# arkworks-rs/sumcheck

Measured on AMD Instinct MI355X. Metric: MLSumcheck prover field-ops/s (BLS12-381 Fr, nv=24), higher is better.
Workload: dtype u256 (BLS12-381 Fr, Montgomery form; integer arithmetic on 9 x 29-bit limbs); 1 GPU; BASELINE config 3: MLSumcheck prove, ListOfProducts [[0, 1, 2, 3], [4, 5, 6], [7, 8], [9]] over 10 tables, nv=24 (24 per GPU shard), BLS12-381 Fr, tables HBM-resident; nv=24, nv_per_gpu=24, tables=10, degree=4, launcher=single process, ranks_seen=1, communicator=none, round_loop=library, round_loop_reason=single GPU: no exchange

## Files before the change

include/sumcheck_hip.h:

```cpp
#ifndef SUMCHECK_HIP_H
#define SUMCHECK_HIP_H

#include <stddef.h>
#include <stdint.h>

#ifdef __cplusplus
extern "C" {
#endif

#define SC_ABI_VERSION 5
#define SC_API __attribute__((visibility("default")))

enum sc_status {
    SC_OK = 0,
    SC_ERR_CONSTANT_POLY = 1,
    SC_ERR_FIRST_ROUND_HAS_MSG = 2,
    SC_ERR_MISSING_MSG = 3,
    SC_ERR_NOT_ACTIVE = 4,
    SC_ERR_BAD_ARG = 5,
    SC_ERR_HIP = 6,
    SC_ERR_OOM = 7,
    SC_ERR_REJECT = 8
};

enum sc_flags {
    SC_TABLES_ON_DEVICE = 1u << 0,
    SC_TABLES_BORROW = 1u << 1,
    SC_TABLES_STREAM = 1u << 2,
    SC_NO_DEVICE_POLLING = 1u << 3
};

typedef struct sc_poly_desc {
    uint32_t num_vars;
    uint32_t max_multiplicands;
    uint32_t n_products;
    const uint64_t *coeffs;
    const uint32_t *prod_offsets;
    const uint32_t *prod_indices;
    uint32_t n_tables;
    const uint64_t *const *tables;
    uint32_t flags;
} sc_poly_desc;

typedef struct sc_prover sc_prover;
typedef struct sc_rng sc_rng;

SC_API int sc_abi_version(void);
SC_API const char *sc_last_error(void);
SC_API int sc_device_count(void);
SC_API int sc_set_device(int ordinal);

SC_API int sc_prover_init(const sc_poly_desc *desc, sc_prover **out);
SC_API int sc_prover_init_streamed(const sc_poly_desc *desc, uint32_t chunk_log2, sc_prover **out);
SC_API int sc_prove_round(sc_prover *p, const uint64_t *r_or_null, uint64_t *out_evals);
SC_API int sc_prover_set_resident(sc_prover *p, uint32_t patience_polls);
SC_API int sc_prover_push_randomness(sc_prover *p, const uint64_t *r);
SC_API int sc_prover_state(sc_prover *p, uint64_t *randomness, uint32_t *n_randomness, uint64_t *tables_out, uint32_t *round);
SC_API void sc_prover_free(sc_prover *p);
SC_API int sc_prover_set_stream(sc_prover *p, void *hip_stream, int use_own);
SC_API int sc_prover_set_polling(sc_prover *p, int allow);

SC_API int sc_prove_round_partial(sc_prover *p, const uint64_t *r_or_null, uint64_t *d_wide_out);
SC_API int sc_wide_reduce(const uint64_t *wide, uint32_t n_elems, uint64_t *out);
SC_API int sc_prover_bind_final(sc_prover *p, const uint64_t *r, uint64_t *d_out);

typedef struct sc_comm sc_comm;
typedef int (*sc_allreduce_u64_fn)(void *ctx, uint64_t *inout, size_t count);
typedef int (*sc_allgather_fn)(void *ctx, const void *send, void *recv, size_t bytes);
SC_API int sc_comm_unique_id(uint8_t *out128);
SC_API int sc_comm_init(const uint8_t *id128, int rank, int nranks, sc_comm **out);
SC_API int sc_comm_init_host(int rank, int nranks, sc_allreduce_u64_fn allreduce, sc_allgather_fn allgather, void *ctx, sc_comm **out);
SC_API int sc_comm_init_p2p(uint64_t group_id, int rank, int nranks, sc_comm **out);
SC_API int sc_comm_selftest(sc_comm *comm);
SC_API void sc_comm_free(sc_comm *comm);
#define SC_COMM_RCCL 1
#define SC_COMM_HOST 2
#define SC_COMM_P2P 3
#define SC_COMM_DIRECT_PUBLISH 0x100
SC_API int sc_comm_info(sc_comm *comm, int *rank_out, int *nranks_out, int *kind_out);
SC_API int sc_comm_exchange_bench(sc_comm *comm, uint32_t n_words, uint32_t iters, double *us_mean_out, double *us_min_out_or_null);
SC_API int sc_set_publish_timeout_ms(uint32_t ms);
SC_API int sc_ml_prove_sharded(sc_prover *p, sc_comm *comm, sc_rng *rng_or_null, uint32_t nv_total, uint64_t *out_proof,
                               uint64_t *out_randomness);
SC_API int sc_ml_prove_sharded_rounds(sc_prover *p, sc_comm *comm, sc_rng *rng, uint32_t nv_total, uint32_t n_rounds, uint64_t *out_proof,
                                      uint64_t *out_randomness);

SC_API int sc_fix_variables(const uint64_t *in, uint32_t nv, const uint64_t *point, uint32_t k, uint64_t *out, uint32_t flags);

SC_API sc_rng *sc_rng_setup(void);
SC_API void sc_rng_free(sc_rng *rng);
SC_API void sc_rng_feed_bytes(sc_rng *rng, const uint8_t *buf, size_t len);
SC_API void sc_rng_fill_bytes(sc_rng *rng, uint8_t *dest, size_t len);
SC_API void sc_rng_feed_poly_info(sc_rng *rng, uint64_t max_multiplicands, uint64_t num_variables);
SC_API void sc_rng_feed_prover_msg(sc_rng *rng, const uint64_t *evals, uint32_t n);
SC_API void sc_rng_sample_fr(sc_rng *rng, uint64_t *out);

SC_API int sc_ml_prove(const sc_poly_desc *desc, sc_rng *rng_or_null, uint64_t *out_proof, sc_prover **out_state_or_null);
SC_API int sc_ml_prove_rounds(sc_prover *p, sc_rng *rng, uint32_t n_rounds, uint64_t *out_proof, uint64_t *out_randomness);
SC_API int sc_ml_prove_handle(sc_prover *p, sc_rng *rng_or_null, uint64_t *out_proof);
SC_API int sc_ml_prove_batch(const sc_poly_desc *descs, uint32_t n, sc_rng *const *rngs_or_null, uint64_t *out_proofs,
                             uint64_t *out_randomness_or_null);

SC_API int sc_interpolate_uni_poly(const uint64_t *p_i, uint32_t len, const uint64_t *eval_at, uint64_t *out);
SC_API int sc_ml_verify(uint32_t num_vars, uint32_t max_multiplicands, const uint64_t *claimed_sum, const uint64_t *proof,
                 uint64_t proof_elems, sc_rng *rng_or_null, uint64_t *out_point, uint64_t *out_expected);

SC_API int sc_gkr_phase_one(const uint64_t *f1_idx, const uint64_t *f1_vals, uint64_t nnz, uint32_t dim, const uint64_t *f3,
                     const uint64_t *g, uint32_t flags, uint64_t *h_g, uint64_t *f1g_idx, uint64_t *f1g_vals, uint64_t *f1g_nnz);
SC_API int sc_gkr_phase_two(const uint64_t *f1g_idx, const uint64_t *f1g_vals, uint64_t nnz, uint32_t dim, const uint64_t *u,
                     uint32_t flags, uint64_t *f1_gu);
SC_API int sc_gkr_prove(sc_rng *rng, const uint64_t *f1_idx, const uint64_t *f1_vals, uint64_t nnz, uint32_t dim,
                 const uint64_t *f2, const uint64_t *f3, const uint64_t *g, uint32_t flags, uint64_t *out_proof, uint64_t *out_uv_or_null);
SC_API int sc_gkr_prove_batch(uint32_t n, uint32_t dim, sc_rng *const *rngs,
                              const uint64_t *const *f1_idx, const uint64_t *const *f1_vals, const uint64_t *nnz,
                              const uint64_t *const *f2, const uint64_t *const *f3, const uint64_t *const *g,
                              uint32_t flags, uint64_t *out_proofs, uint64_t *out_uv_or_null);
SC_API int sc_gkr_phase_one_sharded(sc_comm *comm_or_null, const uint64_t *f1_idx, const uint64_t *f1_vals, uint64_t nnz_local, uint32_t dim,
                                    const uint64_t *f3, const uint64_t *g, uint32_t flags, uint64_t *h_g_or_null, uint64_t *lanes_or_null,
                                    uint64_t *f1g_idx, uint64_t *f1g_vals, uint64_t *f1g_nnz);
SC_API int sc_gkr_phase_two_sharded(sc_comm *comm_or_null, const uint64_t *f1g_idx, const uint64_t *f1g_vals, uint64_t nnz_local, uint32_t dim,
                                    const uint64_t *u, uint32_t flags, uint64_t *f1_gu_or_null, uint64_t *lanes_or_null);
SC_API int sc_gkr_prove_sharded(sc_comm *comm, sc_rng *rng, const uint64_t *f1_idx, const uint64_t *f1_vals, uint64_t nnz_local, uint32_t dim,
                                const uint64_t *f2, const uint64_t *f3, const uint64_t *g, uint32_t flags, uint64_t *out_proof,
                                uint64_t *out_uv_or_null);
SC_API int sc_wide_reduce_table(const uint64_t *lanes, uint64_t n, uint64_t *out, uint32_t flags);
SC_API int sc_dense_scale(const uint64_t *in, uint64_t n, const uint64_t *scalar, uint64_t *out, uint32_t flags);

SC_API int sc_poly_evaluate(const sc_poly_desc *desc, const uint64_t *point, uint64_t *out_value, uint64_t *out_table_values_or_null);

SC_API int sc_sparse_evaluate(const uint64_t *idx, const uint64_t *vals, uint64_t nnz, uint32_t num_vars, const uint64_t *point,
                              uint64_t *out);

SC_API int sc_poly_evaluate_batch(const sc_poly_desc *descs, uint32_t n, const uint64_t *points,
                                  uint64_t *out_values, uint64_t *out_table_values_or_null);
SC_API int sc_gkr_subclaim_batch(uint32_t n, uint32_t dim,
                                 const uint64_t *const *f1_idx, const uint64_t *const *f1_vals, const uint64_t *nnz,
                                 const uint64_t *const *f2, const uint64_t *const *f3, const uint64_t *const *g,
                                 const uint64_t *uv, uint32_t flags, uint64_t *out_evals);

SC_API int sc_release_caches(void);
SC_API int sc_set_cache_limit(uint64_t bytes);
SC_API int sc_library_stats(uint64_t *out, uint32_t n);
SC_API int sc_set_policy(const char *key, int64_t value);
SC_API int sc_get_policy(const char *key, int64_t *value);
SC_API uint32_t sc_plan_count(void);
SC_API const char *sc_plan_name(uint32_t i);
SC_API int sc_plan_stats(uint64_t *out, uint32_t n);

SC_API int sc_synth_table_device(uint64_t seed, uint64_t stream, uint64_t first, uint64_t n, uint64_t *d_out);
SC_API int sc_prover_last_round_ms(sc_prover *p, float *ms);
SC_API int sc_prover_set_timing(sc_prover *p, int on);
SC_API int sc_prover_get_timing(sc_prover *p, double *ms_per_product, uint64_t *launches_per_product, double *rounds_ms);
SC_API int sc_prover_get_round_timing(sc_prover *p, double *ms_per_round, uint64_t *launches_per_round);
SC_API int sc_prover_reset(sc_prover *p, const uint64_t *const *tables_or_null, uint32_t flags);
SC_API int sc_claim_weights(uint32_t M, const uint64_t *r, uint64_t *out);
SC_API int sc_fr_elementwise(int op, const uint64_t *a, const uint64_t *b, uint64_t *out, uint64_t n);
SC_API int sc_bench_modmul(uint64_t n_threads, uint32_t reps, uint32_t variant, float *ms_out, uint64_t *checksum_out);

#ifdef __cplusplus
}
#endif
#endif
```

sumcheck_amd/_lib.py:

```python
from __future__ import annotations

import ctypes as C
import os

HERE = os.path.dirname(os.path.abspath(__file__))
SO_PATH = os.path.join(HERE, "libsumcheck_hip_exp.so" if os.environ.get("SC_LIB_VARIANT") == "exp" else "libsumcheck_hip.so")
if os.environ.get("SC_LIB_PATH"):
    SO_PATH = os.environ["SC_LIB_PATH"]

u64p = C.POINTER(C.c_uint64)
u32p = C.POINTER(C.c_uint32)
u8p = C.POINTER(C.c_uint8)

SC_OK = 0
SC_ERR_CONSTANT_POLY = 1
SC_ERR_FIRST_ROUND_HAS_MSG = 2
SC_ERR_MISSING_MSG = 3
SC_ERR_NOT_ACTIVE = 4
SC_ERR_BAD_ARG = 5
SC_ERR_HIP = 6
SC_ERR_OOM = 7
SC_ERR_REJECT = 8

SC_TABLES_ON_DEVICE = 1
SC_TABLES_BORROW = 2
SC_TABLES_STREAM = 4
SC_NO_DEVICE_POLLING = 8


class PolyDesc(C.Structure):
    _fields_ = [
        ("num_vars", C.c_uint32),
        ("max_multiplicands", C.c_uint32),
        ("n_products", C.c_uint32),
        ("coeffs", u64p),
        ("prod_offsets", u32p),
        ("prod_indices", u32p),
        ("n_tables", C.c_uint32),
        ("tables", C.POINTER(C.c_void_p)),
        ("flags", C.c_uint32),
    ]


_V = C.c_void_p
SIGNATURES = {
    "sc_abi_version": (C.c_int, []),
    "sc_last_error": (C.c_char_p, []),
    "sc_device_count": (C.c_int, []),
    "sc_set_device": (C.c_int, [C.c_int]),
    "sc_prover_init": (C.c_int, [C.POINTER(PolyDesc), C.POINTER(_V)]),
    "sc_prover_init_streamed": (C.c_int, [C.POINTER(PolyDesc), C.c_uint32, C.POINTER(_V)]),
    "sc_prove_round": (C.c_int, [_V, _V, _V]),
    "sc_prover_push_randomness": (C.c_int, [_V, _V]),
    "sc_prover_state": (C.c_int, [_V, _V, u32p, _V, u32p]),
    "sc_prover_free": (None, [_V]),
    "sc_prover_set_stream": (C.c_int, [_V, _V, C.c_int]),
    "sc_prover_set_polling": (C.c_int, [_V, C.c_int]),
    "sc_prover_set_resident": (C.c_int, [_V, C.c_uint32]),
    "sc_set_cache_limit": (C.c_int, [C.c_uint64]),
    "sc_library_stats": (C.c_int, [u64p, C.c_uint32]),
    "sc_set_policy": (C.c_int, [C.c_char_p, C.c_int64]),
    "sc_get_policy": (C.c_int, [C.c_char_p, C.POINTER(C.c_int64)]),
    "sc_plan_count": (C.c_uint32, []),
    "sc_plan_name": (C.c_char_p, [C.c_uint32]),
    "sc_plan_stats": (C.c_int, [u64p, C.c_uint32]),
    "sc_prove_round_partial": (C.c_int, [_V, _V, _V]),
    "sc_wide_reduce": (C.c_int, [_V, C.c_uint32, _V]),
    "sc_prover_bind_final": (C.c_int, [_V, _V, _V]),
    "sc_comm_unique_id": (C.c_int, [_V]),
    "sc_comm_init": (C.c_int, [_V, C.c_int, C.c_int, C.POINTER(_V)]),
    "sc_comm_init_host": (C.c_int, [C.c_int, C.c_int, _V, _V, _V, C.POINTER(_V)]),
    "sc_comm_init_p2p": (C.c_int, [C.c_uint64, C.c_int, C.c_int, C.POINTER(_V)]),
    "sc_comm_selftest": (C.c_int, [_V]),
    "sc_comm_free": (None, [_V]),
    "sc_comm_info": (C.c_int, [_V, C.POINTER(C.c_int), C.POINTER(C.c_int), C.POINTER(C.c_int)]),
    "sc_comm_exchange_bench": (C.c_int, [_V, C.c_uint32, C.c_uint32, C.POINTER(C.c_double), C.POINTER(C.c_double)]),
    "sc_set_publish_timeout_ms": (C.c_int, [C.c_uint32]),
    "sc_ml_prove_sharded": (C.c_int, [_V, _V, _V, C.c_uint32, _V, _V]),
    "sc_ml_prove_sharded_rounds": (C.c_int, [_V, _V, _V, C.c_uint32, C.c_uint32, _V, _V]),
    "sc_fix_variables": (C.c_int, [_V, C.c_uint32, _V, C.c_uint32, _V, C.c_uint32]),
    "sc_poly_evaluate": (C.c_int, [_V, _V, _V, _V]),
    "sc_ml_prove_rounds": (C.c_int, [_V, _V, C.c_uint32, _V, _V]),
    "sc_release_caches": (C.c_int, []),
    "sc_sparse_evaluate": (C.c_int, [_V, _V, C.c_uint64, C.c_uint32, _V, _V]),
    "sc_rng_setup": (_V, []),
    "sc_rng_free": (None, [_V]),
    "sc_rng_feed_bytes": (None, [_V, C.c_char_p, C.c_size_t]),
    "sc_rng_fill_bytes": (None, [_V, _V, C.c_size_t]),
    "sc_rng_feed_poly_info": (None, [_V, C.c_uint64, C.c_uint64]),
    "sc_rng_feed_prover_msg": (None, [_V, _V, C.c_uint32]),
    "sc_rng_sample_fr": (None, [_V, _V]),
    "sc_ml_prove": (C.c_int, [C.POINTER(PolyDesc), _V, _V, C.POINTER(_V)]),
    "sc_ml_prove_handle": (C.c_int, [_V, _V, _V]),
    "sc_ml_prove_batch": (C.c_int, [C.POINTER(PolyDesc), C.c_uint32, C.POINTER(_V), _V, _V]),
    "sc_interpolate_uni_poly": (C.c_int, [_V, C.c_uint32, _V, _V]),
    "sc_ml_verify": (C.c_int, [C.c_uint32, C.c_uint32, _V, _V, C.c_uint64, _V, _V, _V]),
    "sc_gkr_phase_one": (C.c_int, [_V, _V, C.c_uint64, C.c_uint32, _V, _V, C.c_uint32, _V, _V, _V, u64p]),
    "sc_gkr_phase_two": (C.c_int, [_V, _V, C.c_uint64, C.c_uint32, _V, C.c_uint32, _V]),
    "sc_gkr_prove": (C.c_int, [_V, _V, _V, C.c_uint64, C.c_uint32, _V, _V, _V, C.c_uint32, _V, _V]),
    "sc_gkr_prove_batch": (C.c_int, [C.c_uint32, C.c_uint32, C.POINTER(_V), C.POINTER(_V), C.POINTER(_V), u64p, C.POINTER(_V), C.POINTER(_V), C.POINTER(_V),
                                     C.c_uint32, _V, _V]),
    "sc_poly_evaluate_batch": (C.c_int, [C.POINTER(PolyDesc), C.c_uint32, _V, _V, _V]),
    "sc_gkr_subclaim_batch": (C.c_int, [C.c_uint32, C.c_uint32, C.POINTER(_V), C.POINTER(_V), u64p, C.POINTER(_V), C.POINTER(_V), C.POINTER(_V), _V, C.c_uint32, _V]),
    "sc_dense_scale": (C.c_int, [_V, C.c_uint64, _V, _V, C.c_uint32]),
    "sc_gkr_phase_one_sharded": (C.c_int, [_V, _V, _V, C.c_uint64, C.c_uint32, _V, _V, C.c_uint32, _V, _V, _V, _V, u64p]),
    "sc_gkr_phase_two_sharded": (C.c_int, [_V, _V, _V, C.c_uint64, C.c_uint32, _V, C.c_uint32, _V, _V]),
    "sc_gkr_prove_sharded": (C.c_int, [_V, _V, _V, _V, C.c_uint64, C.c_uint32, _V, _V, _V, C.c_uint32, _V, _V]),
    "sc_wide_reduce_table": (C.c_int, [_V, C.c_uint64, _V, C.c_uint32]),
    "sc_synth_table_device": (C.c_int, [C.c_uint64, C.c_uint64, C.c_uint64, C.c_uint64, _V]),
    "sc_prover_last_round_ms": (C.c_int, [_V, C.POINTER(C.c_float)]),
    "sc_prover_set_timing": (C.c_int, [_V, C.c_int]),
    "sc_prover_get_timing": (C.c_int, [_V, C.POINTER(C.c_double), u64p, C.POINTER(C.c_double)]),
    "sc_prover_get_round_timing": (C.c_int, [_V, C.POINTER(C.c_double), u64p]),
    "sc_prover_reset": (C.c_int, [_V, _V, C.c_uint32]),
    "sc_claim_weights": (C.c_int, [C.c_uint32, _V, _V]),
    "sc_fr_elementwise": (C.c_int, [C.c_int, _V, _V, _V, C.c_uint64]),
    "sc_bench_modmul": (C.c_int, [C.c_uint64, C.c_uint32, C.c_uint32, C.POINTER(C.c_float), u64p]),
}

ABI_VERSION = 5
_lib = None


def _missing_symbol(name):
    def stub(*_a, **_k):
        raise SumcheckError(SC_ERR_BAD_ARG, f"{SO_PATH} does not export {name} (an older build loaded with SC_AB_ALLOW_MISSING=1)")
    return stub


class SumcheckError(RuntimeError):
    def __init__(self, code: int, msg: str):
        super().__init__(f"[sc_status {code}] {msg}")
        self.code = code
        self.msg = msg


def lib():
    global _lib
    if _lib is None:
        if not os.path.exists(SO_PATH):
            raise ImportError(
                f"{SO_PATH} is missing: build it with `python -c 'import __graft_entry__ as g; g.build()'` "
                "(sumcheck_amd has no CPU fallback)")
        try:
            import torch
        except Exception:
            pass
        L = C.CDLL(SO_PATH)
        allow_missing = os.environ.get("SC_AB_ALLOW_MISSING") == "1"
        for name, (res, args) in SIGNATURES.items():
            try:
                fn = getattr(L, name)
            except AttributeError:
                if not allow_missing:
                    raise
                setattr(L, name, _missing_symbol(name))
                continue
            fn.restype = res
            fn.argtypes = args
        got = L.sc_abi_version()
        if got != ABI_VERSION:
            msg = f"{SO_PATH} reports ABI version {got}, this loader declares {ABI_VERSION}: signatures may not match"
            if not allow_missing:
                raise ImportError(msg + " (rebuild: python -c 'import __graft_entry__ as g; g.build()')")
            import warnings
            warnings.warn(msg)
        _lib = L
    return _lib


def check(rc: int):
    if rc != SC_OK:
        raise SumcheckError(rc, lib().sc_last_error().decode("utf-8", "replace"))


def set_policy(key: str, value: int) -> None:
    check(lib().sc_set_policy(key.encode(), int(value)))


def get_policy(key: str) -> int:
    v = C.c_int64()
    check(lib().sc_get_policy(key.encode(), C.byref(v)))
    return int(v.value)


class policy:

    def __init__(self, **kv):
        self.kv, self.old = kv, {}

    def __enter__(self):
        for k, v in self.kv.items():
            self.old[k] = get_policy(k)
            set_policy(k, v)
        return self

    def __exit__(self, *exc):
        for k, v in self.old.items():
            set_policy(k, v)
        return False


def plan_stats() -> dict:
    L = lib()
    n = L.sc_plan_count()
    out = (C.c_uint64 * n)()
    check(L.sc_plan_stats(out, n))
    return {L.sc_plan_name(i).decode(): int(out[i]) for i in range(n)}
```

sumcheck_amd/csrc/abi.hip:

```cpp
#include "prover_internal.hpp"

static std::atomic<uint32_t> g_publish_timeout_ms{0};
std::chrono::milliseconds publish_timeout() {
    uint32_t ms = g_publish_timeout_ms.load(std::memory_order_relaxed);
    if (ms == 0) {
        const char *e = std::getenv("SC_PUBLISH_TIMEOUT_MS");
        const long v = e ? std::atol(e) : 0;
        ms = v > 0 ? (uint32_t)std::min<long>(v, 3600 * 1000L) : 20000u;
        g_publish_timeout_ms.store(ms, std::memory_order_relaxed);
    }
    return std::chrono::milliseconds(ms);
}
extern "C" int sc_set_publish_timeout_ms(uint32_t ms) {
    g_publish_timeout_ms.store(ms ? ms : 20000u, std::memory_order_relaxed);
    return SC_OK;
}
static thread_local std::string g_last_error;
static thread_local int g_device = 0;

static std::recursive_mutex g_gate_mutex[64];
thread_local uint16_t g_gate_depth[64];
void gate_lock(int device) {
    g_gate_mutex[(unsigned)device & 63u].lock();
    ++g_gate_depth[(unsigned)device & 63u];
}
void gate_unlock(int device) {
    --g_gate_depth[(unsigned)device & 63u];
    g_gate_mutex[(unsigned)device & 63u].unlock();
}
void sc_internal_gate_lock(int device) { gate_lock(device); }
void sc_internal_gate_unlock(int device) { gate_unlock(device); }

uint64_t sc_internal_cache_limit();
int sc_internal_device() { return g_device; }
int &sc_internal_device_ref() { return g_device; }

int sc_internal_fail(int code, const char *fmt, ...) {
    char buf[512];
    va_list ap;
    va_start(ap, fmt);
    vsnprintf(buf, sizeof(buf), fmt, ap);
    va_end(ap);
    g_last_error = buf;
    return code;
}

extern "C" int sc_abi_version(void) { return SC_ABI_VERSION; }
extern "C" const char *sc_last_error(void) { return g_last_error.c_str(); }
extern "C" int sc_device_count(void) {
    int n = 0;
    if (hipGetDeviceCount(&n) != hipSuccess) {
        (void)hipGetLastError();
        return 0;
    }
    return n;
}
extern "C" int sc_set_device(int ordinal) {
    HIP_TRY(hipSetDevice(ordinal));
    g_device = ordinal;
    return SC_OK;
}

extern "C" sc_rng *sc_rng_setup(void) { return new (std::nothrow) sc_rng(); }
extern "C" void sc_rng_free(sc_rng *rng) { delete rng; }
extern "C" void sc_rng_feed_bytes(sc_rng *rng, const uint8_t *buf, size_t len) { rng->rng.feed_bytes(buf, len); }
extern "C" void sc_rng_fill_bytes(sc_rng *rng, uint8_t *dest, size_t len) { rng->rng.fill_bytes(dest, len); }
extern "C" void sc_rng_feed_poly_info(sc_rng *rng, uint64_t max_multiplicands, uint64_t num_variables) {
    rng->rng.feed_poly_info(max_multiplicands, num_variables);
}
extern "C" void sc_rng_feed_prover_msg(sc_rng *rng, const uint64_t *evals, uint32_t n) {
    rng->rng.feed_prover_msg(reinterpret_cast<const sch::Fr *>(evals), n);
}
extern "C" void sc_rng_sample_fr(sc_rng *rng, uint64_t *out) {
    const sch::Fr a = rng->rng.sample_fr();
    std::memcpy(out, a.l, 32);
}


int resident_quiesce(sc_prover *p);
void prover_destroy(sc_prover *p) {
    if (!p) return;
    (void)resident_quiesce(p);
    DeviceGate gate_(p->device);
    (void)hipSetDevice(p->device);
    if (p->deferred_pending && p->sig) {
        __atomic_store_n(p->sig, p->sig_seq, __ATOMIC_RELEASE);
        p->deferred_pending = false;
    }
    if (p->own_stream) (void)hipStreamSynchronize(p->own_stream);
    if (p->arena) (void)hipFree(p->arena);
    if (p->d_partials) (void)hipFree(p->d_partials);
    if (p->d_partials2) (void)hipFree(p->d_partials2);
    if (p->d_fin_counters) (void)hipFree(p->d_fin_counters);
    if (p->d_finprods) (void)hipFree(p->d_finprods);
    if (p->d_W) (void)hipFree(p->d_W);
    if (p->d_scratch) (void)hipFree(p->d_scratch);
    if (p->d_sums[0]) (void)hipFree(p->d_sums[0]);
    if (p->d_out) (void)hipFree(p->d_out);
    if (p->h_out) (void)hipHostFree(p->h_out);
    if (p->h_flag) (void)hipHostFree(p->h_flag);
    for (int q = 0; q < 2; ++q) {
        if (p->ring[q]) (void)hipFree(p->ring[q]);
        if (p->ev_copied[q]) (void)hipEventDestroy(p->ev_copied[q]);
        if (p->ev_consumed[q]) (void)hipEventDestroy(p->ev_consumed[q]);
    }
    if (p->d_chunk_msg) (void)hipFree(p->d_chunk_msg);
    if (p->copy_stream) (void)hipStreamDestroy(p->copy_stream);
    if (p->copy_stream2) (void)hipStreamDestroy(p->copy_stream2);
    for (int q = 0; q < 2; ++q)
        if (p->ev_copied2[q]) (void)hipEventDestroy(p->ev_copied2[q]);
    if (p->tail) prover_destroy(p->tail);
    if (p->d_tail_send) (void)hipFree(p->d_tail_send);
    if (p->d_tail_recv) (void)hipFree(p->d_tail_recv);
    if (p->d_tail_tabs) (void)hipFree(p->d_tail_tabs);
    if (p->d_wide) (void)hipFree(p->d_wide);
    if (p->h_wide) (void)hipHostFree(p->h_wide);
    if (p->d_combos) (void)hipFree(p->d_combos);
    if (p->h_mail) (void)hipHostFree(p->h_mail);
    if (p->d_mail) (void)hipFree(p->d_mail);
    if (p->d_tail_sync) (void)hipFree(p->d_tail_sync);
    if (p->d_tail_xw) (void)hipFree(p->d_tail_xw);
    if (p->d_vram_mail) (void)hipFree(p->d_vram_mail);
    if (p->d_cur_tables) (void)hipFree(p->d_cur_tables);
    if (p->h_cur_tables) (void)hipHostFree(p->h_cur_tables);
    if (p->d_slot_table) (void)hipFree(p->d_slot_table);
    if (p->d_slot_exp) (void)hipFree(p->d_slot_exp);
    if (p->ev0) (void)hipEventDestroy(p->ev0);
    if (p->ev1) (void)hipEventDestroy(p->ev1);
    for (hipEvent_t e : p->prod_ev) (void)hipEventDestroy(e);
    if (p->own_stream) (void)hipStreamDestroy(p->own_stream);
    delete p;
}

bool handle_pool_offer(sc_prover *p);
extern "C" void sc_prover_free(sc_prover *p) {
    if (p) (void)resident_quiesce(p);
    if (p && handle_pool_offer(p)) return;
    prover_destroy(p);
}

int validate_desc(const sc_poly_desc *d) {
    if (!d) return sc_internal_fail(SC_ERR_BAD_ARG, "null descriptor");
    if (d->num_vars == 0) return sc_internal_fail(SC_ERR_CONSTANT_POLY, "Attempt to prove a constant.");
    if (d->num_vars > 40) return sc_internal_fail(SC_ERR_BAD_ARG, "num_vars %u too large", d->num_vars);
    if (d->n_tables == 0 || !d->tables) return sc_internal_fail(SC_ERR_BAD_ARG, "no tables");
    if (d->n_products && (!d->coeffs || !d->prod_offsets || !d->prod_indices)) return sc_internal_fail(SC_ERR_BAD_ARG, "null product arrays");
    uint32_t mx = 0;
    for (uint32_t k = 0; k < d->n_products; ++k) {
        if (d->prod_offsets[k + 1] <= d->prod_offsets[k]) return sc_internal_fail(SC_ERR_BAD_ARG, "product %u is empty", k);
        mx = std::max(mx, d->prod_offsets[k + 1] - d->prod_offsets[k]);
        for (uint32_t q = d->prod_offsets[k]; q < d->prod_offsets[k + 1]; ++q)
            if (d->prod_indices[q] >= d->n_tables) return sc_internal_fail(SC_ERR_BAD_ARG, "product %u refers to table %u >= %u", k, d->prod_indices[q], d->n_tables);
    }
    if (mx != d->max_multiplicands) return sc_internal_fail(SC_ERR_BAD_ARG, "max_multiplicands %u != max product length %u", d->max_multiplicands, mx);
    for (uint32_t u = 0; u < d->n_tables; ++u)
        if (!d->tables[u]) return sc_internal_fail(SC_ERR_BAD_ARG, "table %u is null", u);
    return SC_OK;
}

sch::Fr fr_small(int64_t v) { return v >= 0 ? sch::from_u64((uint64_t)v) : sch::neg(sch::from_u64((uint64_t)(-v))); }

void build_node_matrix(uint32_t M, uint32_t D, const sch::Fr &scale, std::vector<sch::Fr> &out) {
    std::vector<int64_t> xs;
    std::vector<uint32_t> fin;
    int inf_col = -1;
    for (uint32_t s = 0; s <= M; ++s) {
        const int32_t nv = scd::node_value((int)s);
        if (nv == scd::kNodeInf) inf_col = (int)s;
        else fin.push_back(s);
        xs.push_back(nv);
    }
    out.assign((size_t)D * (M + 1), sch::zero());
    for (uint32_t t = 0; t < D; ++t) {
        sch::Fr inf_w = sch::kOne;
        for (uint32_t e = 0; e < M; ++e) inf_w = sch::mul(inf_w, fr_small(t));
        for (uint32_t s : fin) {
            sch::Fr num = sch::kOne, den = sch::kOne;
            for (uint32_t j : fin) {
                if (j == s) continue;
                num = sch::mul(num, fr_small((int64_t)t - xs[j]));
                den = sch::mul(den, fr_small(xs[s] - xs[j]));
            }
            const sch::Fr l = sch::mul(num, sch::inverse(den));
            out[(size_t)t * (M + 1) + s] = sch::mul(scale, l);
            if (inf_col >= 0) {
                sch::Fr xm = sch::kOne;
                for (uint32_t e = 0; e < M; ++e) xm = sch::mul(xm, fr_small(xs[s]));
                inf_w = sch::sub(inf_w, sch::mul(xm, l));
            }
        }
        if (inf_col >= 0) out[(size_t)t * (M + 1) + inf_col] = sch::mul(scale, inf_w);
    }
}

void claim_weights(uint32_t M, const sch::Fr &r, sch::Fr *lam) {
    struct Den {
        sch::Fr inv[5][5];
        Den() {
            for (uint32_t m = 1; m <= 4; ++m)
                for (uint32_t s = 0; s <= m; ++s) {
                    inv[m][s] = sch::zero();
                    if (scd::node_value((int)s) == scd::kNodeInf) continue;
                    sch::Fr den = sch::kOne;
                    for (uint32_t j = 0; j <= m; ++j)
                        if (j != s && scd::node_value((int)j) != scd::kNodeInf) den = sch::mul(den, fr_small((int64_t)scd::node_value((int)s) - scd::node_value((int)j)));
                    inv[m][s] = sch::inverse(den);
                }
        }
    };
    static const Den den;
    sch::Fr diff[5];
    for (uint32_t j = 0; j <= M; ++j)
        if (scd::node_value((int)j) != scd::kNodeInf) diff[j] = sch::sub(r, fr_small(scd::node_value((int)j)));
    sch::Fr inf_w = sch::kOne;
    for (uint32_t e = 0; e < M; ++e) inf_w = sch::mul(inf_w, r);
    int inf_col = -1;
    for (uint32_t s = 0; s <= M; ++s) {
        const int32_t xs = scd::node_value((int)s);
        if (xs == scd::kNodeInf) {
            inf_col = (int)s;
            continue;
        }
        sch::Fr l = den.inv[M][s];
        for (uint32_t j = 0; j <= M; ++j)
            if (j != s && scd::node_value((int)j) != scd::kNodeInf) l = sch::mul(l, diff[j]);
        lam[s] = l;
        sch::Fr xm = sch::kOne;
        for (uint32_t e = 0; e < M; ++e) xm = sch::mul(xm, fr_small(xs));
        inf_w = sch::sub(inf_w, sch::mul(xm, l));
    }
    if (inf_col >= 0) lam[inf_col] = inf_w;
}

int prover_build(const sc_poly_desc *d, sc_prover *p) {
    DeviceGate gate_(g_device);
    if (sc_device_count() <= 0) return sc_internal_fail(SC_ERR_HIP, "no HIP device visible: libsumcheck_hip has no CPU fallback");
    p->device = g_device;
    HIP_TRY(hipSetDevice(p->device));
    HIP_TRY(hipStreamCreateWithFlags(&p->own_stream, hipStreamNonBlocking));
    p->stream = p->own_stream;
    HIP_TRY(hipEventCreate(&p->ev0));
    HIP_TRY(hipEventCreate(&p->ev1));
    p->nv = d->num_vars;
    p->max_mult = d->max_multiplicands;
    p->D = d->max_multiplicands + 1;
    p->K = d->n_products;
    p->U = d->n_tables;
    p->randomness.reserve(p->nv);
    if (d->flags & SC_NO_DEVICE_POLLING) {
        p->pipeline_ok = false;
        p->polling_off_by_caller = true;
    }
#ifdef SC_EXPERIMENTS
    if (const char *e = std::getenv("SC_FE")) p->use_fe = std::atoi(e) != 0;
    if (const char *e = std::getenv("SC_KERNEL")) p->kernel_variant = std::atoi(e);
    if (!p->use_fe && p->kernel_variant == 3) p->kernel_variant = 0;
#endif
    p->use_f29 = p->kernel_variant == 3;
    p->wide_tree = wide_tree_enabled();
#ifdef SC_EXPERIMENTS
    if (const char *e = std::getenv("SC_F29")) p->use_f29 = p->use_f29 && std::atoi(e) != 0;
#endif
    for (uint32_t k = 0; k < d->n_products; ++k)
        if (d->prod_offsets[k + 1] - d->prod_offsets[k] > (p->wide_tree ? 8u : 4u)) p->use_f29 = false;
    if (d->n_tables > (uint32_t)scd::kMaxSmallTables) p->use_f29 = false;
    p->merge_rounds = p->kernel_variant == 3 && d->n_products > 0 && d->n_products <= (uint32_t)scd::kMaxRoundProds;
    for (uint32_t k = 0; k < d->n_products; ++k)
        if (d->prod_offsets[k + 1] - d->prod_offsets[k] > 4) p->merge_rounds = false;
#ifdef SC_EXPERIMENTS
    if (const char *e = std::getenv("SC_MERGE")) p->merge_rounds = p->merge_rounds && std::atoi(e) != 0;
    if (const char *e = std::getenv("SC_FUSED_FIN")) p->fused_finalize = std::atoi(e) != 0;
#endif
    p->use_tail = scd::policy(scd::kPolTail) != 0;

    uint64_t partial_elems = 0;
    std::vector<uint32_t> slot_table, slot_exp;
    std::vector<FinProd> fin(p->K);
    std::vector<Combo> combos;
    std::vector<sch::Fr> Wall;
    for (uint32_t k = 0; k < p->K; ++k) {
        Product pr;
        std::memcpy(&pr.coeff, d->coeffs + 4 * k, 32);
        if (sch::geq_p(pr.coeff)) return sc_internal_fail(SC_ERR_BAD_ARG, "coefficient %u is not a canonical field element", k);
        for (uint32_t q = d->prod_offsets[k]; q < d->prod_offsets[k + 1]; ++q) {
            const uint32_t t = d->prod_indices[q];
            auto it = std::find(pr.tables.begin(), pr.tables.end(), t);
            if (it == pr.tables.end()) {
                pr.tables.push_back(t);
                pr.exps.push_back(1);
            } else {
                pr.exps[it - pr.tables.begin()]++;
            }
        }
        p->prod_indices.emplace_back(d->prod_indices + d->prod_offsets[k], d->prod_indices + d->prod_offsets[k + 1]);
        pr.M = d->prod_offsets[k + 1] - d->prod_offsets[k];
        pr.fused = pr.M <= (uint32_t)scd::kMaxFusedM;
        if (!pr.fused) p->any_generic = true;
        pr.partial_off = partial_elems;
        partial_elems += (uint64_t)scd::kMaxGrid * (pr.M + 1);
        pr.slot_off = (uint32_t)slot_table.size();
        slot_table.insert(slot_table.end(), pr.tables.begin(), pr.tables.end());
        slot_exp.insert(slot_exp.end(), pr.exps.begin(), pr.exps.end());
        fin[k].M = pr.M;
        fin[k].pad = 0;
        fin[k].partial_off = pr.partial_off;
        {
            sch::Fr sc = pr.coeff;
            for (uint32_t dbl = 0; dbl < 5 * (pr.M - 1); ++dbl) sc = sch::add(sc, sc);
            std::vector<sch::Fr> w;
            fin[k].w_off = Wall.size();
            build_node_matrix(pr.M, p->D, pr.coeff, w);
            Wall.insert(Wall.end(), w.begin(), w.end());
            build_node_matrix(pr.M, p->D, sc, w);
            Wall.insert(Wall.end(), w.begin(), w.end());
        }
        for (uint32_t t = 0; t <= pr.M; ++t) {
            Combo c;
            c.t = t;
            c.M = pr.M;
            c.slot_off = pr.slot_off;
            c.n_slots = (uint32_t)pr.tables.size();
            c.partial_off = pr.partial_off;
            combos.push_back(c);
        }
        p->prods.push_back(std::move(pr));
    }

    const bool on_device = d->flags & SC_TABLES_ON_DEVICE;
    const bool borrow = on_device && (d->flags & SC_TABLES_BORROW);
    const uint64_t n = 1ULL << p->nv;
    const bool streamed = !on_device && (d->flags & SC_TABLES_STREAM) && p->nv >= 11;
    const bool small_foot = borrow || streamed;
    bool staged = false;
    const uint64_t s0 = small_foot ? std::max<uint64_t>(n >> 1, 1) : n;
    const uint64_t s1 = small_foot ? std::max<uint64_t>(n >> 2, 1) : std::max<uint64_t>(n >> 1, 1);
    const uint64_t per_table = (s0 + s1) * 36;
    HIP_TRY(hipMalloc(&p->arena, per_table * p->U));
    p->arena_bytes = per_table * p->U;
    p->tabs.resize(p->U);
    p->borrow = borrow;
    if (on_device && !borrow) HIP_TRY(hipDeviceSynchronize());
    for (uint32_t u = 0; u < p->U; ++u) {
        Table &t = p->tabs[u];
        char *base = static_cast<char *>(p->arena) + per_table * u;
        t.buf[0] = reinterpret_cast<uint4 *>(base);
        t.buf[1] = reinterpret_cast<uint4 *>(base + s0 * 32);
        t.buf_top[0] = reinterpret_cast<int32_t *>(base + (s0 + s1) * 32);
        t.buf_top[1] = t.buf_top[0] + s0;
        if (streamed) {
            t.cur = nullptr;
            t.next = 0;
            p->host_tabs.push_back(d->tables[u]);
        } else if (borrow) {
            t.cur = reinterpret_cast<const uint4 *>(d->tables[u]);
            t.next = 0;
            p->origin.push_back(t.cur);
        } else {
            if (!on_device && (d->flags & SC_TABLES_STREAM)) p->host_tabs.push_back(d->tables[u]);
            if (!(staged = !on_device && staged_init_applies(p)))
                HIP_TRY(hipMemcpyAsync(t.buf[0], d->tables[u], n * 32, on_device ? hipMemcpyDeviceToDevice : hipMemcpyHostToDevice, p->stream));
            t.cur = t.buf[0];
            t.next = 1;
        }
    }

    if (streamed) {
        p->streamed = true;
        uint32_t cl = p->stream_chunk_request ? p->stream_chunk_request : 22u;
        cl = std::max(10u, std::min(cl, p->nv));
        p->chunk_log2 = cl;
        for (int q = 0; q < 2; ++q) {
            HIP_TRY(hipMalloc(&p->ring[q], ((size_t)p->U << cl) * 32));
            HIP_TRY(hipEventCreateWithFlags(&p->ev_copied[q], hipEventDisableTiming));
            HIP_TRY(hipEventCreateWithFlags(&p->ev_consumed[q], hipEventDisableTiming));
        }
        HIP_TRY(hipStreamCreateWithFlags(&p->copy_stream, hipStreamNonBlocking));
        HIP_TRY(hipMalloc(&p->d_chunk_msg, (size_t)2 * p->D * 32));
    }
    HIP_TRY(hipMalloc(&p->d_partials, std::max<uint64_t>(partial_elems, 1) * 32));
    HIP_TRY(hipMalloc(&p->d_partials2, std::max<uint64_t>(partial_elems, 1) * 32));
    HIP_TRY(hipMalloc(&p->d_fin_counters, 4 * (2 + scd::kMaxGrid / 32 + 16)));
    HIP_TRY(hipMemsetAsync(p->d_fin_counters, 0, 4 * (2 + scd::kMaxGrid / 32 + 16), p->stream));
    p->d_fin_mb_counter = p->d_fin_counters + (2 + scd::kMaxGrid / 32 + 8);
    HIP_TRY(hipMalloc(&p->d_finprods, std::max<size_t>(p->K, 1) * sizeof(FinProd)));
    if (p->K) HIP_TRY(hipMemcpyAsync(p->d_finprods, fin.data(), p->K * sizeof(FinProd), hipMemcpyHostToDevice, p->stream));
    p->h_finprods = fin;
    HIP_TRY(hipMalloc(&p->d_W, std::max<size_t>(2 * Wall.size(), 1) * 32));
    p->w_elems = (uint32_t)Wall.size();
    if (!Wall.empty()) {
        HIP_TRY(hipMemcpyAsync(p->d_W, Wall.data(), Wall.size() * 32, hipMemcpyHostToDevice, p->stream));
        HIP_TRY(hipMemcpyAsync(p->d_W + Wall.size(), Wall.data(), Wall.size() * 32, hipMemcpyHostToDevice, p->stream));
    }
    HIP_TRY(hipMalloc(&p->d_scratch, (size_t)(2 + p->D) * std::max<uint32_t>(p->K, 1) * p->D * 32));
    {
        const size_t one = (size_t)std::max<uint32_t>(p->K, 1) * p->D * 32;
        HIP_TRY(hipMalloc(&p->d_sums[0], 2 * one));
        p->d_sums[1] = reinterpret_cast<FrHost *>(reinterpret_cast<char *>(p->d_sums[0]) + one);
    }
    HIP_TRY(hipMalloc(&p->d_out, (size_t)p->D * 32));
    HIP_TRY(hipHostMalloc(reinterpret_cast<void **>(&p->h_out), (size_t)p->D * 32, hipHostMallocMapped | hipHostMallocCoherent));
    HIP_TRY(hipHostMalloc(reinterpret_cast<void **>(&p->h_flag), 64, hipHostMallocMapped | hipHostMallocCoherent));
    *p->h_flag = 0;
    HIP_TRY(hipHostGetDevicePointer(reinterpret_cast<void **>(&p->h_out_dev), p->h_out, 0));
    HIP_TRY(hipHostGetDevicePointer(reinterpret_cast<void **>(&p->h_flag_dev), p->h_flag, 0));
    p->has_meta = combos.size() <= (size_t)scd::kMetaCombos && slot_table.size() <= (size_t)scd::kMetaSlots;
    if (p->has_meta) {
        std::memset(&p->meta, 0, sizeof(p->meta));
        std::copy(combos.begin(), combos.end(), p->meta.combo);
        std::copy(slot_table.begin(), slot_table.end(), p->meta.slot_table);
        std::copy(slot_exp.begin(), slot_exp.end(), p->meta.slot_exp);
    }
    p->n_combos = (int)combos.size();
    HIP_TRY(hipMalloc(&p->d_combos, std::max<size_t>(combos.size(), 1) * sizeof(Combo)));
    if (!combos.empty()) HIP_TRY(hipMemcpyAsync(p->d_combos, combos.data(), combos.size() * sizeof(Combo), hipMemcpyHostToDevice, p->stream));
    HIP_TRY(hipMalloc(&p->d_slot_table, std::max<size_t>(slot_table.size(), 1) * 4));
    HIP_TRY(hipMalloc(&p->d_slot_exp, std::max<size_t>(slot_exp.size(), 1) * 4));
    if (!slot_table.empty()) {
        HIP_TRY(hipMemcpyAsync(p->d_slot_table, slot_table.data(), slot_table.size() * 4, hipMemcpyHostToDevice, p->stream));
        HIP_TRY(hipMemcpyAsync(p->d_slot_exp, slot_exp.data(), slot_exp.size() * 4, hipMemcpyHostToDevice, p->stream));
    }
    if (p->any_generic || p->U > (uint32_t)scd::kMaxSmallTables) {
        HIP_TRY(hipMalloc(&p->d_cur_tables, 2 * p->U * sizeof(void *)));
        HIP_TRY(hipHostMalloc(reinterpret_cast<void **>(&p->h_cur_tables), 2 * p->U * sizeof(void *), hipHostMallocDefault));
    }
    if (staged) {
        int rc_s = staged_copy_and_round1(p, d->tables);
        if (rc_s) return rc_s;
    }
    HIP_TRY(hipStreamSynchronize(p->stream));
    return SC_OK;
}

std::vector<uint8_t> pool_key_of(const sc_poly_desc *d, int device);
sc_prover *handle_pool_take(const std::vector<uint8_t> &key);
void reset_owner_policy(sc_prover *p, uint32_t desc_flags) {
    p->polling_off_by_caller = (desc_flags & SC_NO_DEVICE_POLLING) != 0;
    p->pipeline_ok = !p->polling_off_by_caller;
    p->resident_spins = kResidentSpinsDefault;
    if (p->timing) (void)sc_prover_set_timing(p, 0);
    p->n_retries = 0;
}
extern "C" int sc_prover_init(const sc_poly_desc *desc, sc_prover **out) {
    if (!out) return sc_internal_fail(SC_ERR_BAD_ARG, "null out");
    *out = nullptr;
    int rc = validate_desc(desc);
    if (rc) return rc;
    std::vector<uint8_t> key = pool_key_of(desc, g_device);
    if (sc_prover *kept = handle_pool_take(key)) {
        if (sc_prover_reset(kept, desc->tables, desc->flags & SC_TABLES_ON_DEVICE) == SC_OK) {
            reset_owner_policy(kept, desc->flags);
            *out = kept;
            return SC_OK;
        }
        kept->pool_key.clear();
        prover_destroy(kept);
    }
    sc_prover *p = new (std::nothrow) sc_prover();
    if (!p) return sc_internal_fail(SC_ERR_OOM, "host allocation failed");
    rc = prover_build(desc, p);
    if (rc) {
        prover_destroy(p);
        return rc;
    }
    p->pool_key = std::move(key);
    *out = p;
    return SC_OK;
}

extern "C" int sc_prover_init_streamed(const sc_poly_desc *desc, uint32_t chunk_log2, sc_prover **out) {
    if (!out) return sc_internal_fail(SC_ERR_BAD_ARG, "null out");
    *out = nullptr;
    int rc = validate_desc(desc);
    if (rc) return rc;
    if (desc->flags & SC_TABLES_ON_DEVICE) return sc_internal_fail(SC_ERR_BAD_ARG, "streamed tables are host tables");
    sc_prover *p = new (std::nothrow) sc_prover();
    if (!p) return sc_internal_fail(SC_ERR_OOM, "host allocation failed");
    p->stream_chunk_request = chunk_log2;
    sc_poly_desc d2 = *desc;
    d2.flags |= SC_TABLES_STREAM;
    rc = prover_build(&d2, p);
    if (rc) {
        prover_destroy(p);
        return rc;
    }
    *out = p;
    return SC_OK;
}

extern "C" int sc_prover_set_stream(sc_prover *p, void *hip_stream, int use_own) {
    if (!p) return sc_internal_fail(SC_ERR_BAD_ARG, "null prover");
    int rc_q = resident_quiesce(p);
    if (rc_q) return rc_q;
    DeviceGate gate_(p->device);
    HIP_TRY(hipSetDevice(p->device));
    HIP_TRY(hipStreamSynchronize(p->stream));
    p->stream = use_own ? p->own_stream : static_cast<hipStream_t>(hip_stream);
    return SC_OK;
}

int collect_timing(sc_prover *p) {
    if (!p->timing || !p->timing_pending) return SC_OK;
    HIP_TRY(hipEventSynchronize(p->ev1));
    float ms = 0.f;
    HIP_TRY(hipEventElapsedTime(&ms, p->ev0, p->ev1));
    p->rounds_ms += ms;
    for (uint32_t k = 0; k < (p->prod_merged ? 1u : p->K) && p->prod_timed; ++k) {
        HIP_TRY(hipEventElapsedTime(&ms, p->prod_ev[2 * k], p->prod_ev[2 * k + 1]));
        p->prod_ms[k] += ms;
        p->prod_launches[k] += 1;
        if (p->timed_round >= 1 && p->timed_round <= p->round_kernel_ms.size()) {
            p->round_kernel_ms[p->timed_round - 1] += ms;
            if (k == 0) p->round_kernel_launches[p->timed_round - 1] += 1;
        }
    }
    p->timing_pending = false;
    return SC_OK;
}

int prover_bind_out(sc_prover *p, const uint64_t *r, uint64_t *d_out) {
    int rc_q = resident_quiesce(p);
    if (rc_q) return rc_q;
    DeviceGate gate_(p->device);
    if (p->exhausted || p->round == 0 || p->round > p->nv) return sc_internal_fail(SC_ERR_NOT_ACTIVE, "bind needs a prover that has run at least one round");
    if (p->streamed && p->round < 2) return sc_internal_fail(SC_ERR_NOT_ACTIVE, "a streamed handle's tables are resident from round 2 on: nothing to bind yet");
    sch::Fr rr;
    std::memcpy(&rr, r, 32);
    if (sch::geq_p(rr)) return sc_internal_fail(SC_ERR_BAD_ARG, "challenge is not a canonical field element");
    HIP_TRY(hipSetDevice(p->device));
    p->randomness.push_back(rr);
    const uint64_t n_out = 1ULL << (p->nv - p->round);
    for (uint32_t u0 = 0; u0 < p->U; u0 += (uint32_t)scd::kMaxSmallTables) {
        const uint32_t cnt = std::min<uint32_t>(p->U - u0, (uint32_t)scd::kMaxSmallTables);
        TablePtrs tp;
        std::memset(&tp, 0, sizeof(tp));
        for (uint32_t j = 0; j < cnt; ++j) {
            tp.src[j] = p->tabs[u0 + j].cur;
// ... 355 lines not shown
    DeviceGate gate_(g_device);
    HIP_TRY(hipSetDevice(g_device));
    const bool on_device = d->flags & SC_TABLES_ON_DEVICE;
    const uint64_t n = 1ULL << nv;
    std::vector<int> levels;
    for (uint32_t left = nv; left > 0;) {
        const int l = left >= 3 ? 3 : (int)left;
        levels.push_back(l);
        left -= l;
    }
    const uint64_t na = levels.empty() ? 1 : n >> levels[0];
    const uint64_t nb = levels.size() < 2 ? 1 : na >> levels[1];
    const size_t bytes_stage = on_device ? 0 : (size_t)U * n * 32, bytes_a = (size_t)U * na * 32, bytes_b = (size_t)U * nb * 32, bytes_v = (size_t)U * 32;
    struct Area {
        void *p = nullptr;
    } stage, wa, wb, vals;
    EvalLease lease;
    DevMem own;
    StreamGuard sg;
    hipStream_t s_eval = nullptr;
    char *base = static_cast<char *>(lease.get(g_device, bytes_stage + bytes_a + bytes_b + bytes_v, &s_eval));
    if (!base) {
        HIP_TRY(hipMalloc(&own.p, bytes_stage + bytes_a + bytes_b + bytes_v));
        HIP_TRY(hipStreamCreateWithFlags(&sg.s, hipStreamNonBlocking));
        base = static_cast<char *>(own.p);
        s_eval = sg.s;
    }
    stage.p = base;
    wa.p = base + bytes_stage;
    wb.p = base + bytes_stage + bytes_a;
    vals.p = base + bytes_stage + bytes_a + bytes_b;
    std::vector<const uint4 *> cur(U);
    for (uint32_t u = 0; u < U; ++u) {
        if (on_device) {
            cur[u] = reinterpret_cast<const uint4 *>(d->tables[u]);
        } else {
            uint4 *dst = static_cast<uint4 *>(stage.p) + 2 * n * u;
            HIP_TRY(hipMemcpyAsync(dst, d->tables[u], n * 32, hipMemcpyHostToDevice, s_eval));
            cur[u] = dst;
        }
    }
    uint64_t m = n;
    uint32_t var = 0;
    for (size_t ps = 0; ps < levels.size(); ++ps) {
        const int L = levels[ps];
        m >>= L;
        const bool last = ps + 1 == levels.size();
        uint4 *area = static_cast<uint4 *>((ps & 1) ? wb.p : wa.p);
        for (uint32_t u0 = 0; u0 < U; u0 += (uint32_t)scd::kMaxSmallTables) {
            const uint32_t cnt = std::min<uint32_t>(U - u0, (uint32_t)scd::kMaxSmallTables);
            scd::FoldArgs fa;
            std::memset(&fa, 0, sizeof(fa));
            for (uint32_t j = 0; j < cnt; ++j) {
                fa.src[j] = cur[u0 + j];
                fa.dst[j] = last ? static_cast<uint4 *>(vals.p) + 2 * (u0 + j) : area + 2 * m * (u0 + j);
            }
            for (int l = 0; l < L; ++l) {
                sch::Fr r32v = pt[var + l];
                for (int dbl = 0; dbl < 5; ++dbl) r32v = sch::add(r32v, r32v);
                fa.r32[l] = to_dev(r32v);
            }
            HIP_TRY(scd::launch_fold_multi(fa, L, (int)cnt, m, s_eval));
            for (uint32_t j = 0; j < cnt; ++j) cur[u0 + j] = fa.dst[j];
        }
        var += L;
    }
    std::vector<sch::Fr> tv(U);
    if (levels.empty()) {
        for (uint32_t u = 0; u < U; ++u) HIP_TRY(hipMemcpyAsync(&tv[u], cur[u], 32, hipMemcpyDeviceToHost, s_eval));
    } else {
        HIP_TRY(hipMemcpyAsync(tv.data(), vals.p, (size_t)U * 32, hipMemcpyDeviceToHost, s_eval));
    }
    HIP_TRY(hipStreamSynchronize(s_eval));
    sch::Fr acc = sch::zero();
    for (uint32_t k = 0; k < d->n_products; ++k) {
        sch::Fr pr;
        std::memcpy(&pr, d->coeffs + 4 * k, 32);
        if (sch::geq_p(pr)) return sc_internal_fail(SC_ERR_BAD_ARG, "coefficient %u is not a canonical field element", k);
        for (uint32_t q = d->prod_offsets[k]; q < d->prod_offsets[k + 1]; ++q) pr = sch::mul(pr, tv[d->prod_indices[q]]);
        acc = sch::add(acc, pr);
    }
    std::memcpy(out_value, &acc, 32);
    if (out_table_values_or_null) std::memcpy(out_table_values_or_null, tv.data(), (size_t)U * 32);
    return SC_OK;
}

static std::atomic<uint64_t> g_cache_limit{16ULL << 30};
uint64_t sc_internal_cache_limit() { return g_cache_limit.load(std::memory_order_relaxed); }
struct HandlePool {
    std::mutex mu;
    sc_prover *h = nullptr;
};
static HandlePool g_pool;
std::vector<uint8_t> pool_key_of(const sc_poly_desc *d, int device) {
    std::vector<uint8_t> k;
    auto put = [&](const void *p, size_t n) {
        const uint8_t *b = static_cast<const uint8_t *>(p);
        k.insert(k.end(), b, b + n);
    };
    const uint32_t head[8] = {d->num_vars, d->max_multiplicands, d->n_products, d->n_tables, d->flags, (uint32_t)device,
                              (uint32_t)scd::policy(scd::kPolWideTree), (uint32_t)scd::policy(scd::kPolTail)};
    put(head, sizeof(head));
    if (d->n_products) {
        put(d->prod_offsets, (size_t)(d->n_products + 1) * 4);
        put(d->prod_indices, (size_t)d->prod_offsets[d->n_products] * 4);
        put(d->coeffs, (size_t)d->n_products * 32);
    }
    return k;
}
sc_prover *handle_pool_take(const std::vector<uint8_t> &key) {
    std::lock_guard<std::mutex> lk(g_pool.mu);
    if (!g_pool.h || g_pool.h->pool_key != key) return nullptr;
    sc_prover *p = g_pool.h;
    g_pool.h = nullptr;
    return p;
}
bool handle_pool_offer(sc_prover *p) {
    if (p->pool_key.empty() || p->arena_bytes > sc_internal_cache_limit() || p->streamed) return false;
    if (p->stream != p->own_stream) return false;
    abandon_deferred(p);
    {
        DeviceGate gate_(p->device);
        (void)hipSetDevice(p->device);
        (void)hipStreamSynchronize(p->own_stream);
    }
    if (p->timing) (void)sc_prover_set_timing(p, 0);
    sc_prover *old = nullptr;
    {
        std::lock_guard<std::mutex> lk(g_pool.mu);
        old = g_pool.h;
        g_pool.h = p;
    }
    if (old) prover_destroy(old);
    return true;
}
void sc_internal_release_handle_pool() {
    sc_prover *old = nullptr;
    {
        std::lock_guard<std::mutex> lk(g_pool.mu);
        old = g_pool.h;
        g_pool.h = nullptr;
    }
    if (old) prover_destroy(old);
}

namespace {
struct PolicyDef {
    const char *name;
    int64_t def, lo, hi;
};
constexpr PolicyDef kPolicyDefs[scd::kPolCount] = {
    {"pipeline", 1, 0, 1},     {"resident", 1, 0, 1},          {"tail_slices", 1, 0, 1}, {"vram_mailbox", 1, 0, 1},           {"wide_tree", 1, 0, 1},
    {"rccl_direct", 1, 0, 1},  {"shard_gather_log2", 15, 1, 15}, {"gkr_direct", 1, 0, 1},  {"wait_spins", 1 << 22, 1, 0xffffffffLL}, {"tail", 1, 0, 1},
    {"staged_init", 1, 0, 1},  {"batch", 1, 0, 2},
};
struct PolicyTable {
    std::atomic<int64_t> v[scd::kPolCount];
    PolicyTable() {
        for (int i = 0; i < scd::kPolCount; ++i) {
            int64_t x = kPolicyDefs[i].def;
#ifdef SC_EXPERIMENTS
            std::string env = "SC_";
            for (const char *c = kPolicyDefs[i].name; *c; ++c) env += (char)std::toupper((unsigned char)*c);
            if (const char *e = std::getenv(env.c_str())) x = std::min(std::max<int64_t>(std::atoll(e), kPolicyDefs[i].lo), kPolicyDefs[i].hi);
#endif
            v[i].store(x, std::memory_order_relaxed);
        }
    }
};
PolicyTable &policy_table() {
    static PolicyTable t;
    return t;
}
std::atomic<uint64_t> g_plan[scd::kPlanCount];
constexpr const char *kPlanNames[scd::kPlanCount] = {
    "big.merged.round1", "big.merged.bind_chain", "big.merged.bind", "big.claim_identity", "big.store_f29", "big.store_canonical", "big.per_product_tree",
    "big.wide", "big.wide16", "big.generic", "big.node_by_node", "big.bind_pass", "big.streamed", "big.staged_round1", "finalize.multi_block", "finalize.one_block", "finalize.no_lds",
    "small.launched", "small.combos_table", "small.ptrs", "small.pipelined", "tail.slices8", "tail.slices12", "tail.rounds", "resident.slices",
    "resident.rounds", "sharded.rccl_direct", "sharded.rccl_publish", "sharded.host", "sharded.p2p", "sharded.gather_tail", "gkr.bucketed_grouped",
    "gkr.bucketed_counted", "gkr.list_form", "gkr.coeff_from_bound_table", "gkr.sharded", "fold_multi",
    "batch.eval_one_block", "batch.eval_serial", "batch.gkr_eval_one_block", "batch.gkr_eval_serial",
    "batch.one_block", "batch.serial", "batch.gkr_one_block", "batch.gkr_serial",
};
}
int64_t scd::policy(int key) { return key >= 0 && key < scd::kPolCount ? policy_table().v[key].load(std::memory_order_relaxed) : 0; }
void scd::plan_hit(int plan) {
    if (plan >= 0 && plan < scd::kPlanCount) g_plan[plan].fetch_add(1, std::memory_order_relaxed);
}
extern "C" int sc_set_policy(const char *key, int64_t value) {
    if (!key) return sc_internal_fail(SC_ERR_BAD_ARG, "null policy key");
    for (int i = 0; i < scd::kPolCount; ++i) {
        if (std::strcmp(key, kPolicyDefs[i].name) != 0) continue;
        if (value < kPolicyDefs[i].lo || value > kPolicyDefs[i].hi)
            return sc_internal_fail(SC_ERR_BAD_ARG, "policy %s takes %lld..%lld", key, (long long)kPolicyDefs[i].lo, (long long)kPolicyDefs[i].hi);
        policy_table().v[i].store(value, std::memory_order_relaxed);
        return SC_OK;
    }
    return sc_internal_fail(SC_ERR_BAD_ARG, "unknown policy key '%s'", key);
}
extern "C" int sc_get_policy(const char *key, int64_t *value) {
    if (!key || !value) return sc_internal_fail(SC_ERR_BAD_ARG, "null argument");
    for (int i = 0; i < scd::kPolCount; ++i) {
        if (std::strcmp(key, kPolicyDefs[i].name) != 0) continue;
        *value = scd::policy(i);
        return SC_OK;
    }
    return sc_internal_fail(SC_ERR_BAD_ARG, "unknown policy key '%s'", key);
}
extern "C" uint32_t sc_plan_count(void) { return (uint32_t)scd::kPlanCount; }
extern "C" const char *sc_plan_name(uint32_t i) { return i < (uint32_t)scd::kPlanCount ? kPlanNames[i] : nullptr; }
extern "C" int sc_plan_stats(uint64_t *out, uint32_t n) {
    if (!out) return sc_internal_fail(SC_ERR_BAD_ARG, "null argument");
    for (uint32_t i = 0; i < n; ++i) out[i] = i < (uint32_t)scd::kPlanCount ? g_plan[i].load(std::memory_order_relaxed) : 0;
    return SC_OK;
}

extern "C" int sc_library_stats(uint64_t *out, uint32_t n) {
    if (!out) return sc_internal_fail(SC_ERR_BAD_ARG, "null argument");
    for (uint32_t i = 0; i < n; ++i) out[i] = i < 8 ? g_stat[i].load(std::memory_order_relaxed) : 0;
    return SC_OK;
}

extern "C" int sc_set_cache_limit(uint64_t bytes) {
    const uint64_t before = g_cache_limit.exchange(bytes);
    return bytes < before ? sc_release_caches() : SC_OK;
}

extern "C" int sc_prover_set_resident(sc_prover *p, uint32_t patience_polls) {
    if (!p) return sc_internal_fail(SC_ERR_BAD_ARG, "null prover");
    int rc_q = resident_quiesce(p);
    if (rc_q) return rc_q;
    p->resident_spins = patience_polls;
    return SC_OK;
}

extern "C" int sc_prover_set_polling(sc_prover *p, int allow) {
    if (!p) return sc_internal_fail(SC_ERR_BAD_ARG, "null prover");
    if (p->deferred_pending) return sc_internal_fail(SC_ERR_BAD_ARG, "a pipelined round is waiting for its challenge");
    int rc_q = resident_quiesce(p);
    if (rc_q) return rc_q;
    p->pipeline_ok = allow != 0;
    p->polling_off_by_caller = allow == 0;
    return SC_OK;
}


sch::Fr fr_from_u128(sch::u128 x) {
    const sch::Fr lo = sch::from_u64((uint64_t)x), hi = sch::from_u64((uint64_t)(x >> 64));
    static const sch::Fr two64 = sch::mul(sch::Fr{{0, 1, 0, 0}}, sch::kR2);
    return sch::add(lo, sch::mul(hi, two64));
}

sch::Fr interpolate(const sch::Fr *y, uint32_t len, const sch::Fr &x) {
    std::vector<sch::Fr> evals;
    evals.reserve(len);
    sch::Fr prod = x;
    evals.push_back(x);
    sch::Fr check = sch::zero();
    for (uint32_t i = 1; i < len; ++i) {
        if (sch::eq(x, check)) return y[i - 1];
        check = sch::add(check, sch::kOne);
        const sch::Fr tmp = sch::sub(x, check);
        evals.push_back(tmp);
        prod = sch::mul(prod, tmp);
    }
    if (sch::eq(x, check)) return y[len - 1];
    sch::Fr res = sch::zero();
    auto term = [&](uint32_t i, const sch::Fr &num, const sch::Fr &den) {
        res = sch::add(res, sch::mul(sch::mul(sch::mul(y[i], prod), num), sch::inverse(sch::mul(den, evals[i]))));
    };
    if (len <= 20) {
        uint64_t fact = 1;
        for (uint32_t k = 2; k < len; ++k) fact *= k;
        const sch::Fr last_denom = sch::from_u64(fact);
        int64_t ratio_numerator = 1;
        uint64_t ratio_enumerator = 1;
        for (uint32_t i = len; i-- > 0;) {
            const sch::Fr rn = ratio_numerator < 0 ? sch::neg(sch::from_u64((uint64_t)(-ratio_numerator))) : sch::from_u64((uint64_t)ratio_numerator);
            term(i, sch::from_u64(ratio_enumerator), sch::mul(last_denom, rn));
            if (i != 0) {
                ratio_numerator *= -((int64_t)len - (int64_t)i);
                ratio_enumerator *= (uint64_t)i;
            }
        }
    } else if (len <= 33) {
        sch::u128 fact = 1;
        for (uint32_t k = 2; k < len; ++k) fact *= k;
        const sch::Fr last_denom = fr_from_u128(fact);
        __int128 ratio_numerator = 1;
        sch::u128 ratio_enumerator = 1;
        for (uint32_t i = len; i-- > 0;) {
            const sch::Fr rn = ratio_numerator < 0 ? sch::neg(fr_from_u128((sch::u128)(-ratio_numerator))) : fr_from_u128((sch::u128)ratio_numerator);
            term(i, fr_from_u128(ratio_enumerator), sch::mul(last_denom, rn));
            if (i != 0) {
                ratio_numerator *= -((__int128)len - (__int128)i);
                ratio_enumerator *= (sch::u128)i;
            }
        }
    } else {
        sch::Fr denom_up = sch::kOne;
        for (uint32_t k = 1; k < len; ++k) denom_up = sch::mul(denom_up, sch::from_u64(k));
        sch::Fr denom_down = sch::kOne;
        for (uint32_t i = len; i-- > 0;) {
            term(i, denom_down, denom_up);
            if (i != 0) {
                denom_up = sch::mul(denom_up, sch::neg(sch::from_u64(len - i)));
                denom_down = sch::mul(denom_down, sch::from_u64(i));
            }
        }
    }
    return res;
}

int require_canonical(const uint64_t *limbs, size_t n_elems, const char *what) {
    for (size_t i = 0; i < n_elems; ++i) {
        sch::Fr v;
        std::memcpy(&v, limbs + 4 * i, 32);
        if (sch::geq_p(v)) return sc_internal_fail(SC_ERR_BAD_ARG, "%s element %zu is not a canonical field element", what, i);
    }
    return SC_OK;
}

extern "C" int sc_interpolate_uni_poly(const uint64_t *p_i, uint32_t len, const uint64_t *eval_at, uint64_t *out) {
    if (!p_i || !eval_at || !out || len == 0) return sc_internal_fail(SC_ERR_BAD_ARG, "null argument");
    int rc = require_canonical(p_i, len, "p_i");
    if (!rc) rc = require_canonical(eval_at, 1, "eval_at");
    if (rc) return rc;
    sch::Fr x;
    std::memcpy(&x, eval_at, 32);
    const sch::Fr v = interpolate(reinterpret_cast<const sch::Fr *>(p_i), len, x);
    std::memcpy(out, v.l, 32);
    return SC_OK;
}

extern "C" int sc_ml_verify(uint32_t num_vars, uint32_t max_multiplicands, const uint64_t *claimed_sum, const uint64_t *proof,
                            uint64_t proof_elems, sc_rng *rng_or_null, uint64_t *out_point, uint64_t *out_expected) {
    if (!claimed_sum || !proof || !out_point || !out_expected) return sc_internal_fail(SC_ERR_BAD_ARG, "null argument");
    if (max_multiplicands == 0 || max_multiplicands == UINT32_MAX)
        return sc_internal_fail(SC_ERR_BAD_ARG, "max_multiplicands %u: a round message needs at least two evaluations", max_multiplicands);
    const uint32_t D = max_multiplicands + 1;
    if (proof_elems != (uint64_t)num_vars * D) return sc_internal_fail(SC_ERR_BAD_ARG, "incorrect number of evaluations");
    int rc = require_canonical(claimed_sum, 1, "claimed_sum");
    if (!rc) rc = require_canonical(proof, (size_t)proof_elems, "proof");
    if (rc) return rc;
    sc_rng local;
    sch::Blake2b512Rng &rng = rng_or_null ? rng_or_null->rng : local.rng;
    rng.feed_poly_info(max_multiplicands, num_vars);
    const sch::Fr *msgs = reinterpret_cast<const sch::Fr *>(proof);
    std::vector<sch::Fr> rs(num_vars);
    for (uint32_t i = 0; i < num_vars; ++i) {
        rng.feed_prover_msg(msgs + (size_t)i * D, D);
        rs[i] = rng.sample_fr();
    }
    sch::Fr expected;
    std::memcpy(&expected, claimed_sum, 32);
    for (uint32_t i = 0; i < num_vars; ++i) {
        const sch::Fr *ev = msgs + (size_t)i * D;
        if (!sch::eq(sch::add(ev[0], ev[1]), expected)) return sc_internal_fail(SC_ERR_REJECT, "Prover message is not consistent with the claim.");
        expected = interpolate(ev, D, rs[i]);
    }
    if (num_vars) std::memcpy(out_point, rs.data(), (size_t)num_vars * 32);
    std::memcpy(out_expected, expected.l, 32);
    return SC_OK;
}

extern "C" int sc_wide_reduce(const uint64_t *wide, uint32_t n_elems, uint64_t *out) {
    if (!wide || !out) return sc_internal_fail(SC_ERR_BAD_ARG, "null argument");
    for (uint32_t e = 0; e < n_elems; ++e) {
        uint64_t v[6] = {0, 0, 0, 0, 0, 0};
        for (int j = 0; j < 8; ++j) {
            const uint64_t lane = wide[8 * (size_t)e + j];
            const int w = j >> 1, sh = (j & 1) * 32;
            sch::u128 add = (sch::u128)lane << sh;
            sch::u128 c = (sch::u128)v[w] + (uint64_t)add;
            v[w] = (uint64_t)c;
            c = (c >> 64) + (uint64_t)(add >> 64);
            for (int q = w + 1; q < 6 && c != 0; ++q) {
                c += v[q];
                v[q] = (uint64_t)c;
                c >>= 64;
            }
        }
        if (v[5] != 0) return sc_internal_fail(SC_ERR_BAD_ARG, "wide lanes overflow");
        sch::Fr lo = {{v[0], v[1], v[2], v[3]}};
        while (sch::geq_p(lo)) lo = sch::sub_p(lo);
        const sch::Fr hi = sch::mul(sch::Fr{{v[4], 0, 0, 0}}, sch::kR2);
        const sch::Fr res = sch::add(lo, hi);
        std::memcpy(out + 4 * (size_t)e, res.l, 32);
    }
    return SC_OK;
}

extern "C" int sc_synth_table_device(uint64_t seed, uint64_t stream, uint64_t first, uint64_t n, uint64_t *d_out) {
    if (!d_out) return sc_internal_fail(SC_ERR_BAD_ARG, "null argument");
    if (sc_device_count() <= 0) return sc_internal_fail(SC_ERR_HIP, "no HIP device visible");
    HIP_TRY(hipSetDevice(g_device));
    HIP_TRY(scd::launch_synth(seed, stream, first, n, reinterpret_cast<uint4 *>(d_out), nullptr));
    HIP_TRY(hipStreamSynchronize(nullptr));
    return SC_OK;
}

extern "C" int sc_claim_weights(uint32_t M, const uint64_t *r, uint64_t *out) {
    if (!r || !out) return sc_internal_fail(SC_ERR_BAD_ARG, "null argument");
    if (M < 1 || M > 4) return sc_internal_fail(SC_ERR_BAD_ARG, "claim weights exist for 1..4 multiplicands, not %u", M);
    sch::Fr rr, lam[5];
    std::memcpy(&rr, r, 32);
    if (sch::geq_p(rr)) return sc_internal_fail(SC_ERR_BAD_ARG, "the point is not a canonical field element");
    claim_weights(M, rr, lam);
    std::memcpy(out, lam, (size_t)(M + 1) * 32);
    return SC_OK;
}

extern "C" int sc_fr_elementwise(int op, const uint64_t *a, const uint64_t *b, uint64_t *out, uint64_t n) {
    if (!a || !b || !out) return sc_internal_fail(SC_ERR_BAD_ARG, "null argument");
    if (op < 0 || op > 5) return sc_internal_fail(SC_ERR_BAD_ARG, "unknown op %d", op);
    if (n == 0) return SC_OK;
    if (sc_device_count() <= 0) return sc_internal_fail(SC_ERR_HIP, "no HIP device visible: libsumcheck_hip has no CPU fallback");
    HIP_TRY(hipSetDevice(g_device));
    void *da = nullptr, *db = nullptr, *dout = nullptr;
    HIP_TRY(hipMalloc(&da, n * 32));
    HIP_TRY(hipMalloc(&db, n * 32));
    HIP_TRY(hipMalloc(&dout, n * 32));
    HIP_TRY(hipMemcpy(da, a, n * 32, hipMemcpyHostToDevice));
    HIP_TRY(hipMemcpy(db, b, n * 32, hipMemcpyHostToDevice));
    FrHost u;
    std::memcpy(&u, b, 32);
    HIP_TRY(scd::launch_fr_elementwise(op, static_cast<const uint4 *>(da), static_cast<const uint4 *>(db), u, static_cast<uint4 *>(dout), n, nullptr));
    HIP_TRY(hipMemcpy(out, dout, n * 32, hipMemcpyDeviceToHost));
    (void)hipFree(da);
    (void)hipFree(db);
    (void)hipFree(dout);
    return SC_OK;
}

extern "C" int sc_bench_modmul(uint64_t n_threads, uint32_t reps, uint32_t variant, float *ms_out, uint64_t *checksum_out) {
    if (!ms_out) return sc_internal_fail(SC_ERR_BAD_ARG, "null argument");
    if (sc_device_count() <= 0) return sc_internal_fail(SC_ERR_HIP, "no HIP device visible");
    HIP_TRY(hipSetDevice(g_device));
    uint64_t *d_sink = nullptr;
    hipEvent_t e0, e1;
    HIP_TRY(hipMalloc(&d_sink, 8));
    HIP_TRY(hipEventCreate(&e0));
    HIP_TRY(hipEventCreate(&e1));
    HIP_TRY(scd::launch_bench_modmul(n_threads, 8, variant, d_sink, nullptr));
    HIP_TRY(hipEventRecord(e0, nullptr));
    HIP_TRY(scd::launch_bench_modmul(n_threads, reps, variant, d_sink, nullptr));
    HIP_TRY(hipEventRecord(e1, nullptr));
    HIP_TRY(hipEventSynchronize(e1));
    HIP_TRY(hipEventElapsedTime(ms_out, e0, e1));
    if (checksum_out) HIP_TRY(hipMemcpy(checksum_out, d_sink, 8, hipMemcpyDeviceToHost));
    (void)hipFree(d_sink);
    (void)hipEventDestroy(e0);
    (void)hipEventDestroy(e1);
    return SC_OK;
}
```

sumcheck_amd/csrc/kernels.h:

```cpp
#pragma once
#include <hip/hip_runtime.h>
#include <stdint.h>

namespace scd {

constexpr int kBlock = 256;
constexpr int kMaxFusedM = 8;
constexpr int kMaxGrid = 1024;
constexpr int kMaxSmallTables = 32;
constexpr uint64_t kSmallRoundPairs = 1u << 14;

struct FrHost {
    uint64_t l[4];
};

constexpr int32_t kNodeInf = 0x7fffffff;
__host__ __device__ constexpr int32_t node_value(int s) {
    return s == 0 ? 0 : s == 1 ? 1 : s == 2 ? kNodeInf : ((s - 3) % 2 == 0 ? -((s - 3) / 2 + 1) : ((s - 3) / 2 + 2));
}

struct BindConst {
    int32_t R[9][9];
};

struct Slot {
    const uint4 *src;
    uint4 *dst;
    uint32_t mode;
    uint32_t exp;
    const int32_t *src_top;
    int32_t *dst_top;
};

struct ProdArgs {
    Slot slot[kMaxFusedM];
    int n_slots;
};
constexpr int kMaxWideM = 12;
struct WideArgs16 {
    Slot slot[kMaxWideM];
    int n_slots;
};

constexpr int kMaxRoundProds = 12;
constexpr int kRoundTreeGrid = 768;
struct TreeProd {
    Slot slot[4];
    uint32_t M;
    uint32_t pad;
    uint64_t partial_off;
};
struct RoundFin {
    int enabled;
    int D;
    uint64_t w_off[kMaxRoundProds];
    const uint4 *Wm;
    uint4 *partials2;
    uint32_t *counters;
    uint4 *out;
    uint64_t *out_wide;
    uint4 *h_out;
    uint32_t *h_flag;
    uint32_t seq;
};
struct RoundArgs {
    TreeProd prod[kMaxRoundProds];
    int n_prod;
    RoundFin fin;
    uint32_t part_stride, part_block0;
};

struct FinProd {
    uint32_t M;
    uint32_t pad;
    uint64_t partial_off;
    uint64_t w_off;
};

struct TablePtrs {
    const uint4 *src[kMaxSmallTables];
    uint4 *dst[kMaxSmallTables];
    const int32_t *src_top[kMaxSmallTables];
};
struct Combo {
    uint32_t t;
    uint32_t M;
    uint32_t slot_off;
    uint32_t n_slots;
    uint64_t partial_off;
};

constexpr int kFoldMaxLevels = 3;
struct FoldArgs {
    const uint4 *src[kMaxSmallTables];
    uint4 *dst[kMaxSmallTables];
    FrHost r32[kFoldMaxLevels];
};
hipError_t launch_fold_multi(const FoldArgs &args, int levels, int n_tables, uint64_t n_out, hipStream_t stream);

constexpr int kMetaProds = 16;
struct FinMeta {
    FinProd prod[kMetaProds];
};
constexpr int kMetaCombos = 24, kMetaSlots = 48;
struct ComboMeta {
    Combo combo[kMetaCombos];
    uint32_t slot_table[kMetaSlots];
    uint32_t slot_exp[kMetaSlots];
};

#ifndef SC_TAIL_MAX_PAIRS
#define SC_TAIL_MAX_PAIRS 2048
#endif
constexpr uint64_t kTailMaxPairs = SC_TAIL_MAX_PAIRS;
static_assert(kTailMaxPairs >= kBlock && (kTailMaxPairs & (kTailMaxPairs - 1)) == 0 && kTailMaxPairs <= kSmallRoundPairs, "a power of two within the small rounds");
constexpr int kTailMaxGrid = 1024;
constexpr int kTailFlatPairs = 16;
__host__ __device__ constexpr uint64_t tail_flat_pairs(int n_combos) {
    uint64_t p = kTailFlatPairs;
    while (p < 64 && 2 * p * (uint64_t)n_combos <= (uint64_t)kBlock) p *= 2;
    return p;
}
struct TailTables {
    const uint4 *cur0[kMaxSmallTables];
    const int32_t *cur0_top[kMaxSmallTables];
    uint4 *b0[kMaxSmallTables];
    uint4 *b1[kMaxSmallTables];
};
struct TailArgs {
    TailTables t;
    int n_tables;
    int n_rounds;
    int first_has_bind;
    uint64_t first_pairs;
    FrHost r0;
    int n_combos, K, D;
    const uint4 *Wm;
    uint4 *partials;
    uint32_t *sync;
    uint4 *sums;
    uint64_t *chal;
    uint4 *h_out;
    uint32_t *h_flag;
    uint32_t seq0;
    uint32_t *sig;
    const uint64_t *mail_host;
    uint32_t sig0;
    uint32_t max_spins;
};
constexpr int kTsBlock = 256, kTsMaxBlocks = 256;
constexpr uint64_t kTsMaxPairs = 1u << 16;
constexpr size_t kTsAccWords = 4 * 8 * (size_t)kMetaCombos * 8;
constexpr size_t kTsXwWords = kTsAccWords + (size_t)kTsMaxBlocks * kMaxSmallTables * 10 + 8;
struct TailSlicesArgs {
    TailArgs base;
    int B;
    uint64_t *xw;
    const uint64_t *mail_vram;
    uint32_t tag0;
    uint32_t fin_bytes;
    uint32_t lds_entries;
    uint32_t stage_off;
};
int tail_slices_blocks(uint64_t first_pairs, int n_tables, int K, int D, int n_combos, int max_multiplicands, int max_blocks);
int tail_slices_max_blocks(int device, int max_multiplicands);
hipError_t ensure_dynamic_lds(const void *kernel, int bytes, bool (&done)[64]);
hipError_t launch_tail_slices(TailSlicesArgs args, const ComboMeta &meta, const FinMeta &fin, int max_multiplicands, hipStream_t stream);
struct BatchArgs {
    const uint4 *const *tables;
    const uint4 *Wm;
    uint32_t w_stride;
    uint32_t n, n_tables, nv;
    int n_combos, K, D;
    uint32_t *ticket;
    uint64_t *h_msg;
    const uint64_t *mail;
    uint32_t mail_local;
    uint32_t *h_giveup;
    uint32_t tag0;
    uint32_t max_spins;
    uint32_t fin_bytes;
};
bool batch_shape_fits(uint32_t nv, uint32_t n_tables, int K, int D, uint32_t max_multiplicands);
int batch_blocks_per_cu(int device, uint32_t nv, uint32_t n_tables, int K, int D);
hipError_t launch_batch_proofs(BatchArgs args, const ComboMeta &meta, const FinMeta &fin, int grid, hipStream_t stream);
constexpr int kGkrBatchMaxDim = 9;
constexpr uint64_t kGkrBatchMaxNnzPerCell = 64;
struct GkrBatchInst {
    const uint64_t *idx;
    const uint4 *vals;
    const uint4 *f2, *f3;
    const uint4 *g;
    uint64_t nnz;
};
struct BatchGkrArgs {
    const GkrBatchInst *inst;
    const uint4 *Wm;
    uint32_t n, dim;
    uint32_t *ticket;
    uint64_t *h_msg;
    const uint64_t *mail;
    uint32_t mail_local;
    uint32_t *h_giveup;
    uint32_t tag0;
    uint32_t max_spins;
    uint32_t fin_bytes;
};
bool gkr_batch_shape_fits(uint32_t dim, uint64_t nnz_max);
int gkr_batch_blocks_per_cu(int device, uint32_t dim);
hipError_t launch_batch_gkr_idx_range(const GkrBatchInst *inst, uint32_t n, uint32_t dim, uint32_t *flags, hipStream_t stream);
hipError_t launch_batch_gkr(BatchGkrArgs args, const ComboMeta &meta, const FinMeta &fin, int grid, hipStream_t stream);
constexpr uint32_t kEvalBatchMaxNv = 14;
struct EvalBatchArgs {
    const uint4 *const *tables;
    const uint4 *points;
    uint4 *out;
    uint32_t nv, group_size, pt_stride, pt_base, pt_step, out_stride, out_base;
};
bool eval_batch_shape_fits(uint32_t nv);
hipError_t launch_batch_eval(const EvalBatchArgs &args, uint32_t blocks, hipStream_t stream);
bool gkr_eval_batch_shape_fits(uint32_t dim, uint64_t nnz_max);
hipError_t launch_batch_gkr_eval(const GkrBatchInst *inst, uint32_t n, uint32_t dim, uint4 *out, uint32_t out_stride, hipStream_t stream);
int tail_max_resident_blocks(int device);
uint32_t wait_spins_default();

enum PolicyKey {
    kPolPipeline = 0,
    kPolResident,
    kPolTailSlices,
    kPolVramMailbox,
    kPolWideTree,
    kPolRcclDirect,
    kPolShardGatherLog2,
    kPolGkrDirect,
    kPolWaitSpins,
    kPolTail,
    kPolStagedInit,
    kPolBatch,
    kPolCount
};
int64_t policy(int key);

enum Plan {
    kPlanBigMergedRound1 = 0,
    kPlanBigMergedBindChain,
    kPlanBigMergedBind,
    kPlanBigClaimIdentity,
    kPlanBigF29Store,
    kPlanBigCanonicalStore,
    kPlanBigPerProductTree,
    kPlanBigWide,
    kPlanBigWide16,
    kPlanBigGeneric,
    kPlanBigNodeByNode,
    kPlanBigBindPass,
    kPlanBigStreamed,
    kPlanBigStagedRound1,
    kPlanFinalizeMultiBlock,
    kPlanFinalizeOneBlock,
    kPlanFinalizeNoLds,
    kPlanSmallLaunched,
    kPlanSmallCombosTable,
    kPlanSmallPtrs,
    kPlanSmallPipelined,
    kPlanTailSlices8,
    kPlanTailSlices12,
    kPlanTailRounds,
    kPlanResidentSlices,
    kPlanResidentRounds,
    kPlanShardedRcclDirect,
    kPlanShardedRcclPublish,
    kPlanShardedHost,
    kPlanShardedP2P,
    kPlanShardedGatherTail,
    kPlanGkrBucketedGrouped,
    kPlanGkrBucketedCounted,
    kPlanGkrListForm,
    kPlanGkrCoeffFromBound,
    kPlanGkrSharded,
    kPlanFoldMulti,
    kPlanBatchEvalOneBlock,
    kPlanBatchEvalSerial,
    kPlanBatchGkrEvalOneBlock,
    kPlanBatchGkrEvalSerial,
    kPlanBatchOneBlock,
    kPlanBatchSerial,
    kPlanBatchGkrOneBlock,
    kPlanBatchGkrSerial,
    kPlanCount
};
void plan_hit(int plan);
hipError_t launch_scale_w_by_table_eval(FrHost *W, const FrHost *W0, uint32_t n, const void *table, const FrHost &r, hipStream_t stream);
hipError_t launch_zero_words(uint32_t *p, uint32_t n, hipStream_t stream, uint32_t *p2 = nullptr, uint32_t n2 = 0);
hipError_t launch_tail_rounds(const TailArgs &args, const ComboMeta &meta, const FinMeta &fin, int grid, hipStream_t stream);

int grid_for_pairs(uint64_t n_pairs);

#ifdef SC_EXPERIMENTS
hipError_t launch_prod_round(int M, const ProdArgs &args, const FrHost &r, uint64_t n_pairs, FrHost *d_partials, int grid,
                             hipStream_t stream);
#endif
hipError_t launch_prod_round_fe(int M, const ProdArgs &args, const FrHost &r32, uint64_t n_pairs, FrHost *d_partials, int grid,
                                hipStream_t stream);
hipError_t launch_prod_tree(int M, const ProdArgs &args, const BindConst &rc, uint64_t n_pairs, FrHost *d_partials, int grid,
                            hipStream_t stream);
hipError_t launch_prod_tree_wide(int M, const ProdArgs &args, const BindConst &rc, uint64_t n_pairs, FrHost *d_partials, int grid, hipStream_t stream);
hipError_t launch_prod_tree_wide16(int M, const WideArgs16 &args, const FrHost &comp, uint64_t n_pairs, FrHost *d_partials, int grid, hipStream_t stream);
hipError_t launch_round_tree(const RoundArgs &args, const BindConst &rc, uint64_t n_pairs, FrHost *d_partials, int grid, hipStream_t stream, bool split = true,
                             bool skip1 = false);
#ifdef SC_EXPERIMENTS
int grid_for_tiles(uint64_t n_pairs);
hipError_t launch_round_tile(int M, const ProdArgs &args, const FrHost &r32, uint64_t n_pairs, FrHost *d_partials, int grid,
                             hipStream_t stream);
#endif
hipError_t launch_sum_generic(const uint4 *const *d_cur_tables, const uint32_t *d_slot_table, const uint32_t *d_slot_exp,
                              int n_slots, int M, uint64_t n_pairs, FrHost *d_partials, int grid, hipStream_t stream);
hipError_t launch_fix(const uint4 *src, uint4 *dst, const FrHost &r, uint64_t n_out, hipStream_t stream);
hipError_t launch_wait_challenge(uint32_t *flag_dev, uint32_t want, const FrHost *mail_host_dev, FrHost *mail_dev, hipStream_t stream,
                                 uint32_t spins_override = 0);
hipError_t launch_fix_multi(const TablePtrs &tp, int n_tables, const FrHost &r, const FrHost *r_mail, uint64_t n_out, hipStream_t stream);
hipError_t launch_sum_combos(const TablePtrs &tp, const Combo *d_combos, int n_combos, const uint32_t *d_slot_table,
                             const uint32_t *d_slot_exp, uint64_t n_pairs, FrHost *d_partials, int grid, hipStream_t stream);
hipError_t launch_sum_combos_ptrs(const uint4 *const *d_cur_tables, const Combo *d_combos, int n_combos, const uint32_t *d_slot_table,
                                  const uint32_t *d_slot_exp, uint64_t n_pairs, FrHost *d_partials, int grid, hipStream_t stream);
hipError_t launch_sum_combos_meta(const TablePtrs &tp, const ComboMeta &meta, int n_combos, uint64_t n_pairs, FrHost *d_partials, int grid,
                                  hipStream_t stream);
struct ClaimArgs {
    uint32_t skip1;
    uint32_t pad;
    const uint4 *prev;
    FrHost lam[14];
};
__host__ __device__ constexpr int claim_off(int M) { return (M - 1) * (M + 2) / 2; }
constexpr int kWideTagShift = 44;
__host__ __device__ constexpr uint32_t wide_tag_of(uint32_t seq) { return (seq & 0x7fffu) + 1u; }
bool finalize_keeps_sums(int K, int D, int nblocks, bool have_host_prods, bool have_counter);
hipError_t launch_finalize(const FinProd *d_prods, const FinProd *h_prods_or_null, const FrHost *d_W, int K, int D, int nblocks, const FrHost *d_partials, FrHost *d_scratch,
                           FrHost *d_out, uint64_t *d_out_wide, FrHost *h_out_mapped, uint32_t *h_flag_mapped, uint32_t seq,
                           int scaled , uint32_t *d_counter_or_null, hipStream_t stream, const ClaimArgs *claim_or_null = nullptr);
hipError_t launch_synth(uint64_t seed, uint64_t stream_id, uint64_t first, uint64_t n, uint4 *d_out, hipStream_t stream);
hipError_t launch_scale(const uint4 *src, uint4 *dst, const FrHost &s, uint64_t n, hipStream_t stream);
hipError_t launch_tag_words(uint64_t *d_words, int n, uint32_t gen, hipStream_t stream);
hipError_t launch_publish_words(const uint64_t *d_src, uint64_t *h_dst_mapped, int n, uint32_t *h_flag_mapped, uint32_t seq, hipStream_t stream);
constexpr int kP2PMaxRanks = 16, kP2PWords = 64;
constexpr size_t kP2PInboxWords = 2 * (size_t)kP2PMaxRanks * kP2PWords;
constexpr uint32_t kP2PRetryBit = 0x80000000u;
struct P2PArgs {
    uint64_t *inbox[kP2PMaxRanks];
    int nranks, rank, n_words;
    uint32_t gen;
    uint32_t max_spins;
};
struct PeerLanes {
    const uint64_t *p[kP2PMaxRanks];
    int n;
};
hipError_t launch_sum_peer_lanes(const PeerLanes &peers, uint64_t n_words, uint64_t *out, hipStream_t stream);
hipError_t launch_p2p_allreduce(const P2PArgs &args, uint64_t *d_lanes, uint64_t *h_dst_mapped, uint32_t *h_flag_mapped, uint32_t seq, hipStream_t stream);
hipError_t launch_gather_to_tables(const uint4 *recv, uint4 *tabs, uint32_t G, uint32_t U, uint32_t per, hipStream_t stream);
hipError_t launch_msg_accumulate(const FrHost *in, FrHost *acc, int D, bool first, bool last, FrHost *d_out, uint64_t *d_out_wide, FrHost *h_out_mapped,
                                 uint32_t *h_flag_mapped, uint32_t seq, hipStream_t stream);
hipError_t launch_f29_to_sat(const uint4 *src, const int32_t *src_top, uint4 *dst, uint64_t n, hipStream_t stream);
hipError_t launch_fr_elementwise(int op, const uint4 *a, const uint4 *b, const FrHost &u, uint4 *out, uint64_t n, hipStream_t stream);
hipError_t launch_bench_modmul(uint64_t n_threads, uint32_t reps, uint32_t variant, uint64_t *d_sink, hipStream_t stream);

}
```

sumcheck_amd/csrc/kernels_big.hip:

```cpp
#include "kernel_common.hpp"
#include "finalize_device.hpp"
#include "load_factor.hpp"

#include <algorithm>
#include <cstdlib>
#include <cstring>

namespace scd {

#ifdef SC_EXPERIMENTS
template <int M>
__global__ __launch_bounds__(kBlock) void k_prod_round(const ProdArgs A, const FrHost r_h, const uint64_t n_pairs,
                                                       uint4 *__restrict__ partials) {
    __shared__ uint32_t sm[kBlock / 64][8];
    const FrU r = fru_from_host(r_h);
    Fr acc[M + 1];
#pragma unroll
    for (int t = 0; t <= M; ++t) acc[t] = fr_zero();

    const uint64_t stride = (uint64_t)gridDim.x * kBlock;
    for (uint64_t b = (uint64_t)blockIdx.x * kBlock + threadIdx.x; b < n_pairs; b += stride) {
        Fr prod[M + 1];
        bool first = true;
        for (int s = 0; s < A.n_slots; ++s) {
            Fr lo, hi;
            if (A.slot[s].mode == 0) {
                const uint4 *p = A.slot[s].src + 4 * b;
                lo = fr_load(p);
                hi = fr_load(p + 2);
            } else {
                const uint4 *p = A.slot[s].src + 8 * b;
                const Fr e0 = fr_load(p), e1 = fr_load(p + 2), e2 = fr_load(p + 4), e3 = fr_load(p + 6);
                Fr ml, mh;
                fr_mul2_comba_u(fr_sub(e1, e0), r, fr_sub(e3, e2), r, ml, mh);
                lo = fr_add(e0, ml);
                hi = fr_add(e2, mh);
                uint4 *q = A.slot[s].dst + 4 * b;
                fr_store(q, lo);
                fr_store(q + 2, hi);
            }
            const Fr step = fr_sub(hi, lo);
            const uint32_t e = A.slot[s].exp;
            Fr curP = hi, curN = lo;
            Fr cur[M + 1];
#pragma unroll
            for (int t = 0; t <= M; ++t) {
                const int32_t nv = node_value(t);
                if (nv == 0) cur[t] = lo;
                else if (nv == 1) cur[t] = hi;
                else if (nv == kNodeInf) cur[t] = step;
                else if (nv < 0) { curN = fr_sub(curN, step); cur[t] = curN; }
                else { curP = fr_add(curP, step); cur[t] = curP; }
            }
            uint32_t k = 0;
            if (first) {
#pragma unroll
                for (int t = 0; t <= M; ++t) prod[t] = cur[t];
                k = 1;
            }
            for (; k < e; ++k) {
#pragma unroll
                for (int t = 0; t + 1 <= M; t += 2) fr_mul2_comba(prod[t], cur[t], prod[t + 1], cur[t + 1], prod[t], prod[t + 1]);
                if ((M + 1) % 2 == 1) prod[M] = fr_mul(prod[M], cur[M]);
            }
            first = false;
        }
#pragma unroll
        for (int t = 0; t <= M; ++t) acc[t] = fr_add(acc[t], prod[t]);
    }
#pragma unroll
    for (int t = 0; t <= M; ++t) {
        const Fr s = block_sum(acc[t], sm);
        if (threadIdx.x == 0) fr_store(partials + 2 * ((uint64_t)t * gridDim.x + blockIdx.x), s);
    }
}

#endif

template <int M>
__global__ __launch_bounds__(kBlock) void k_prod_round_fe(const ProdArgs A, const FrHost r32_h, const uint64_t n_pairs,
                                                          uint4 *__restrict__ partials) {
    __shared__ uint32_t sm[kBlock / 64][8];
    const FeU r = feu_from_host(r32_h);
    Fe acc[M + 1];
#pragma unroll
    for (int t = 0; t <= M; ++t) acc[t] = fe_zero();

    const uint64_t stride = (uint64_t)gridDim.x * kBlock;
    uint32_t iter = 0;
    for (uint64_t b = (uint64_t)blockIdx.x * kBlock + threadIdx.x; b < n_pairs; b += stride, ++iter) {
        Fe prod[M + 1];
        bool first = true;
        for (int s = 0; s < A.n_slots; ++s) {
            Fe lo, hi;
            if (A.slot[s].mode == 0) {
                const uint4 *p = A.slot[s].src + 4 * b;
                lo = fe_from_fr(fr_load(p));
                hi = fe_from_fr(fr_load(p + 2));
            } else {
                const uint4 *p = A.slot[s].src + 8 * b;
                const Fe e0 = fe_from_fr(fr_load(p)), e1 = fe_from_fr(fr_load(p + 2));
                const Fe e2 = fe_from_fr(fr_load(p + 4)), e3 = fe_from_fr(fr_load(p + 6));
                const Fe l0 = fe_add(e0, fe_mul_u(fe_sub(e1, e0), r));
                const Fe h0 = fe_add(e2, fe_mul_u(fe_sub(e3, e2), r));
                const Fr lc = fe_to_fr(l0), hc = fe_to_fr(h0);
                uint4 *q = A.slot[s].dst + 4 * b;
                fr_store(q, lc);
                fr_store(q + 2, hc);
                lo = fe_from_fr(lc);
                hi = fe_from_fr(hc);
            }
            const Fe step = fe_sub(hi, lo);
            const uint32_t e = A.slot[s].exp;
            Fe curP = hi, curN = lo;
#pragma unroll
            for (int t = 0; t <= M; ++t) {
                const int32_t nv = node_value(t);
                Fe cur;
                if (nv == 0) cur = lo;
                else if (nv == 1) cur = hi;
                else if (nv == kNodeInf) cur = step;
                else if (nv < 0) {
                    curN = (nv == -1) ? fe_sub(curN, step) : fe_sub(fe_carry_pass(curN), step);
                    cur = curN;
                } else {
                    curP = (nv == 2) ? fe_add(curP, step) : fe_add(fe_carry_pass(curP), step);
                    cur = curP;
                }
                uint32_t k = 0;
                if (first) { prod[t] = (nv == 0 || nv == 1) ? cur : fe_carry_pass(cur); k = 1; }
                for (; k < e; ++k) prod[t] = fe_mul(cur, prod[t]);
            }
            first = false;
        }
#pragma unroll
        for (int t = 0; t <= M; ++t) acc[t] = fe_carry_pass(fe_add(acc[t], prod[t]));
        if ((iter & 31u) == 31u) {
#pragma unroll
            for (int t = 0; t <= M; ++t) acc[t] = fe_from_fr(fe_to_fr(acc[t]));
        }
    }
#pragma unroll
    for (int t = 0; t <= M; ++t) {
        const Fr s = block_sum(fe_to_fr(acc[t]), sm);
        if (threadIdx.x == 0) fr_store(partials + 2 * ((uint64_t)t * gridDim.x + blockIdx.x), s);
    }
}

template <int M, bool kR1 = false, bool kChain = kChainDefault, bool kSkip1 = false>
__device__ __forceinline__ void tree_pass(const Slot *S, const int32_t (&r)[kBindLds], const uint64_t n_pairs, uint4 *__restrict__ row, uint32_t (*sm)[8],
                                          int32_t *lacc, const uint32_t part_stride = 0) {
    const uint64_t pstride = part_stride ? part_stride : gridDim.x;
    static_assert(!(kSkip1 && kR1), "round 1 has no previous round to take node 1 from");
    int32_t *my = lacc + threadIdx.x;
#pragma unroll
    for (int i = 0; i < 9 * (M + 1); ++i) my[i * kBlock] = 0;
    const uint64_t stride = (uint64_t)gridDim.x * kBlock;
    uint32_t iter = 0;
    uint64_t b = (uint64_t)blockIdx.x * kBlock + threadIdx.x;
#ifdef SC_M4_PAIRS
    constexpr bool kM4Pairs = true;
#else
    constexpr bool kM4Pairs = kR1;
#endif
    if constexpr (M == 2 || M == 3 || (M == 4 && kM4Pairs)) {
        for (; b + stride < n_pairs; b += 2 * stride, ++iter) {
            Fe P[M + 1];
            const uint64_t b2 = b + stride;
            [[maybe_unused]] auto accumulate = [&](const int t, const Fe &v) {
                Fe acc;
#pragma unroll
                for (int l = 0; l < 9; ++l) acc.l[l] = my[(9 * t + l) * kBlock];
                acc = fe_add(acc, v);
                if (iter & 1u) acc = fe_carry_pass(acc);
                if ((iter & 31u) == 31u) acc = fe_from_fr(fe_to_fr(acc));
#pragma unroll
                for (int l = 0; l < 9; ++l) my[(9 * t + l) * kBlock] = acc.l[l];
            };
            if constexpr (M == 4) {
                Fe a0, a1, ai, b0, b1, bi, c0, c1, ci, d0, d1, di;
                {
                    Fe l0, h0, l1, h1;
                    LoadFactor<0, kR1, kChain>::run(S, b, r, l0, h0);
                    LoadFactor<1, kR1, kChain>::run(S, b, r, l1, h1);
                    a0 = fe_mul<kChain>(l0, l1);
                    a1 = fe_mul<kChain>(h0, h1);
                    ai = fe_mul<kChain>(fe_sub(h0, l0), fe_sub(h1, l1));
                }
                fe_pin3(a0, a1, ai);
                {
                    Fe l2, h2, l3, h3;
                    LoadFactor<2, kR1, kChain>::run(S, b, r, l2, h2);
                    LoadFactor<3, kR1, kChain>::run(S, b, r, l3, h3);
                    b0 = fe_mul<kChain>(l2, l3);
                    b1 = fe_mul<kChain>(h2, h3);
                    bi = fe_mul<kChain>(fe_sub(h2, l2), fe_sub(h3, l3));
                }
                fe_pin3(b0, b1, bi);
                {
                    Fe l0, h0, l1, h1;
                    LoadFactor<0, kR1, kChain>::run(S, b2, r, l0, h0);
                    LoadFactor<1, kR1, kChain>::run(S, b2, r, l1, h1);
                    c0 = fe_mul<kChain>(l0, l1);
                    c1 = fe_mul<kChain>(h0, h1);
                    ci = fe_mul<kChain>(fe_sub(h0, l0), fe_sub(h1, l1));
                }
                fe_pin3(c0, c1, ci);
                {
                    Fe l2, h2, l3, h3;
                    LoadFactor<2, kR1, kChain>::run(S, b2, r, l2, h2);
                    LoadFactor<3, kR1, kChain>::run(S, b2, r, l3, h3);
                    d0 = fe_mul<kChain>(l2, l3);
                    d1 = fe_mul<kChain>(h2, h3);
                    di = fe_mul<kChain>(fe_sub(h2, l2), fe_sub(h3, l3));
                }
                accumulate(0, fe_mul2_sum<kChain>(a0, b0, c0, d0));
                if constexpr (!kSkip1) accumulate(1, fe_mul2_sum<kChain>(a1, b1, c1, d1));
                accumulate(2, fe_mul2_sum<kChain>(ai, bi, ci, di));
                auto extend = [](Fe &q0, Fe &q1, const Fe &qi) {
                    const Fe t = fe_add(qi, qi);
                    const Fe m1 = fe_carry_pass(fe_sub(fe_add(t, fe_add(q0, q0)), q1));
                    const Fe p2 = fe_carry_pass(fe_sub(fe_add(t, fe_add(q1, q1)), q0));
                    q0 = m1;
                    q1 = p2;
                };
                extend(a0, a1, ai);
                extend(b0, b1, bi);
                extend(c0, c1, ci);
                extend(d0, d1, di);
                fe_pin3(a0, b0, c0);
                fe_pin3(a1, b1, c1);
                accumulate(3, fe_mul2_sum<kChain>(a0, b0, c0, d0));
                accumulate(4, fe_mul2_sum<kChain>(a1, b1, c1, d1));
                continue;
            } else if constexpr (M == 2) {
                Fe l0, h0, l1, h1, m0, k0, m1, k1;
                LoadFactor<0, kR1, kChain>::run(S, b, r, l0, h0);
                LoadFactor<1, kR1, kChain>::run(S, b, r, l1, h1);
                LoadFactor<0, kR1, kChain>::run(S, b2, r, m0, k0);
                LoadFactor<1, kR1, kChain>::run(S, b2, r, m1, k1);
                P[0] = fe_mul2_sum<kChain>(l0, l1, m0, m1);
                if constexpr (!kSkip1) P[1] = fe_mul2_sum<kChain>(h0, h1, k0, k1);
                P[2] = fe_mul2_sum<kChain>(fe_sub(h0, l0), fe_sub(h1, l1), fe_sub(k0, m0), fe_sub(k1, m1));
            } else {
                Fe q0, q1, qi, l2, h2;
                {
                    Fe l0, h0, l1, h1;
                    LoadFactor<0, kR1, kChain>::run(S, b, r, l0, h0);
                    LoadFactor<1, kR1, kChain>::run(S, b, r, l1, h1);
                    q0 = fe_mul<kChain>(l0, l1);
                    q1 = fe_mul<kChain>(h0, h1);
                    qi = fe_mul<kChain>(fe_sub(h0, l0), fe_sub(h1, l1));
                }
                fe_pin3(q0, q1, qi);
                LoadFactor<2, kR1, kChain>::run(S, b, r, l2, h2);
                Fe s0, s1, si, m2, k2;
                {
                    Fe l0, h0, l1, h1;
                    LoadFactor<0, kR1, kChain>::run(S, b2, r, l0, h0);
                    LoadFactor<1, kR1, kChain>::run(S, b2, r, l1, h1);
                    s0 = fe_mul<kChain>(l0, l1);
                    s1 = fe_mul<kChain>(h0, h1);
                    si = fe_mul<kChain>(fe_sub(h0, l0), fe_sub(h1, l1));
                }
                fe_pin3(s0, s1, si);
                LoadFactor<2, kR1, kChain>::run(S, b2, r, m2, k2);
                P[0] = fe_mul2_sum<kChain>(l2, q0, m2, s0);
                if constexpr (!kSkip1) P[1] = fe_mul2_sum<kChain>(h2, q1, k2, s1);
                P[2] = fe_mul2_sum<kChain>(fe_sub(h2, l2), qi, fe_sub(k2, m2), si);
                const Fe qm1 = fe_carry_pass(fe_sub(fe_add(fe_add(qi, qi), fe_add(q0, q0)), q1));
                const Fe sm1 = fe_carry_pass(fe_sub(fe_add(fe_add(si, si), fe_add(s0, s0)), s1));
                P[3] = fe_mul2_sum<kChain>(fe_carry_pass(fe_sub(fe_add(l2, l2), h2)), qm1, fe_carry_pass(fe_sub(fe_add(m2, m2), k2)), sm1);
            }
#pragma unroll
            for (int t = 0; t <= M; ++t) {
                if (kSkip1 && t == 1) continue;
                Fe a;
#pragma unroll
                for (int l = 0; l < 9; ++l) a.l[l] = my[(9 * t + l) * kBlock];
                a = fe_add(a, P[t]);
                if (iter & 1u) a = fe_carry_pass(a);
                if ((iter & 31u) == 31u) a = fe_from_fr(fe_to_fr(a));
#pragma unroll
                for (int l = 0; l < 9; ++l) my[(9 * t + l) * kBlock] = a.l[l];
            }
        }
    }
    for (; b < n_pairs; b += stride, ++iter) {
        Fe P[M + 1];
        if constexpr (M == 1) {
            LoadFactor<0, kR1, kChain>::run(S, b, r, P[0], P[1]);
        } else if constexpr (M == 2) {
            Fe l0, h0, l1, h1;
            LoadFactor<0, kR1, kChain>::run(S, b, r, l0, h0);
            LoadFactor<1, kR1, kChain>::run(S, b, r, l1, h1);
            P[0] = fe_mul<kChain>(l0, l1);
            if constexpr (!kSkip1) P[1] = fe_mul<kChain>(h0, h1);
            P[2] = fe_mul<kChain>(fe_sub(h0, l0), fe_sub(h1, l1));
        } else if constexpr (M == 3) {
            Fe q0, q1, qi;
            {
                Fe l0, h0, l1, h1;
                LoadFactor<0, kR1, kChain>::run(S, b, r, l0, h0);
                LoadFactor<1, kR1, kChain>::run(S, b, r, l1, h1);
                q0 = fe_mul<kChain>(l0, l1);
                q1 = fe_mul<kChain>(h0, h1);
                qi = fe_mul<kChain>(fe_sub(h0, l0), fe_sub(h1, l1));
            }
            fe_pin3(q0, q1, qi);
            const Fe qm1 = fe_carry_pass(fe_sub(fe_add(fe_add(qi, qi), fe_add(q0, q0)), q1));
            Fe l2, h2;
            LoadFactor<2, kR1, kChain>::run(S, b, r, l2, h2);
            P[0] = fe_mul<kChain>(l2, q0);
            if constexpr (!kSkip1) P[1] = fe_mul<kChain>(h2, q1);
            P[2] = fe_mul<kChain>(fe_sub(h2, l2), qi);
            P[3] = fe_mul<kChain>(fe_sub(fe_add(l2, l2), h2), qm1);
        } else {
            static_assert(M == 4, "the tree kernels take products of at most four multiplicands");
            Fe a0, a1, ai, b0, b1, bi;
            {
                Fe l0, h0, l1, h1;
                LoadFactor<0, kR1, kChain>::run(S, b, r, l0, h0);
                LoadFactor<1, kR1, kChain>::run(S, b, r, l1, h1);
                a0 = fe_mul<kChain>(l0, l1);
                a1 = fe_mul<kChain>(h0, h1);
                ai = fe_mul<kChain>(fe_sub(h0, l0), fe_sub(h1, l1));
            }
            fe_pin3(a0, a1, ai);
            {
                Fe l2, h2, l3, h3;
                LoadFactor<2, kR1, kChain>::run(S, b, r, l2, h2);
                LoadFactor<3, kR1, kChain>::run(S, b, r, l3, h3);
                b0 = fe_mul<kChain>(l2, l3);
                b1 = fe_mul<kChain>(h2, h3);
                bi = fe_mul<kChain>(fe_sub(h2, l2), fe_sub(h3, l3));
            }
            const Fe a2i = fe_add(ai, ai), b2i = fe_add(bi, bi);
            P[0] = fe_mul<kChain>(a0, b0);
            if constexpr (!kSkip1) P[1] = fe_mul<kChain>(a1, b1);
            P[2] = fe_mul<kChain>(ai, bi);
            P[3] = fe_mul<kChain>(fe_carry_pass(fe_sub(fe_add(a2i, fe_add(a0, a0)), a1)), fe_carry_pass(fe_sub(fe_add(b2i, fe_add(b0, b0)), b1)));
            P[4] = fe_mul<kChain>(fe_carry_pass(fe_sub(fe_add(a2i, fe_add(a1, a1)), a0)), fe_carry_pass(fe_sub(fe_add(b2i, fe_add(b1, b1)), b0)));
        }
#pragma unroll
        for (int t = 0; t <= M; ++t) {
            if (kSkip1 && t == 1) continue;
            Fe a;
#pragma unroll
            for (int l = 0; l < 9; ++l) a.l[l] = my[(9 * t + l) * kBlock];
            a = fe_add(a, P[t]);
            if (iter & 1u) a = fe_carry_pass(a);
            if ((iter & 31u) == 31u) a = fe_from_fr(fe_to_fr(a));
#pragma unroll
            for (int l = 0; l < 9; ++l) my[(9 * t + l) * kBlock] = a.l[l];
        }
    }
#ifndef SC_SERIAL_EPILOGUE
    (void)sm;
    Fr s[M + 1];
#pragma unroll
    for (int t = 0; t <= M; ++t) {
        if (kSkip1 && t == 1) { s[t] = fr_zero(); continue; }
        Fe a;
#pragma unroll
        for (int l = 0; l < 9; ++l) a.l[l] = my[(9 * t + l) * kBlock];
        s[t] = fe_to_fr(a);
    }
#pragma unroll
    for (int off = 32; off >= 1; off >>= 1) {
#pragma unroll
        for (int t = 0; t <= M; ++t)
            if (!(kSkip1 && t == 1)) s[t] = fr_add(s[t], fr_shfl_down(s[t], off));
    }
    const int lane = threadIdx.x & 63, wave = threadIdx.x >> 6;
    uint32_t *x = reinterpret_cast<uint32_t *>(lacc);
    __syncthreads();
    if (lane == 0) {
#pragma unroll
        for (int t = 0; t <= M; ++t)
#pragma unroll
            for (int i = 0; i < 8; ++i) x[(wave * (M + 1) + t) * 8 + i] = s[t].v[i];
    }
    __syncthreads();
    if (threadIdx.x <= (uint32_t)M && !(kSkip1 && threadIdx.x == 1)) {
        const int t = threadIdx.x;
        Fr acc;
#pragma unroll
        for (int i = 0; i < 8; ++i) acc.v[i] = x[t * 8 + i];
        for (int w = 1; w < kBlock / 64; ++w) {
            Fr o;
#pragma unroll
            for (int i = 0; i < 8; ++i) o.v[i] = x[(w * (M + 1) + t) * 8 + i];
            acc = fr_add(acc, o);
        }
        fr_store(row + 2 * ((uint64_t)t * pstride), acc);
    }
    __syncthreads();
#else
#pragma unroll
    for (int t = 0; t <= M; ++t) {
        if (kSkip1 && t == 1) continue;
        Fe a;
#pragma unroll
        for (int l = 0; l < 9; ++l) a.l[l] = my[(9 * t + l) * kBlock];
        const Fr s = block_sum(fe_to_fr(a), sm);
        if (threadIdx.x == 0) fr_store(row + 2 * ((uint64_t)t * pstride), s);
    }
#endif
}

template <int M>
__global__ __launch_bounds__(kBlock) void k_prod_tree(const ProdArgs A, const BindConst r, const uint64_t n_pairs,
                                                      uint4 *__restrict__ partials) {
    __shared__ uint32_t sm[kBlock / 64][8];
    __shared__ int32_t rt[kBindLds];
    __shared__ int32_t lacc[9 * (M + 1) * kBlock];
    bind_consts_to_lds(r, rt);
    tree_pass<M>(A.slot, rt, n_pairs, partials + 2 * (uint64_t)blockIdx.x, sm, lacc);
}

#ifdef SC_EXPERIMENTS
constexpr int kTilePairs = 64;

template <int M>
__global__ __launch_bounds__(64 * (M + 1)) void k_round_tile(const ProdArgs A, const FrHost r32_h, const uint64_t n_pairs,
                                                             uint4 *__restrict__ partials) {
    constexpr int kThreads = 64 * (M + 1);
    constexpr int kEnt = 2 * kTilePairs;
    __shared__ int32_t lds[M * 9 * kEnt];
    const FeU r = feu_from_host(r32_h);
    const int tid = threadIdx.x;
    const int node_idx = tid >> 6;
    const int lane = tid & 63;
    const int32_t nv = node_value(node_idx);
    const int n_slots = A.n_slots;
    Fe acc = fe_zero();
    const uint64_t n_tiles = (n_pairs + kTilePairs - 1) / kTilePairs;
    uint32_t iter = 0;
    for (uint64_t tile = blockIdx.x; tile < n_tiles; tile += gridDim.x, ++iter) {
        const uint64_t b0 = tile * kTilePairs;
        const uint64_t ent_left = 2 * (n_pairs - b0);
        for (int item = tid; item < n_slots * kEnt; item += kThreads) {
            const int s = item / kEnt, i = item % kEnt;
            Fe v = fe_zero();
            if ((uint64_t)i < ent_left) {
                if (A.slot[s].mode == 0) {
                    v = fe_from_fr(fr_load(A.slot[s].src + 2 * (2 * b0 + i)));
                } else {
                    const uint4 *p = A.slot[s].src + 4 * (2 * b0 + i);
                    const Fe e0 = fe_from_fr(fr_load(p)), e1 = fe_from_fr(fr_load(p + 2));
                    const Fr c = fe_to_fr(fe_add(e0, fe_mul_u(fe_sub(e1, e0), r)));
                    fr_store(A.slot[s].dst + 2 * (2 * b0 + i), c);
                    v = fe_from_fr(c);
                }
            }
            int32_t *row = lds + (s * 9) * kEnt + i;
#pragma unroll
            for (int l = 0; l < 9; ++l) row[l * kEnt] = v.l[l];
        }
        __syncthreads();
        {
            Fe prod;
            bool first = true;
            for (int s = 0; s < n_slots; ++s) {
                Fe lo, hi;
                const int32_t *row = lds + (s * 9) * kEnt + 2 * lane;
#pragma unroll
                for (int l = 0; l < 9; ++l) {
                    const int2 w = *reinterpret_cast<const int2 *>(row + l * kEnt);
                    lo.l[l] = w.x;
                    hi.l[l] = w.y;
                }
                Fe val;
                if (nv == 0) val = lo;
                else if (nv == 1) val = hi;
                else if (nv == kNodeInf) val = fe_sub(hi, lo);
                else if (nv == -1) val = fe_sub(fe_add(lo, lo), hi);
                else if (nv == 2) val = fe_sub(fe_add(hi, hi), lo);
                else {
                    const Fe step = fe_sub(hi, lo);
                    if (nv > 0) {
                        val = fe_sub(fe_add(hi, hi), lo);
                        for (int32_t c = 2; c < nv; ++c) val = fe_add(fe_carry_pass(val), step);
                    } else {
                        val = fe_sub(fe_add(lo, lo), hi);
                        for (int32_t c = -1; c > nv; --c) val = fe_sub(fe_carry_pass(val), step);
                    }
                }
                uint32_t k = 0;
                if (first) { prod = (nv == 0 || nv == 1) ? val : fe_carry_pass(val); k = 1; first = false; }
                for (; k < A.slot[s].exp; ++k) prod = fe_mul(val, prod);
            }
            if (b0 + lane < n_pairs) acc = fe_carry_pass(fe_add(acc, prod));
            if ((iter & 31u) == 31u) acc = fe_from_fr(fe_to_fr(acc));
        }
        __syncthreads();
    }
    Fr sum = fe_to_fr(acc);
#pragma unroll
    for (int off = 32; off >= 1; off >>= 1) sum = fr_add(sum, fr_shfl_down(sum, off));
    if (lane == 0) fr_store(partials + 2 * ((uint64_t)node_idx * gridDim.x + blockIdx.x), sum);
}

#endif

#ifdef SC_EXPERIMENTS
constexpr int kFinGroup = 32;
__global__ __launch_bounds__(kBlock, 3) void k_round_tree(const RoundArgs R, const BindConst r, const uint64_t n_pairs,
                                                       uint4 *__restrict__ partials) {
    __shared__ uint32_t sm[kBlock / 64][8];
    __shared__ int32_t rt[kBindLds];
    __shared__ int32_t lacc[9 * 5 * kBlock];
#ifdef SC_EXPERIMENTS
    __shared__ uint32_t role_sh;
#endif
    bind_consts_to_lds(r, rt);
    const int n = R.n_prod;
    int k = (int)((blockIdx.x & 7u) % (uint32_t)n);
    for (int i = 0; i < n; ++i) {
        const TreeProd &T = R.prod[k];
        uint4 *row = partials + 2 * (T.partial_off + (uint64_t)blockIdx.x);
        switch (T.M) {
        case 1: tree_pass<1>(T.slot, rt, n_pairs, row, sm, lacc); break;
        case 2: tree_pass<2>(T.slot, rt, n_pairs, row, sm, lacc); break;
        case 3: tree_pass<3>(T.slot, rt, n_pairs, row, sm, lacc); break;
        default: tree_pass<4>(T.slot, rt, n_pairs, row, sm, lacc); break;
        }
        if (++k == n) k = 0;
    }
#ifdef SC_EXPERIMENTS
    if (!R.fin.enabled) return;
    const uint32_t G = gridDim.x, n_groups = (G + kFinGroup - 1) / kFinGroup;
    const uint32_t g = blockIdx.x / kFinGroup, g_first = g * kFinGroup, g_size = min((uint32_t)kFinGroup, G - g_first);
    __syncthreads();
    if (threadIdx.x == 0) {
        __builtin_amdgcn_fence(__ATOMIC_RELEASE, "agent");
        const uint32_t d = __hip_atomic_fetch_add(R.fin.counters + 1 + g, 1u, __ATOMIC_RELAXED, __HIP_MEMORY_SCOPE_AGENT);
        role_sh = d == g_size - 1 ? 1u : 0u;
        if (role_sh) __builtin_amdgcn_fence(__ATOMIC_ACQUIRE, "agent");
    }
    __syncthreads();
    if (!role_sh) return;
    {
        int n_items = 0;
        for (int q = 0; q < n; ++q) n_items += (int)R.prod[q].M + 1;
        for (int it0 = 0; it0 < 4 * n_items; it0 += kBlock) {
            const int it = it0 + (int)threadIdx.x;
            const bool live = it < 4 * n_items;
            int c = live ? it >> 2 : 0, q4 = it & 3, pk = 0;
            while (c > (int)R.prod[pk].M) { c -= (int)R.prod[pk].M + 1; ++pk; }
            const uint4 *base = partials + 2 * (R.prod[pk].partial_off + (uint64_t)c * G + g_first);
            Fr acc = fr_zero();
            if (live)
                for (uint32_t b = (uint32_t)q4 * 8; b < min((uint32_t)q4 * 8 + 8, g_size); ++b) acc = fr_add(acc, fr_load(base + 2 * b));
            acc = fr_add(acc, fr_shfl_down(acc, 2));
            acc = fr_add(acc, fr_shfl_down(acc, 1));
            if (live && q4 == 0) fr_store(R.fin.partials2 + 2 * (R.prod[pk].partial_off + (uint64_t)c * n_groups + g), acc);
        }
    }
    __syncthreads();
    if (threadIdx.x == 0) {
        __builtin_amdgcn_fence(__ATOMIC_RELEASE, "agent");
        const uint32_t d = __hip_atomic_fetch_add(R.fin.counters, 1u, __ATOMIC_RELAXED, __HIP_MEMORY_SCOPE_AGENT);
        role_sh = d == n_groups - 1 ? 2u : 0u;
        if (role_sh) __builtin_amdgcn_fence(__ATOMIC_ACQUIRE, "agent");
    }
    __syncthreads();
    if (role_sh != 2u) return;
    for (uint32_t i = threadIdx.x; i <= n_groups; i += kBlock)
        __hip_atomic_store(R.fin.counters + i, 0u, __ATOMIC_RELAXED, __HIP_MEMORY_SCOPE_AGENT);
    auto prod_of = [&](int q) -> FinProd {
        FinProd f;
        f.M = R.prod[q].M;
        f.pad = 0;
        f.partial_off = R.prod[q].partial_off;
        f.w_off = R.fin.w_off[q];
        return f;
    };
    finalize_body<kBlock>(prod_of, R.fin.Wm, n, R.fin.D, (int)n_groups, R.fin.partials2, reinterpret_cast<uint4 *>(lacc), R.fin.out, R.fin.out_wide,
                          R.fin.h_out, R.fin.h_flag, R.fin.seq, 1);
#endif
}
#endif

__global__ __launch_bounds__(kBlock, 3) void k_round1_tree_split(const RoundArgs R, const uint64_t n_pairs, uint4 *__restrict__ partials) {
    __shared__ uint32_t sm[kBlock / 64][8];
    __shared__ int32_t rt[kBindLds];
    __shared__ int32_t lacc[9 * 5 * kBlock];
    const TreeProd &T = R.prod[blockIdx.y];
    uint4 *row = partials + 2 * (T.partial_off + (uint64_t)R.part_block0 + (uint64_t)blockIdx.x);
#ifdef SC_NO_CHAIN_R1
    constexpr bool kC1 = false;
#else
    constexpr bool kC1 = true;
#endif
    switch (T.M) {
    case 1: tree_pass<1, true, kC1>(T.slot, rt, n_pairs, row, sm, lacc, R.part_stride); break;
    case 2: tree_pass<2, true, kC1>(T.slot, rt, n_pairs, row, sm, lacc, R.part_stride); break;
    case 3: tree_pass<3, true, kC1>(T.slot, rt, n_pairs, row, sm, lacc, R.part_stride); break;
    default: tree_pass<4, true, kC1>(T.slot, rt, n_pairs, row, sm, lacc, R.part_stride); break;
    }
}
template <bool kChain, bool kSkip1>
__global__ __launch_bounds__(kBlock, 3) void k_round_tree_split(const RoundArgs R, const BindConst r, const uint64_t n_pairs, uint4 *__restrict__ partials) {
    __shared__ uint32_t sm[kBlock / 64][8];
    __shared__ int32_t rt[kBindLds];
    __shared__ int32_t lacc[9 * 5 * kBlock];
    bind_consts_to_lds(r, rt);
    const TreeProd &T = R.prod[blockIdx.y];
    uint4 *row = partials + 2 * (T.partial_off + (uint64_t)blockIdx.x);
    switch (T.M) {
    case 1: tree_pass<1, false, kChain, kSkip1>(T.slot, rt, n_pairs, row, sm, lacc); break;
    case 2: tree_pass<2, false, kChain, kSkip1>(T.slot, rt, n_pairs, row, sm, lacc); break;
    case 3: tree_pass<3, false, kChain, kSkip1>(T.slot, rt, n_pairs, row, sm, lacc); break;
    default: tree_pass<4, false, kChain, kSkip1>(T.slot, rt, n_pairs, row, sm, lacc); break;
    }
}

#ifdef SC_EXPERIMENTS
__global__ __launch_bounds__(kBlock, 3) void k_round1_tree(const RoundArgs R, const uint64_t n_pairs, uint4 *__restrict__ partials) {
    __shared__ uint32_t sm[kBlock / 64][8];
    __shared__ int32_t rt[kBindLds];
    __shared__ int32_t lacc[9 * 5 * kBlock];
    const int n = R.n_prod;
    int k = (int)((blockIdx.x & 7u) % (uint32_t)n);
    for (int i = 0; i < n; ++i) {
        const TreeProd &T = R.prod[k];
        uint4 *row = partials + 2 * (T.partial_off + (uint64_t)blockIdx.x);
        switch (T.M) {
        case 1: tree_pass<1, true>(T.slot, rt, n_pairs, row, sm, lacc); break;
        case 2: tree_pass<2, true>(T.slot, rt, n_pairs, row, sm, lacc); break;
        case 3: tree_pass<3, true>(T.slot, rt, n_pairs, row, sm, lacc); break;
        default: tree_pass<4, true>(T.slot, rt, n_pairs, row, sm, lacc); break;
        }
        if (++k == n) k = 0;
    }
}
#endif

#ifdef SC_EXPERIMENTS
template <int M>
static hipError_t launch_prod_round_t(const ProdArgs &args, const FrHost &r, uint64_t n_pairs, FrHost *d_partials, int grid,
                                      hipStream_t stream) {
    hipLaunchKernelGGL(k_prod_round<M>, dim3(grid), dim3(kBlock), 0, stream, args, r, n_pairs, (uint4 *)d_partials);
    return hipGetLastError();
}

#endif

template <int M>
static hipError_t launch_prod_round_fe_t(const ProdArgs &args, const FrHost &r32, uint64_t n_pairs, FrHost *d_partials, int grid,
                                         hipStream_t stream) {
    hipLaunchKernelGGL(k_prod_round_fe<M>, dim3(grid), dim3(kBlock), 0, stream, args, r32, n_pairs, (uint4 *)d_partials);
    return hipGetLastError();
}

hipError_t launch_prod_round_fe(int M, const ProdArgs &args, const FrHost &r32, uint64_t n_pairs, FrHost *d_partials, int grid,
                                hipStream_t stream) {
    switch (M) {
    case 1: return launch_prod_round_fe_t<1>(args, r32, n_pairs, d_partials, grid, stream);
    case 2: return launch_prod_round_fe_t<2>(args, r32, n_pairs, d_partials, grid, stream);
    case 3: return launch_prod_round_fe_t<3>(args, r32, n_pairs, d_partials, grid, stream);
    case 4: return launch_prod_round_fe_t<4>(args, r32, n_pairs, d_partials, grid, stream);
    case 5: return launch_prod_round_fe_t<5>(args, r32, n_pairs, d_partials, grid, stream);
    case 6: return launch_prod_round_fe_t<6>(args, r32, n_pairs, d_partials, grid, stream);
    case 7: return launch_prod_round_fe_t<7>(args, r32, n_pairs, d_partials, grid, stream);
    case 8: return launch_prod_round_fe_t<8>(args, r32, n_pairs, d_partials, grid, stream);
    default: return hipErrorInvalidValue;
    }
}

template <int M>
static hipError_t launch_prod_tree_t(const ProdArgs &args, const BindConst &r32, uint64_t n_pairs, FrHost *d_partials, int grid,
                                     hipStream_t stream) {
    hipLaunchKernelGGL(k_prod_tree<M>, dim3(grid), dim3(kBlock), 0, stream, args, r32, n_pairs, (uint4 *)d_partials);
    return hipGetLastError();
}

hipError_t launch_prod_tree(int M, const ProdArgs &args, const BindConst &r32, uint64_t n_pairs, FrHost *d_partials, int grid,
                            hipStream_t stream) {
    switch (M) {
    case 1: return launch_prod_tree_t<1>(args, r32, n_pairs, d_partials, grid, stream);
    case 2: return launch_prod_tree_t<2>(args, r32, n_pairs, d_partials, grid, stream);
    case 3: return launch_prod_tree_t<3>(args, r32, n_pairs, d_partials, grid, stream);
    case 4: return launch_prod_tree_t<4>(args, r32, n_pairs, d_partials, grid, stream);
    default: return launch_prod_tree_wide(M, args, r32, n_pairs, d_partials, grid, stream);
    }
}

hipError_t launch_round_tree(const RoundArgs &args, const BindConst &r32, uint64_t n_pairs, FrHost *d_partials, int grid, hipStream_t stream, bool split,
                             bool skip1) {
    size_t extra_lds = 0;
#ifdef SC_EXPERIMENTS
    static const size_t env_lds = [] {
        const char *e = std::getenv("SC_EXTRA_LDS");
        return e ? (size_t)std::strtoul(e, nullptr, 10) : (size_t)0;
    }();
    extra_lds = env_lds;
#endif
    bool round1 = args.fin.enabled == 0;
    for (int q = 0; q < args.n_prod && round1; ++q)
        for (uint32_t f = 0; f < args.prod[q].M; ++f) round1 = round1 && args.prod[q].slot[f].mode == 0 && args.prod[q].slot[f].src_top == nullptr;
#ifdef SC_EXPERIMENTS
    if (!split) {
        if (skip1) return hipErrorInvalidValue;
        if (round1 && extra_lds == 0) hipLaunchKernelGGL(k_round1_tree, dim3(grid), dim3(kBlock), 0, stream, args, n_pairs, (uint4 *)d_partials);
        else hipLaunchKernelGGL(k_round_tree, dim3(grid), dim3(kBlock), extra_lds, stream, args, r32, n_pairs, (uint4 *)d_partials);
        return hipGetLastError();
    }
#else
    (void)split;
    (void)extra_lds;
#endif
#ifdef SC_NO_CHAIN_R2
    bool canonical_sources = false;
#else
    bool canonical_sources = !round1;
#endif
    for (int q = 0; q < args.n_prod && canonical_sources; ++q)
        for (uint32_t f = 0; f < args.prod[q].M; ++f) canonical_sources = canonical_sources && args.prod[q].slot[f].src_top == nullptr;
    const dim3 g(grid, args.n_prod), b(kBlock);
    uint4 *const part = (uint4 *)d_partials;
    plan_hit(round1 ? kPlanBigMergedRound1 : canonical_sources ? kPlanBigMergedBindChain : kPlanBigMergedBind);
    if (skip1) plan_hit(kPlanBigClaimIdentity);
    if (round1) {
        if (skip1) return hipErrorInvalidValue;
        hipLaunchKernelGGL(k_round1_tree_split, g, b, 0, stream, args, n_pairs, part);
    } else if (canonical_sources) {
        if (skip1) hipLaunchKernelGGL((k_round_tree_split<true, true>), g, b, 0, stream, args, r32, n_pairs, part);
        else hipLaunchKernelGGL((k_round_tree_split<true, false>), g, b, 0, stream, args, r32, n_pairs, part);
    } else {
        if (skip1) hipLaunchKernelGGL((k_round_tree_split<kChainDefault, true>), g, b, 0, stream, args, r32, n_pairs, part);
        else hipLaunchKernelGGL((k_round_tree_split<kChainDefault, false>), g, b, 0, stream, args, r32, n_pairs, part);
    }
    return hipGetLastError();
}

#ifdef SC_EXPERIMENTS
template <int M>
static hipError_t launch_round_tile_t(const ProdArgs &args, const FrHost &r32, uint64_t n_pairs, FrHost *d_partials, int grid,
                                      hipStream_t stream) {
    hipLaunchKernelGGL(k_round_tile<M>, dim3(grid), dim3(64 * (M + 1)), 0, stream, args, r32, n_pairs, (uint4 *)d_partials);
    return hipGetLastError();
}

int grid_for_tiles(uint64_t n_pairs) {
    uint64_t g = (n_pairs + kTilePairs - 1) / kTilePairs;
    if (g < 1) g = 1;
    if (g > (uint64_t)kMaxGrid) g = kMaxGrid;
    return (int)g;
}

hipError_t launch_round_tile(int M, const ProdArgs &args, const FrHost &r32, uint64_t n_pairs, FrHost *d_partials, int grid,
                             hipStream_t stream) {
    switch (M) {
    case 1: return launch_round_tile_t<1>(args, r32, n_pairs, d_partials, grid, stream);
    case 2: return launch_round_tile_t<2>(args, r32, n_pairs, d_partials, grid, stream);
    case 3: return launch_round_tile_t<3>(args, r32, n_pairs, d_partials, grid, stream);
    case 4: return launch_round_tile_t<4>(args, r32, n_pairs, d_partials, grid, stream);
    case 5: return launch_round_tile_t<5>(args, r32, n_pairs, d_partials, grid, stream);
    case 6: return launch_round_tile_t<6>(args, r32, n_pairs, d_partials, grid, stream);
    case 7: return launch_round_tile_t<7>(args, r32, n_pairs, d_partials, grid, stream);
    case 8: return launch_round_tile_t<8>(args, r32, n_pairs, d_partials, grid, stream);
    default: return hipErrorInvalidValue;
    }
}

hipError_t launch_prod_round(int M, const ProdArgs &args, const FrHost &r, uint64_t n_pairs, FrHost *d_partials, int grid,
                             hipStream_t stream) {
    switch (M) {
    case 1: return launch_prod_round_t<1>(args, r, n_pairs, d_partials, grid, stream);
    case 2: return launch_prod_round_t<2>(args, r, n_pairs, d_partials, grid, stream);
    case 3: return launch_prod_round_t<3>(args, r, n_pairs, d_partials, grid, stream);
    case 4: return launch_prod_round_t<4>(args, r, n_pairs, d_partials, grid, stream);
    case 5: return launch_prod_round_t<5>(args, r, n_pairs, d_partials, grid, stream);
    case 6: return launch_prod_round_t<6>(args, r, n_pairs, d_partials, grid, stream);
    case 7: return launch_prod_round_t<7>(args, r, n_pairs, d_partials, grid, stream);
    case 8: return launch_prod_round_t<8>(args, r, n_pairs, d_partials, grid, stream);
    default: return hipErrorInvalidValue;
    }
}

#endif

}
```

sumcheck_amd/csrc/protocol.hip:

```cpp
#include "prover_internal.hpp"

uint64_t small_pairs_limit() {
#ifdef SC_EXPERIMENTS
    static const uint64_t v = [] {
        const char *e = std::getenv("SC_SMALL_LOG2");
        return e ? (1ULL << std::atoi(e)) : scd::kSmallRoundPairs;
    }();
    return v;
#else
    return scd::kSmallRoundPairs;
#endif
}

bool launches_are_async(sc_prover *p) {
    static const bool ok = [p] {
        uint32_t *h = nullptr, *d = nullptr;
        FrHost *dm = nullptr;
        if (hipHostMalloc(reinterpret_cast<void **>(&h), 256, hipHostMallocMapped | hipHostMallocCoherent) != hipSuccess) return false;
        bool good = hipHostGetDevicePointer(reinterpret_cast<void **>(&d), h, 0) == hipSuccess &&
                    hipMalloc(reinterpret_cast<void **>(&dm), sizeof(FrHost)) == hipSuccess;
        if (good) {
            std::memset(h, 0, 256);
            good = scd::launch_wait_challenge(d, 0xffffffffu, reinterpret_cast<const FrHost *>(d + 16), dm, p->stream, 1) == hipSuccess &&
                   hipStreamSynchronize(p->stream) == hipSuccess;
// ... 120 lines not shown
    if (r_or_null) {
        std::memcpy(&r, r_or_null, 32);
        if (sch::geq_p(r)) return sc_internal_fail(SC_ERR_BAD_ARG, "challenge is not a canonical field element");
    }
    HIP_TRY(hipSetDevice(p->device));
    int rc_t = collect_timing(p);
    if (rc_t) return rc_t;
    const bool bind = r_or_null != nullptr;
    if (bind) p->randomness.push_back(r);
    p->round += 1;
    scd::BindConst rc;
    std::memset(&rc, 0, sizeof(rc));
    if (bind) make_bind_const(r, rc);
    const uint64_t C = 1ULL << p->chunk_log2, n = 1ULL << p->nv, n_chunks = n / C;
    const uint64_t pairs_per_chunk = bind ? C / 4 : C / 2;
    const bool merged = p->merge_rounds && !p->any_generic;
    const int grid = merged ? std::min(scd::grid_for_pairs(pairs_per_chunk), scd::kRoundTreeGrid) : scd::grid_for_pairs(pairs_per_chunk);
    sch::Fr r32v = sch::zero();
    const FrHost r32 = to_dev(r32v);
    p->seq += 1;
    for (uint64_t c = 0; c < n_chunks; ++c) {
        const int q = (int)(c & 1);
        if (c >= 2) HIP_TRY(hipStreamWaitEvent(p->copy_stream, p->ev_consumed[q], 0));
        for (uint32_t u = 0; u < p->U; ++u)
            HIP_TRY(hipMemcpyAsync(static_cast<char *>(p->ring[q]) + (((size_t)u << p->chunk_log2) * 32), p->host_tabs[u] + 4 * c * C, C * 32, hipMemcpyHostToDevice,
                                   p->copy_stream));
        HIP_TRY(hipEventRecord(p->ev_copied[q], p->copy_stream));
        HIP_TRY(hipStreamWaitEvent(p->stream, p->ev_copied[q], 0));
        auto ring_tab = [&](uint32_t u) { return reinterpret_cast<const uint4 *>(static_cast<char *>(p->ring[q]) + (((size_t)u << p->chunk_log2) * 32)); };
        if (merged) {
            scd::RoundArgs ra;
            std::memset(&ra, 0, sizeof(ra));
            ra.n_prod = (int)p->K;
            std::vector<uint8_t> bound(p->U, 0);
            for (uint32_t k = 0; k < p->K; ++k) {
                const Product &pr = p->prods[k];
                scd::TreeProd &tp = ra.prod[k];
                tp.M = pr.M;
                tp.partial_off = pr.partial_off;
                int f = 0;
                for (size_t s = 0; s < pr.tables.size(); ++s) {
                    const uint32_t u = pr.tables[s];
                    Table &t = p->tabs[u];
                    for (uint32_t rep = 0; rep < pr.exps[s]; ++rep, ++f) {
                        scd::Slot &sl = tp.slot[f];
                        sl.exp = 1;
                        sl.src = ring_tab(u);
                        sl.src_top = nullptr;
                        if (!bind) {
                            sl.mode = 0;
                        } else if (!bound[u]) {
                            sl.mode = 1;
                            sl.dst = t.buf[0] + 2 * (c * (C / 2));
                            sl.dst_top = p->use_f29 ? t.buf_top[0] + c * (C / 2) : nullptr;
                            bound[u] = 1;
                        } else {
                            sl.mode = 3;
                            sl.dst_top = p->use_f29 ? t.buf_top[0] : nullptr;
                        }
                    }
                }
            }
            HIP_TRY(scd::launch_round_tree(ra, rc, pairs_per_chunk, p->d_partials, grid, p->stream, true));
            if (bind) {
                for (uint32_t u = 0; u < p->U; ++u)
                    if (!bound[u]) HIP_TRY(scd::launch_fix(ring_tab(u), p->tabs[u].buf[0] + 2 * (c * (C / 2)), to_dev(r), C / 2, p->stream));
            }
        } else {
            std::vector<const uint4 *> src(p->U);
            for (uint32_t u = 0; u < p->U; ++u) {
                if (bind) {
                    uint4 *dst = p->tabs[u].buf[0] + 2 * (c * (C / 2));
                    HIP_TRY(scd::launch_fix(ring_tab(u), dst, to_dev(r), C / 2, p->stream));
                    src[u] = dst;
                } else {
                    src[u] = ring_tab(u);
                }
            }
            bool ptrs_uploaded = false;
            for (uint32_t k = 0; k < p->K; ++k) {
                const Product &pr = p->prods[k];
                FrHost *partials = p->d_partials + pr.partial_off;
                ProdArgs a;
                std::memset(&a, 0, sizeof(a));
                if (pr.fused && p->kernel_variant == 3 && pr.M <= 4) {
                    a.n_slots = (int)pr.M;
                    int f = 0;
                    for (size_t s2 = 0; s2 < pr.tables.size(); ++s2)
                        for (uint32_t rep = 0; rep < pr.exps[s2]; ++rep, ++f) {
                            a.slot[f].exp = 1;
                            a.slot[f].mode = 0;
                            a.slot[f].src = src[pr.tables[s2]];
                        }
                    HIP_TRY(scd::launch_prod_tree((int)pr.M, a, rc, pairs_per_chunk, partials, grid, p->stream));
                } else if (pr.fused) {
                    a.n_slots = (int)pr.tables.size();
                    for (size_t s2 = 0; s2 < pr.tables.size(); ++s2) {
                        a.slot[s2].exp = pr.exps[s2];
                        a.slot[s2].mode = 0;
                        a.slot[s2].src = src[pr.tables[s2]];
                    }
                    HIP_TRY(scd::launch_prod_round_fe((int)pr.M, a, r32, pairs_per_chunk, partials, grid, p->stream));
                } else {
                    if (!ptrs_uploaded) {
                        const uint4 **h = p->h_cur_tables + (size_t)q * p->U;
                        if (c >= 2) HIP_TRY(hipEventSynchronize(p->ev_consumed[q]));
                        for (uint32_t u = 0; u < p->U; ++u) h[u] = src[u];
                        HIP_TRY(hipMemcpyAsync(p->d_cur_tables + (size_t)q * p->U, h, p->U * sizeof(void *), hipMemcpyHostToDevice, p->stream));
                        ptrs_uploaded = true;
                    }
                    HIP_TRY(scd::launch_sum_generic(p->d_cur_tables + (size_t)q * p->U, p->d_slot_table + pr.slot_off, p->d_slot_exp + pr.slot_off, (int)pr.tables.size(),
                                                    (int)pr.M, pairs_per_chunk, partials, grid, p->stream));
                }
            }
        }
        HIP_TRY(scd::launch_finalize(p->d_finprods, p->h_finprods.empty() ? nullptr : p->h_finprods.data(), p->d_W, (int)p->K, (int)p->D, grid, p->d_partials,
                                     p->d_scratch, p->d_chunk_msg, nullptr, nullptr, nullptr, 0, 1, p->d_fin_mb_counter, p->stream));
        const bool last = c + 1 == n_chunks;
        HIP_TRY(scd::launch_msg_accumulate(p->d_chunk_msg, p->d_chunk_msg + p->D, (int)p->D, c == 0, last, p->d_out, last ? d_wide : nullptr,
                                           (last && publish_to_host) ? p->h_out_dev : nullptr, (last && publish_to_host) ? p->h_flag_dev : nullptr, p->seq, p->stream));
        HIP_TRY(hipEventRecord(p->ev_consumed[q], p->stream));
    }
    if (bind) {
        for (uint32_t u = 0; u < p->U; ++u) {
            Table &t = p->tabs[u];
            bool referenced = false;
            for (const Product &pr : p->prods)
                for (uint32_t tt : pr.tables) referenced |= tt == u;
            t.cur = t.buf[0];
            t.cur_top = (merged && p->use_f29 && referenced) ? t.buf_top[0] : nullptr;
            t.next = 1;
        }
    }
    p->timed = false;
    p->timing_pending = false;
    return SC_OK;
}

struct SlowCallProbe {
    const char *what;
    std::chrono::steady_clock::time_point t0;
    bool on;
    explicit SlowCallProbe(const char *w) : what(w), on(std::getenv("SC_HOST_TRACE") != nullptr) {
        if (on) t0 = std::chrono::steady_clock::now();
    }
    ~SlowCallProbe() {
        if (!on) return;
        const double ms = std::chrono::duration<double, std::milli>(std::chrono::steady_clock::now() - t0).count();
        if (ms > 1.0) std::fprintf(stderr, "[sc] slow host call: %s took %.1f ms\n", what, ms);
    }
};
bool fin_mb_enabled();
bool staged_init_applies(const sc_prover *p) {
    return scd::policy(scd::kPolStagedInit) != 0 && p->merge_rounds && !p->any_generic && !p->streamed && !p->borrow && !p->fused_finalize && p->kernel_variant == 3 &&
           p->nv >= 18 && p->K > 0 && p->K <= (uint32_t)scd::kMetaProds;
}
int staged_copy_and_round1(sc_prover *p, const uint64_t *const *host_tables) {
    HIP_TRY(hipSetDevice(p->device));
    if (!p->copy_stream) HIP_TRY(hipStreamCreateWithFlags(&p->copy_stream, hipStreamNonBlocking));
    if (!p->copy_stream2) HIP_TRY(hipStreamCreateWithFlags(&p->copy_stream2, hipStreamNonBlocking));
    for (int q = 0; q < 2; ++q) {
        if (!p->ev_copied[q]) HIP_TRY(hipEventCreateWithFlags(&p->ev_copied[q], hipEventDisableTiming));
        if (!p->ev_copied2[q]) HIP_TRY(hipEventCreateWithFlags(&p->ev_copied2[q], hipEventDisableTiming));
    }
    const uint64_t n = 1ULL << p->nv, n_pairs = n >> 1;
    int G = n_pairs >= (1ULL << 21) ? 1024 : n_pairs >= (1ULL << 20) ? 768 : n_pairs >= (1ULL << 18) ? 384 : n_pairs >= (1ULL << 17) ? 256 : 192;
    if (p->K == 1) G = std::min(G, scd::kRoundTreeGrid);
    G = std::min(G, scd::grid_for_pairs(n_pairs));
    int levels = p->nv >= 21 ? 5 : 2;
    int sec[6], n_chunks = levels + 1;
    if (levels == 5 && G % 8 == 0) {
        sec[0] = G / 4, sec[1] = G / 8, sec[2] = G / 8;
        sec[3] = G / 8, sec[4] = G / 8, sec[5] = G / 4;
    } else {
        levels = 2;
        while (levels > 0 && (G % (1 << levels)) != 0) --levels;
        n_chunks = levels + 1;
        for (int c = 0; c < n_chunks; ++c) sec[c] = G >> (c < levels ? c + 1 : levels);
    }
    for (uint32_t u = 0; u < p->U; ++u)
        if (!host_tables[u]) return sc_internal_fail(SC_ERR_BAD_ARG, "table %u is null", u);
    scd::BindConst rc;
    std::memset(&rc, 0, sizeof(rc));
    HIP_TRY(hipEventRecord(p->ev_copied[1], p->stream));
    HIP_TRY(hipStreamWaitEvent(p->copy_stream, p->ev_copied[1], 0));
    HIP_TRY(hipStreamWaitEvent(p->copy_stream2, p->ev_copied[1], 0));
    int block0 = 0;
    for (int c = 0; c < n_chunks; ++c) {
        const int sh = c < levels ? c + 1 : levels;
        const uint64_t chunk = n >> sh, first = n - (n >> c);
        const int gc = sec[c];
        for (uint32_t u = 0; u < p->U; ++u) {
            HIP_TRY(hipMemcpyAsync(reinterpret_cast<char *>(p->tabs[u].buf[0]) + (size_t)first * 32, reinterpret_cast<const char *>(host_tables[u]) + (size_t)first * 32,
                                   (size_t)chunk * 32, hipMemcpyHostToDevice, (u & 1) ? p->copy_stream2 : p->copy_stream));
        }
        HIP_TRY(hipEventRecord(p->ev_copied[c & 1], p->copy_stream));
        HIP_TRY(hipStreamWaitEvent(p->stream, p->ev_copied[c & 1], 0));
        if (p->U > 1) {
            HIP_TRY(hipEventRecord(p->ev_copied2[c & 1], p->copy_stream2));
            HIP_TRY(hipStreamWaitEvent(p->stream, p->ev_copied2[c & 1], 0));
        }
        scd::RoundArgs ra;
        std::memset(&ra, 0, sizeof(ra));
        ra.n_prod = (int)p->K;
        for (uint32_t k = 0; k < p->K; ++k) {
            const Product &pr = p->prods[k];
            scd::TreeProd &tp = ra.prod[k];
            tp.M = pr.M;
            tp.partial_off = pr.partial_off;
            int f = 0;
            for (size_t s2 = 0; s2 < pr.tables.size(); ++s2)
                for (uint32_t rep = 0; rep < pr.exps[s2]; ++rep, ++f) {
                    tp.slot[f].exp = 1;
                    tp.slot[f].mode = 0;
                    tp.slot[f].src = p->tabs[pr.tables[s2]].buf[0] + 2 * (size_t)first;
                }
        }
        ra.part_stride = (uint32_t)G;
        ra.part_block0 = (uint32_t)block0;
        HIP_TRY(scd::launch_round_tree(ra, rc, chunk >> 1, p->d_partials, gc, p->stream, true, false));
        block0 += gc;
    }
    if (block0 != G) return sc_internal_fail(SC_ERR_HIP, "staged initialisation: the sections do not cover the grid");
    scd::plan_hit(scd::kPlanBigStagedRound1);
    const bool keeps = scd::finalize_keeps_sums((int)p->K, (int)p->D, G, !p->h_finprods.empty(), fin_mb_enabled());
    HIP_TRY(scd::launch_finalize(p->d_finprods, p->h_finprods.data(), p->d_W, (int)p->K, (int)p->D, G, p->d_partials, keeps ? p->d_sums[1] : p->d_scratch, p->d_out, nullptr,
                                 p->h_out_dev, p->h_flag_dev, p->seq + 1, 1, fin_mb_enabled() ? p->d_fin_mb_counter : nullptr, p->stream, nullptr));
    p->r1_cached = true;
    p->r1_keeps = keeps;
    return SC_OK;
}

int launch_round(sc_prover *p, const uint64_t *r_or_null, uint64_t *d_wide, bool publish_to_host, bool deferred) {
    if (p->res.active) {
        int rc_q = resident_quiesce(p);
        if (rc_q) return rc_q;
    }
    DeviceGate gate(p->device);
    if (p->streamed && p->round < 2 && !p->exhausted) {
        if (deferred) return sc_internal_fail(SC_ERR_BAD_ARG, "streamed tables: rounds 1 and 2 are not pipelined");
        return launch_round_streamed(p, r_or_null, d_wide, publish_to_host);
    }
    if (p->exhausted) return sc_internal_fail(SC_ERR_NOT_ACTIVE, "Prover is not active");
    if (p->deferred_pending) return sc_internal_fail(SC_ERR_BAD_ARG, "a pipelined round is waiting for its challenge");
    if (r_or_null && p->round == 0) return sc_internal_fail(SC_ERR_FIRST_ROUND_HAS_MSG, "first round should be prover first.");
    if (!r_or_null && p->round > 0 && !deferred) return sc_internal_fail(SC_ERR_MISSING_MSG, "verifier message is empty");
    if (p->round + 1 > p->nv) return sc_internal_fail(SC_ERR_NOT_ACTIVE, "Prover is not active");
    sch::Fr r = sch::zero();
    if (r_or_null) {
        std::memcpy(&r, r_or_null, 32);
        if (sch::geq_p(r)) return sc_internal_fail(SC_ERR_BAD_ARG, "challenge is not a canonical field element");
    }
    if (deferred) {
        const uint64_t np = 1ULL << (p->nv - (p->round + 1));
        if (!(np <= small_pairs_limit() && p->U <= (uint32_t)scd::kMaxSmallTables && p->K > 0)) return sc_internal_fail(SC_ERR_BAD_ARG, "only late rounds are pipelined");
    }
    HIP_TRY(hipSetDevice(p->device));
    if (!deferred) {
        int rc_t = collect_timing(p);
        if (rc_t) return rc_t;
    }
    if (p->r1_cached) {
        p->r1_cached = false;
        if (p->round == 0 && !r_or_null && !deferred && !d_wide && publish_to_host) {
            p->round = 1;
            p->seq += 1;
            p->sums_round = p->r1_keeps ? 1 : -1;
            p->timed = false;
            p->timing_pending = false;
            p->prod_timed = false;
            return SC_OK;
        }
    }
    bool bind = r_or_null != nullptr || deferred;
    if (r_or_null) p->randomness.push_back(r);
    p->round += 1;
    const uint64_t n_pairs = 1ULL << (p->nv - p->round);
    const FrHost rdev = to_dev(r);
    sch::Fr r32v = r;
    for (int d = 0; d < 5; ++d) r32v = sch::add(r32v, r32v);
    const FrHost r32 = to_dev(r32v);
    int scaled = 0;
    const uint64_t small_pairs = small_pairs_limit();
    const bool small_round = n_pairs <= small_pairs && p->K > 0 && (p->U <= (uint32_t)scd::kMaxSmallTables || p->d_cur_tables != nullptr);
#ifdef SC_EXPERIMENTS
    const bool tiled = !small_round && !p->any_generic && p->kernel_variant == 2;
#else
    const bool tiled = false;
    (void)tiled;
#endif
    scd::BindConst rc;
    std::memset(&rc, 0, sizeof(rc));
    if (bind && !small_round && p->kernel_variant == 3) make_bind_const(r, rc);
    int grid = scd::grid_for_pairs(n_pairs);
#ifdef SC_EXPERIMENTS
    if (tiled) grid = scd::grid_for_tiles(n_pairs);
#endif
    const bool timed = p->timing && !deferred;
    if (timed) HIP_TRY(hipEventRecord(p->ev0, p->stream));
    const FrHost *r_mail = nullptr;
    if (deferred) {
        p->sig_seq += 1;
        {
            SlowCallProbe pr("launch k_wait_challenge");
            HIP_TRY(scd::launch_wait_challenge(p->sig_dev, p->sig_seq, p->h_mail_dev + (p->sig_seq & 1u), p->d_mail + (p->sig_seq & 1u), p->stream));
        }
        r_mail = p->d_mail + (p->sig_seq & 1u);
        p->deferred_pending = true;
    }

    auto bind_table = [&](uint32_t u) -> hipError_t {
        Table &t = p->tabs[u];
        uint4 *dst = t.buf[t.next];
        hipError_t e = scd::launch_fix(t.cur, dst, rdev, 2 * n_pairs, p->stream);
        t.cur = dst;
        t.next ^= 1;
        return e;
    };

    const bool small = small_round;
    if (small) {
        TablePtrs tp;
        if (bind) {
            for (uint32_t u0 = 0; u0 < p->U; u0 += (uint32_t)scd::kMaxSmallTables) {
                const uint32_t cnt = std::min<uint32_t>(p->U - u0, (uint32_t)scd::kMaxSmallTables);
                std::memset(&tp, 0, sizeof(tp));
                for (uint32_t j = 0; j < cnt; ++j) {
                    Table &t = p->tabs[u0 + j];
                    tp.src[j] = t.cur;
                    tp.src_top[j] = t.cur_top;
                    tp.dst[j] = t.buf[t.next];
                }
                {
                    SlowCallProbe pr("launch k_fix_multi");
                    HIP_TRY(scd::launch_fix_multi(tp, (int)cnt, rdev, r_mail, 2 * n_pairs, p->stream));
                }
                for (uint32_t j = 0; j < cnt; ++j) {
                    Table &t = p->tabs[u0 + j];
                    t.cur = t.buf[t.next];
                    t.cur_top = nullptr;
                    t.next ^= 1;
                }
            }
        }
        SlowCallProbe pr_sum("launch k_sum_combos");
        scd::plan_hit(deferred ? scd::kPlanSmallPipelined : p->U > (uint32_t)scd::kMaxSmallTables ? scd::kPlanSmallPtrs : p->has_meta ? scd::kPlanSmallLaunched : scd::kPlanSmallCombosTable);
        if (p->U <= (uint32_t)scd::kMaxSmallTables) {
            std::memset(&tp, 0, sizeof(tp));
            for (uint32_t u = 0; u < p->U; ++u) tp.src[u] = p->tabs[u].cur;
            if (p->has_meta) HIP_TRY(scd::launch_sum_combos_meta(tp, p->meta, p->n_combos, n_pairs, p->d_partials, grid, p->stream));
            else HIP_TRY(scd::launch_sum_combos(tp, p->d_combos, p->n_combos, p->d_slot_table, p->d_slot_exp, n_pairs, p->d_partials, grid, p->stream));
        } else {
            for (uint32_t u = 0; u < p->U; ++u) p->h_cur_tables[u] = p->tabs[u].cur;
            HIP_TRY(hipMemcpyAsync(p->d_cur_tables, p->h_cur_tables, p->U * sizeof(void *), hipMemcpyHostToDevice, p->stream));
            HIP_TRY(scd::launch_sum_combos_ptrs(p->d_cur_tables, p->d_combos, p->n_combos, p->d_slot_table, p->d_slot_exp, n_pairs, p->d_partials, grid, p->stream));
        }
        scaled = 1;
        bind = false;
    }
    if (bind && p->any_generic) {
        scd::plan_hit(scd::kPlanBigBindPass);
        for (uint32_t u0 = 0; u0 < p->U; u0 += (uint32_t)scd::kMaxSmallTables) {
            const uint32_t cnt = std::min<uint32_t>(p->U - u0, (uint32_t)scd::kMaxSmallTables);
            TablePtrs tp;
            std::memset(&tp, 0, sizeof(tp));
            for (uint32_t j = 0; j < cnt; ++j) {
                Table &t = p->tabs[u0 + j];
                tp.src[j] = t.cur;
                tp.src_top[j] = t.cur_top;
                tp.dst[j] = t.buf[t.next];
            }
            HIP_TRY(scd::launch_fix_multi(tp, (int)cnt, rdev, nullptr, 2 * n_pairs, p->stream));
            for (uint32_t j = 0; j < cnt; ++j) {
                Table &t = p->tabs[u0 + j];
                t.cur = t.buf[t.next];
                t.cur_top = nullptr;
                t.next ^= 1;
            }
        }
        bind = false;
    }
    std::vector<uint8_t> bound(p->U, 0);
    bool ptrs_uploaded = false;
    bool finalized = false;
    bool skip1 = false;
    const bool merged = !small && p->merge_rounds && !p->any_generic;
    if (merged) {
        grid = std::min(grid, scd::kRoundTreeGrid);
        bool split = !p->fused_finalize;
        int split_grid = n_pairs >= (1ULL << 21) ? 1024 : n_pairs >= (1ULL << 20) ? 768 : n_pairs >= (1ULL << 18) ? 384 : n_pairs >= (1ULL << 17) ? 256 : 192;
#ifdef SC_EXPERIMENTS
        static const bool split_off = std::getenv("SC_SPLIT") && std::atoi(std::getenv("SC_SPLIT")) == 0;
        static const int split_cap = std::getenv("SC_SPLIT_GRID") ? std::atoi(std::getenv("SC_SPLIT_GRID")) : 0;
        if (split_off) split = false;
        if (split_cap > 0) split_grid = split_cap;
#endif
#ifndef SC_NO_KGRID
        if (p->K < 4 && n_pairs < (1ULL << 21)) split_grid = std::min(scd::kMaxGrid, split_grid * 4 / (int)p->K);
        else if (p->K == 1) split_grid = std::min(split_grid, scd::kRoundTreeGrid);
#else
        if (p->K == 1) split_grid = std::min(split_grid, scd::kRoundTreeGrid);
#endif
        if (split) grid = std::min(scd::grid_for_pairs(n_pairs), split_grid);
        skip1 = bind && split && p->sums_round == (int64_t)p->round - 1 && skip1_enabled() &&
                scd::finalize_keeps_sums((int)p->K, (int)p->D, grid, !p->h_finprods.empty(), fin_mb_enabled());
        scd::RoundArgs ra;
        std::memset(&ra, 0, sizeof(ra));
        ra.n_prod = (int)p->K;
        std::vector<const uint4 *> old_src(p->U);
        std::vector<const int32_t *> old_top(p->U);
        for (uint32_t u = 0; u < p->U; ++u) {
            old_src[u] = p->tabs[u].cur;
            old_top[u] = p->tabs[u].cur_top;
        }
        for (uint32_t k = 0; k < p->K; ++k) {
            const Product &pr = p->prods[k];
            scd::TreeProd &tp = ra.prod[k];
            tp.M = pr.M;
            tp.partial_off = pr.partial_off;
            int f = 0;
            for (size_t s = 0; s < pr.tables.size(); ++s) {
                const uint32_t u = pr.tables[s];
                Table &t = p->tabs[u];
                for (uint32_t rep = 0; rep < pr.exps[s]; ++rep, ++f) {
                    scd::Slot &sl = tp.slot[f];
                    sl.exp = 1;
                    sl.src = old_src[u];
                    sl.src_top = old_top[u];
                    if (!bind) {
                        sl.mode = 0;
                    } else if (!bound[u]) {
                        sl.mode = 1;
                        sl.dst = t.buf[t.next];
                        sl.dst_top = p->use_f29 ? t.buf_top[t.next] : nullptr;
                        t.cur = t.buf[t.next];
                        t.cur_top = sl.dst_top;
                        t.next ^= 1;
                        bound[u] = 1;
                    } else {
                        sl.mode = 3;
                        sl.dst_top = p->use_f29 ? t.buf_top[0] : nullptr;
                    }
                }
            }
        }
        p->seq += 1;
        ra.fin.enabled = p->fused_finalize ? 1 : 0;
        ra.fin.D = (int)p->D;
        for (uint32_t k = 0; k < p->K; ++k) ra.fin.w_off[k] = p->h_finprods[k].w_off;
        ra.fin.Wm = reinterpret_cast<const uint4 *>(p->d_W);
        ra.fin.partials2 = reinterpret_cast<uint4 *>(p->d_partials2);
        ra.fin.counters = p->d_fin_counters;
        ra.fin.out = reinterpret_cast<uint4 *>(p->d_out);
        ra.fin.out_wide = d_wide;
        ra.fin.h_out = publish_to_host ? reinterpret_cast<uint4 *>(p->h_out_dev) : nullptr;
        ra.fin.h_flag = publish_to_host ? p->h_flag_dev : nullptr;
        ra.fin.seq = p->seq;
        if (p->timing) HIP_TRY(hipEventRecord(p->prod_ev[0], p->stream));
        if (bind) scd::plan_hit(p->use_f29 ? scd::kPlanBigF29Store : scd::kPlanBigCanonicalStore);
        HIP_TRY(scd::launch_round_tree(ra, rc, n_pairs, p->d_partials, grid, p->stream, split, skip1));
        if (p->timing) HIP_TRY(hipEventRecord(p->prod_ev[1], p->stream));
        scaled = 1;
        if (p->fused_finalize) finalized = true;
        else p->seq -= 1;
    }
    for (uint32_t k = 0; k < p->K && !small && !merged; ++k) {
        const Product &pr = p->prods[k];
        FrHost *partials = p->d_partials + pr.partial_off;
        if (p->timing) HIP_TRY(hipEventRecord(p->prod_ev[2 * k], p->stream));
        if (pr.fused && p->kernel_variant == 3 && (pr.M <= 4 || p->wide_tree)) {
            ProdArgs a;
            std::memset(&a, 0, sizeof(a));
            a.n_slots = (int)pr.M;
            int f = 0;
            for (size_t s = 0; s < pr.tables.size(); ++s) {
                Table &t = p->tabs[pr.tables[s]];
                const uint4 *old_src = t.cur;
                const int32_t *old_top = t.cur_top;
                bool stored_here = false;
                for (uint32_t rep = 0; rep < pr.exps[s]; ++rep, ++f) {
                    a.slot[f].exp = 1;
                    if (bind && !bound[pr.tables[s]]) {
                        a.slot[f].mode = 1;
                        a.slot[f].src = old_src;
                        a.slot[f].src_top = old_top;
                        a.slot[f].dst = t.buf[t.next];
                        a.slot[f].dst_top = p->use_f29 ? t.buf_top[t.next] : nullptr;
                        t.cur = t.buf[t.next];
                        t.cur_top = a.slot[f].dst_top;
                        t.next ^= 1;
                        bound[pr.tables[s]] = 1;
                        stored_here = true;
                    } else if (stored_here) {
                        a.slot[f].mode = 3;
                        a.slot[f].src = old_src;
                        a.slot[f].src_top = old_top;
                        a.slot[f].dst = nullptr;
                        a.slot[f].dst_top = p->use_f29 ? t.buf_top[0] : nullptr;
                    } else {
                        a.slot[f].mode = 0;
                        a.slot[f].src = t.cur;
                        a.slot[f].src_top = t.cur_top;
                        a.slot[f].dst = nullptr;
                    }
                }
            }
            scd::plan_hit(pr.M <= 4 ? scd::kPlanBigPerProductTree : scd::kPlanBigWide);
            if (bind) scd::plan_hit(p->use_f29 ? scd::kPlanBigF29Store : scd::kPlanBigCanonicalStore);
            HIP_TRY(scd::launch_prod_tree((int)pr.M, a, rc, n_pairs, partials, grid, p->stream));
            scaled = 1;
        } else if (pr.fused) {
            ProdArgs a;
            std::memset(&a, 0, sizeof(a));
            a.n_slots = (int)pr.tables.size();
            for (size_t s = 0; s < pr.tables.size(); ++s) {
                Table &t = p->tabs[pr.tables[s]];
                a.slot[s].exp = pr.exps[s];
                if (bind && !bound[pr.tables[s]]) {
                    a.slot[s].mode = 1;
                    a.slot[s].src = t.cur;
                    a.slot[s].dst = t.buf[t.next];
                    t.cur = t.buf[t.next];
                    t.next ^= 1;
                    bound[pr.tables[s]] = 1;
                } else {
                    a.slot[s].mode = 0;
                    a.slot[s].src = t.cur;
                    a.slot[s].dst = nullptr;
                }
            }
#ifdef SC_EXPERIMENTS
            if (tiled) {
                HIP_TRY(scd::launch_round_tile((int)pr.M, a, r32, n_pairs, partials, grid, p->stream));
                scaled = 1;
            } else if (!p->use_fe) {
                HIP_TRY(scd::launch_prod_round((int)pr.M, a, rdev, n_pairs, partials, grid, p->stream));
            } else
#endif
            {
                scd::plan_hit(scd::kPlanBigNodeByNode);
                HIP_TRY(scd::launch_prod_round_fe((int)pr.M, a, r32, n_pairs, partials, grid, p->stream));
                scaled = 1;
            }
        } else if (pr.M <= (uint32_t)scd::kMaxWideM && p->wide_tree && p->kernel_variant == 3) {
            scd::WideArgs16 a;
            std::memset(&a, 0, sizeof(a));
            const std::vector<uint32_t> &factors = p->prod_indices[k];
            a.n_slots = (int)factors.size();
            for (size_t f = 0; f < factors.size(); ++f) {
                const Table &t = p->tabs[factors[f]];
                a.slot[f].mode = 0;
                a.slot[f].exp = 1;
                a.slot[f].src = t.cur;
                a.slot[f].src_top = t.cur_top;
            }
            sch::Fr comp = sch::kOne;
            for (uint32_t dbl = 0; dbl < 5 * (pr.M - 1); ++dbl) comp = sch::add(comp, comp);
            scd::plan_hit(scd::kPlanBigWide16);
            HIP_TRY(scd::launch_prod_tree_wide16((int)pr.M, a, to_dev(comp), n_pairs, partials, grid, p->stream));
        } else {
            if (!ptrs_uploaded) {
                for (uint32_t u = 0; u < p->U; ++u) p->h_cur_tables[u] = p->tabs[u].cur;
                HIP_TRY(hipMemcpyAsync(p->d_cur_tables, p->h_cur_tables, p->U * sizeof(void *), hipMemcpyHostToDevice, p->stream));
                ptrs_uploaded = true;
            }
            scd::plan_hit(scd::kPlanBigGeneric);
            HIP_TRY(scd::launch_sum_generic(p->d_cur_tables, p->d_slot_table + pr.slot_off, p->d_slot_exp + pr.slot_off,
                                            (int)pr.tables.size(), (int)pr.M, n_pairs, partials, grid, p->stream));
        }
        if (p->timing) HIP_TRY(hipEventRecord(p->prod_ev[2 * k + 1], p->stream));
    }
    if (bind) {
        for (uint32_t u = 0; u < p->U; ++u)
            if (!bound[u]) HIP_TRY(bind_table(u));
    }
    if (!finalized) {
    p->seq += 1;
    const bool keeps = scd::finalize_keeps_sums((int)p->K, (int)p->D, grid, !p->h_finprods.empty(), fin_mb_enabled());
    scd::ClaimArgs ca;
    std::memset(&ca, 0, sizeof(ca));
    if (skip1) {
        ca.skip1 = 1;
        ca.prev = reinterpret_cast<const uint4 *>(p->d_sums[(p->round - 1) & 1]);
        bool done[5] = {false, false, false, false, false};
        for (uint32_t k = 0; k < p->K; ++k) {
            const uint32_t M = p->prods[k].M;
            if (done[M]) continue;
            done[M] = true;
            sch::Fr lam[5];
            claim_weights(M, r, lam);
            for (uint32_t s2 = 0; s2 <= M; ++s2) ca.lam[scd::claim_off((int)M) + (int)s2] = to_dev(lam[s2]);
        }
    }
    SlowCallProbe pr_fin("launch k_finalize");
    HIP_TRY(scd::launch_finalize(p->d_finprods, p->h_finprods.empty() ? nullptr : p->h_finprods.data(), p->d_W, (int)p->K, (int)p->D, grid, p->d_partials,
                                 keeps ? p->d_sums[p->round & 1] : p->d_scratch, p->d_out, d_wide,
                                 publish_to_host ? p->h_out_dev : nullptr, publish_to_host ? p->h_flag_dev : nullptr,
                                 (p->wide_tagged && d_wide) ? p->wide_gen : p->seq,
                                 scaled | ((p->wide_tagged && d_wide) ? 2 : 0), fin_mb_enabled() ? p->d_fin_mb_counter : nullptr, p->stream, skip1 ? &ca : nullptr));
    p->sums_round = keeps && merged ? (int64_t)p->round : -1;
    }
    if (timed) HIP_TRY(hipEventRecord(p->ev1, p->stream));
    if (!deferred) {
        p->timed = timed;
        p->timing_pending = timed;
        p->prod_timed = timed && !small;
        p->prod_merged = merged;
        p->timed_round = p->round;
    }
    return SC_OK;
}

int await_round(sc_prover *p, uint64_t *out_evals, uint32_t want);

int resident_start(sc_prover *p, const uint64_t *r_or_null, uint64_t *out_evals);
int resident_round(sc_prover *p, const uint64_t *r_or_null, uint64_t *out_evals);
extern "C" int sc_prove_round(sc_prover *p, const uint64_t *r_or_null, uint64_t *out_evals) {
    if (!p || !out_evals) return sc_internal_fail(SC_ERR_BAD_ARG, "null argument");
    int rc = p->res.active ? resident_round(p, r_or_null, out_evals) : resident_start(p, r_or_null, out_evals);
    if (rc != kResidentGone) return rc;
    rc = launch_round(p, r_or_null, nullptr, true);
    if (rc) return rc;
    return await_round(p, out_evals, p->seq);
}

int await_round(sc_prover *p, uint64_t *out_evals, const uint32_t want) {
    uint64_t spins = 0;
    bool seen = false;
    const auto t_start = std::chrono::steady_clock::now();
    while (!(seen = (__atomic_load_n(p->h_flag, __ATOMIC_ACQUIRE) == want))) {
        if ((++spins & 0xfff) == 0) {
            if (std::chrono::steady_clock::now() - t_start > std::chrono::seconds(2)) break;
        }
    }
    if (!seen) {
        if (p->deferred_pending) {
            abandon_deferred(p);
            return sc_internal_fail(SC_ERR_HIP, "round did not publish its message within 2 s");
        }
        {
            DeviceGate gate_(p->device);
            HIP_TRY(hipStreamSynchronize(p->stream));
        }
        if (__atomic_load_n(p->h_flag, __ATOMIC_ACQUIRE) != want) return sc_internal_fail(SC_ERR_HIP, "round finished without publishing its message");
    }
    if (wait_gave_up(p)) {
        if (std::getenv("SC_HOST_TRACE"))
            std::fprintf(stderr, "[sc] give-up seen in await_round: marker %u, sig word %u, sig_seq %u, awaited seq %u, h_flag %u, round %u, deferred_pending %d, waited %.3f s\n",
                         __atomic_load_n(p->sig + 1, __ATOMIC_ACQUIRE), __atomic_load_n(p->sig, __ATOMIC_ACQUIRE), p->sig_seq, want,
                         __atomic_load_n(p->h_flag, __ATOMIC_ACQUIRE), p->round, (int)p->deferred_pending,
                         std::chrono::duration<double>(std::chrono::steady_clock::now() - t_start).count());
        abandon_deferred(p);
        p->exhausted = true;
        return sc_internal_fail(SC_ERR_HIP, "the host took longer than the wait kernel's bound to deliver a challenge; the proof is void");
    }
    std::memcpy(out_evals, p->h_out, (size_t)p->D * 32);
    return SC_OK;
}

constexpr size_t kTailSyncBytes = 4 * (16 + (size_t)scd::kTailMaxGrid);
std::atomic<uint64_t> g_stat[8];
struct TailOwner {
    std::mutex mu;
    sc_prover *owner = nullptr;
    bool resident = false;
    const uint32_t *marker = nullptr;
};
static TailOwner g_tail_owner[64];
bool tail_slot_acquire(sc_prover *p, bool resident) {
    TailOwner &t = g_tail_owner[(unsigned)p->device & 63u];
    std::lock_guard<std::mutex> lk(t.mu);
    if (t.owner && t.owner != p) {
        if (!(t.resident && t.marker && __atomic_load_n(t.marker, __ATOMIC_ACQUIRE) != 0)) {
            g_stat[kStatTailSlotBusy].fetch_add(1, std::memory_order_relaxed);
            return false;
        }
        g_stat[kStatTailSlotReclaims].fetch_add(1, std::memory_order_relaxed);
    }
    t.owner = p;
    t.resident = resident;
    t.marker = p->sig ? p->sig + 1 : nullptr;
    return true;
}
void tail_slot_release(sc_prover *p) {
    TailOwner &t = g_tail_owner[(unsigned)p->device & 63u];
    std::lock_guard<std::mutex> lk(t.mu);
    if (t.owner == p) {
        t.owner = nullptr;
        t.marker = nullptr;
    }
}
struct TailSlot {
    sc_prover *const p;
    bool held;
    explicit TailSlot(sc_prover *p_) : p(p_), held(tail_slot_acquire(p_, false)) {}
    ~TailSlot() {
        if (held) tail_slot_release(p);
    }
    TailSlot(const TailSlot &) = delete;
    TailSlot &operator=(const TailSlot &) = delete;
};
bool tail_shape_ok(const sc_prover *p) {
    return p->use_tail && p->K > 0 && p->U <= (uint32_t)scd::kMaxSmallTables && p->has_meta && p->K <= (uint32_t)scd::kMetaProds &&
           (size_t)p->K * p->D * (p->D + 2) * 32 <= 48 * 1024;
}
int tail_slices_blocks_for(sc_prover *p);
bool tail_possible(sc_prover *p, bool slices = false) {
    if (!tail_shape_ok(p) || p->exhausted || p->round >= p->nv || p->deferred_pending) return false;
    if (p->streamed && p->round < 2) return false;
    const uint64_t next_pairs = 1ULL << (p->nv - (p->round + 1));
    if (next_pairs > scd::kTailMaxPairs && !(slices && next_pairs <= scd::kTsMaxPairs && tail_slices_blocks_for(p) > 0)) return false;
    if (!ensure_mailbox(p)) return false;
    if (!p->d_tail_sync) {
        if (hipMalloc(reinterpret_cast<void **>(&p->d_tail_sync), kTailSyncBytes + 64 + (size_t)p->K * p->D * 32) != hipSuccess) {
            (void)hipGetLastError();
            return false;
        }
        p->tail_max_blocks = scd::tail_max_resident_blocks(p->device);
    }
    return p->tail_max_blocks > 0;
}

int tail_slices_blocks_for(sc_prover *p) {
    if (scd::policy(scd::kPolTailSlices) == 0 || p->max_mult > (uint32_t)(p->wide_tree ? scd::kMaxWideM : scd::kMaxFusedM) || p->round >= p->nv) return 0;
    const int B = scd::tail_slices_blocks(1ULL << (p->nv - (p->round + 1)), (int)p->U, (int)p->K, (int)p->D, p->n_combos, (int)p->max_mult,
                                          scd::tail_slices_max_blocks(p->device, (int)p->max_mult));
    if (B <= 0) return 0;
    if (!p->d_tail_xw) {
        if (hipMalloc(reinterpret_cast<void **>(&p->d_tail_xw), scd::kTsXwWords * 8) != hipSuccess ||
            hipMemsetAsync(p->d_tail_xw, 0, scd::kTsXwWords * 8, p->stream) != hipSuccess) {
            (void)hipGetLastError();
            if (p->d_tail_xw) (void)hipFree(p->d_tail_xw);
            p->d_tail_xw = nullptr;
            return 0;
        }
        p->ts_tag = 1;
        int large_bar = 0;
        if (scd::policy(scd::kPolVramMailbox) != 0 && hipDeviceGetAttribute(&large_bar, hipDeviceAttributeIsLargeBar, p->device) == hipSuccess && large_bar) {
            void *m = nullptr;
            if (hipExtMallocWithFlags(&m, 256, hipDeviceMallocFinegrained) == hipSuccess && hipMemsetAsync(m, 0, 256, p->stream) == hipSuccess &&
                hipStreamSynchronize(p->stream) == hipSuccess)
                p->d_vram_mail = static_cast<uint64_t *>(m);
            else if (m)
                (void)hipFree(m);
        }
        (void)hipGetLastError();
// ... 708 lines not shown
```

sumcheck_amd/csrc/prover_internal.hpp:

```cpp
#pragma once
#include <hip/hip_runtime.h>

#include <dlfcn.h>
#include <rccl/rccl.h>

#include <algorithm>
#include <array>
#include <atomic>
#include <chrono>
#include <condition_variable>
#include <map>
#include <memory>
#include <mutex>
#include <cstdarg>
#include <cstdio>
#include <cstdlib>
#include <cstring>
#include <new>
#include <string>
#include <thread>
#include <vector>

#include "../../include/sumcheck_hip.h"
#include "host_fr.hpp"
#include "kernels.h"
#include "transcript.hpp"

using scd::FinProd;
using scd::FrHost;
using scd::ProdArgs;
using scd::Combo;
using scd::TablePtrs;

std::chrono::milliseconds publish_timeout();
extern thread_local uint16_t g_gate_depth[64];
void gate_lock(int device);
void gate_unlock(int device);
struct DeviceGate {
    const int device;
    explicit DeviceGate(int d) : device(d) { gate_lock(device); }
    ~DeviceGate() { gate_unlock(device); }
    DeviceGate(const DeviceGate &) = delete;
    DeviceGate &operator=(const DeviceGate &) = delete;
};
struct GateYield {
    const int device;
    uint16_t depth;
    GateYield(int d, bool enable) : device(d), depth(enable ? g_gate_depth[(unsigned)d & 63u] : 0) {
        for (uint16_t i = 0; i < depth; ++i) gate_unlock(device);
    }
    ~GateYield() {
        for (uint16_t i = 0; i < depth; ++i) gate_lock(device);
    }
    GateYield(const GateYield &) = delete;
    GateYield &operator=(const GateYield &) = delete;
};
int sc_internal_fail(int code, const char *fmt, ...);
int &sc_internal_device_ref();
#define HIP_TRY(expr)                                                                                                   \
    do {                                                                                                                \
        hipError_t e_ = (expr);                                                                                         \
        if (e_ != hipSuccess) {                                                                                         \
            (void)hipGetLastError();                                                                                    \
            return sc_internal_fail(e_ == hipErrorOutOfMemory ? SC_ERR_OOM : SC_ERR_HIP, "%s failed: %s (%s:%d)", #expr,            \
                        hipGetErrorString(e_), __FILE__, __LINE__);                                                     \
        }                                                                                                               \
    } while (0)

static inline FrHost to_dev(const sch::Fr &a) {
    FrHost h;
    std::memcpy(&h, &a, sizeof(h));
    return h;
}

struct sc_rng {
    sch::Blake2b512Rng rng;
};

struct Product {
    sch::Fr coeff;
    std::vector<uint32_t> tables;
    std::vector<uint32_t> exps;
    uint32_t M = 0;
    bool fused = false;
    uint64_t partial_off = 0;
    uint32_t slot_off = 0;
};

struct Table {
    const uint4 *cur = nullptr;
    const int32_t *cur_top = nullptr;
    uint4 *buf[2] = {nullptr, nullptr};
    int32_t *buf_top[2] = {nullptr, nullptr};
    int next = 0;
};

constexpr uint32_t kResidentSpinsDefault = 256;
struct sc_prover {
    int device = 0;
    hipStream_t stream = nullptr;
    hipStream_t own_stream = nullptr;
    uint32_t nv = 0, max_mult = 0, D = 0, K = 0, U = 0, round = 0;
    bool exhausted = false;
    std::vector<sch::Fr> randomness;
    std::vector<Product> prods;
    std::vector<Table> tabs;
    void *arena = nullptr;
    FrHost *d_partials = nullptr;
    FrHost *d_partials2 = nullptr;
    uint32_t *d_fin_mb_counter = nullptr;
    uint32_t *d_fin_counters = nullptr;
    FinProd *d_finprods = nullptr;
    FrHost *d_W = nullptr;
    uint32_t w_elems = 0;
    bool w_scaled = false;
    FrHost *d_scratch = nullptr;
    FrHost *d_sums[2] = {nullptr, nullptr};
    int64_t sums_round = -1;
    FrHost *d_out = nullptr;
    FrHost *h_out = nullptr;
    uint32_t *h_flag = nullptr;
    FrHost *h_out_dev = nullptr;
    uint32_t *h_flag_dev = nullptr;
    uint32_t seq = 0;
    uint64_t *d_wide = nullptr;
    uint32_t wide_gen = 0;
    bool wide_tagged = false;
    uint64_t *h_wide = nullptr;
    uint64_t *h_wide_dev = nullptr;
    void *d_tail_send = nullptr, *d_tail_recv = nullptr, *d_tail_tabs = nullptr;
    sc_prover *tail = nullptr;
    uint32_t tail_ranks = 0;
    size_t tail_buf_bytes = 0;
    std::vector<std::vector<uint32_t>> prod_indices;
    Combo *d_combos = nullptr;
    std::vector<FinProd> h_finprods;
    scd::ComboMeta meta;
    bool has_meta = false;
    int n_combos = 0;
    bool any_generic = false;
    const uint4 **d_cur_tables = nullptr;
    const uint4 **h_cur_tables = nullptr;
    uint32_t *d_slot_table = nullptr, *d_slot_exp = nullptr;
    hipEvent_t ev0 = nullptr, ev1 = nullptr;
    bool timed = false;
    uint32_t *sig = nullptr;
    uint32_t *sig_dev = nullptr;
    uint32_t sig_seq = 0;
    FrHost *h_mail = nullptr;
    FrHost *h_mail_dev = nullptr;
    FrHost *d_mail = nullptr;
    uint32_t *d_tail_sync = nullptr;
    uint64_t *d_tail_xw = nullptr;
    uint32_t ts_tag = 1;
    uint64_t *d_vram_mail = nullptr;
    int tail_max_blocks = 0;
    uint64_t arena_bytes = 0;
    std::vector<uint8_t> pool_key;
    uint32_t n_retries = 0;
    bool pipeline_ok = true;
    bool polling_off_by_caller = false;
    struct Resident {
        bool active = false;
        bool first_has_bind = false;
        uint32_t seq0 = 0, sig0 = 0, n_rounds = 0, done = 0;
    } res;
    uint32_t resident_spins = kResidentSpinsDefault;
    bool deferred_pending = false;
    bool fused_finalize = false;
    bool use_tail = true;
    bool merge_rounds = false;
    bool wide_tree = true;
    bool use_f29 = false;
    bool use_fe = true;
    int kernel_variant = 3;
    bool streamed = false;
    uint32_t stream_chunk_request = 0;
    uint32_t chunk_log2 = 0;
    std::vector<const uint64_t *> host_tabs;
    void *ring[2] = {nullptr, nullptr};
    hipStream_t copy_stream = nullptr;
    hipStream_t copy_stream2 = nullptr;
    hipEvent_t ev_copied2[2] = {nullptr, nullptr};
    hipEvent_t ev_copied[2] = {nullptr, nullptr}, ev_consumed[2] = {nullptr, nullptr};
    FrHost *d_chunk_msg = nullptr;
    bool r1_cached = false, r1_keeps = false;
    bool borrow = false;
    std::vector<const uint4 *> origin;
    bool timing = false, timing_pending = false;
    bool prod_merged = false;
    bool prod_timed = false;
    std::vector<hipEvent_t> prod_ev;
    std::vector<double> prod_ms;
    std::vector<uint64_t> prod_launches;
    double rounds_ms = 0.0;
    std::vector<double> round_kernel_ms;
    std::vector<uint64_t> round_kernel_launches;
    uint32_t timed_round = 0;
};

int validate_desc(const sc_poly_desc *d);
void prover_destroy(sc_prover *p);
bool handle_pool_offer(sc_prover *p);
std::vector<uint8_t> pool_key_of(const sc_poly_desc *d, int device);
sc_prover *handle_pool_take(const std::vector<uint8_t> &key);
void claim_weights(uint32_t M, const sch::Fr &r, sch::Fr *lam);
void build_node_matrix(uint32_t M, uint32_t D, const sch::Fr &scale, std::vector<sch::Fr> &out);
int collect_timing(sc_prover *p);
int prover_bind_out(sc_prover *p, const uint64_t *r, uint64_t *d_out);
uint64_t sc_internal_cache_limit();
constexpr int kResidentGone = -1;
extern std::atomic<uint64_t> g_stat[8];
enum { kStatTailLaunches = 0, kStatTailSlotBusy = 1, kStatTailSlotReclaims = 2, kStatResidentStarts = 3, kStatResidentGone = 4, kStatProofRetries = 5, kStatTailSlices = 6 };
bool wide_tree_enabled();
int resident_quiesce(sc_prover *p);
int launch_round(sc_prover *p, const uint64_t *r_or_null, uint64_t *d_wide, bool publish_to_host, bool deferred = false);
bool staged_init_applies(const sc_prover *p);
int staged_copy_and_round1(sc_prover *p, const uint64_t *const *host_tables);
int await_round(sc_prover *p, uint64_t *out_evals, uint32_t want);
bool wait_gave_up(sc_prover *p);
void abandon_deferred(sc_prover *p);
int sc_internal_run_rounds(sc_prover *p, sch::Blake2b512Rng &rng, uint32_t n_rounds, uint64_t *out_msgs, sch::Fr *out_challenges);
bool launches_are_async(sc_prover *p);
bool tail_slot_acquire(sc_prover *p, bool resident);
void tail_slot_release(sc_prover *p);
void sc_internal_release_batch_cache();
struct NcclApi {
    void *lib = nullptr;
    decltype(&ncclGetUniqueId) GetUniqueId = nullptr;
    decltype(&ncclCommInitRank) CommInitRank = nullptr;
    decltype(&ncclAllReduce) AllReduce = nullptr;
    decltype(&ncclAllGather) AllGather = nullptr;
    decltype(&ncclCommDestroy) CommDestroy = nullptr;
    decltype(&ncclGetErrorString) GetErrorString = nullptr;
};
extern NcclApi g_nccl;
int nccl_load();
struct P2PGroup {
    std::mutex mu;
    std::condition_variable cv;
    int nranks = 0, joined = 0, left = 0;
    uint64_t *inbox[scd::kP2PMaxRanks] = {};
    int device[scd::kP2PMaxRanks] = {};
    int arrived = 0;
    uint64_t phase = 0;
    void *ptrs[scd::kP2PMaxRanks] = {};
    bool broken = false;
    bool exchange(int rank, void *mine, void **all_out) {
        std::unique_lock<std::mutex> lk(mu);
        if (broken) return false;
        const uint64_t my_phase = phase;
        ptrs[rank] = mine;
        if (++arrived == nranks) {
            arrived = 0;
            if (all_out) std::copy(ptrs, ptrs + nranks, all_out);
            last = std::vector<void *>(ptrs, ptrs + nranks);
            ++phase;
            cv.notify_all();
            return true;
        }
        if (!cv.wait_for(lk, std::chrono::seconds(60), [&] { return phase != my_phase || broken; }) || broken) {
            broken = true;
            cv.notify_all();
            return false;
        }
        if (all_out) std::copy(last.begin(), last.end(), all_out);
        return true;
    }
    std::vector<void *> last;
};

struct sc_comm {
    ncclComm_t comm = nullptr;
    int rank = 0, nranks = 1;
    sc_allreduce_u64_fn h_allreduce = nullptr;
    sc_allgather_fn h_allgather = nullptr;
    void *ctx = nullptr;
    std::shared_ptr<P2PGroup> p2p;
    uint64_t p2p_id = 0;
    uint32_t p2p_gen = 0;
    uint32_t direct_gen = 0;
    bool direct_publish = false;
    bool p2p_shared_device = false;
    int device = 0;
};
#define NCCL_TRY(expr)                                                                                             \
    do {                                                                                                           \
        int r_ = (int)(expr);                                                                                         \
        if (r_ != 0) return sc_internal_fail(SC_ERR_HIP, "%s failed: %s", #expr, g_nccl.GetErrorString ? g_nccl.GetErrorString((ncclResult_t)r_) : "?"); \
    } while (0)
int p2p_allgather(sc_comm *c, const void *d_send, void *d_recv, size_t bytes, hipStream_t s);
int p2p_allreduce_table(sc_comm *c, uint64_t *d_lanes, size_t n_words, hipStream_t s);
```

Baseline: 536.8 billion field-ops/s.

## Fuse round finalize into tree kernel via atomic per-group accumulators

Each block of the merged round-tree kernel now adds its per-node partial sums into per-group 64-bit accumulators with atomic fetch-add, packing a completion count into the high bits. The last block to finish runs the finalize (reduction, claim identity, weighting, output publish) in place. This removes the separate finalize kernel launch and the partials write/read round trip. In exchange it adds atomic traffic and a double-buffered ring that has to be zeroed, and it is gated on a new default-on policy.

```diff
diff --git a/include/sumcheck_hip.h b/include/sumcheck_hip.h
--- a/include/sumcheck_hip.h
+++ b/include/sumcheck_hip.h
@@ -154,6 +154,7 @@
 SC_API int sc_prover_get_round_timing(sc_prover *p, double *ms_per_round, uint64_t *launches_per_round);
 SC_API int sc_prover_reset(sc_prover *p, const uint64_t *const *tables_or_null, uint32_t flags);
 SC_API int sc_claim_weights(uint32_t M, const uint64_t *r, uint64_t *out);
+SC_API int sc_fused_finalize_plan(uint32_t grid, uint32_t n_items, uint64_t *out);
 SC_API int sc_fr_elementwise(int op, const uint64_t *a, const uint64_t *b, uint64_t *out, uint64_t n);
 SC_API int sc_bench_modmul(uint64_t n_threads, uint32_t reps, uint32_t variant, float *ms_out, uint64_t *checksum_out);
 
diff --git a/sumcheck_amd/_lib.py b/sumcheck_amd/_lib.py
--- a/sumcheck_amd/_lib.py
+++ b/sumcheck_amd/_lib.py
@@ -114,6 +114,7 @@
     "sc_prover_get_round_timing": (C.c_int, [_V, C.POINTER(C.c_double), u64p]),
     "sc_prover_reset": (C.c_int, [_V, _V, C.c_uint32]),
     "sc_claim_weights": (C.c_int, [C.c_uint32, _V, _V]),
+    "sc_fused_finalize_plan": (C.c_int, [C.c_uint32, C.c_uint32, _V]),
     "sc_fr_elementwise": (C.c_int, [C.c_int, _V, _V, _V, C.c_uint64]),
     "sc_bench_modmul": (C.c_int, [C.c_uint64, C.c_uint32, C.c_uint32, C.POINTER(C.c_float), u64p]),
 }
diff --git a/sumcheck_amd/csrc/abi.hip b/sumcheck_amd/csrc/abi.hip
--- a/sumcheck_amd/csrc/abi.hip
+++ b/sumcheck_amd/csrc/abi.hip
@@ -90,8 +90,8 @@
     if (p->own_stream) (void)hipStreamSynchronize(p->own_stream);
     if (p->arena) (void)hipFree(p->arena);
     if (p->d_partials) (void)hipFree(p->d_partials);
-    if (p->d_partials2) (void)hipFree(p->d_partials2);
-    if (p->d_fin_counters) (void)hipFree(p->d_fin_counters);
+    if (p->d_fin_acc) (void)hipFree(p->d_fin_acc);
+    if (p->d_fin_mb_counter) (void)hipFree(p->d_fin_mb_counter);
     if (p->d_finprods) (void)hipFree(p->d_finprods);
     if (p->d_W) (void)hipFree(p->d_W);
     if (p->d_scratch) (void)hipFree(p->d_scratch);
@@ -269,7 +269,6 @@
         if (d->prod_offsets[k + 1] - d->prod_offsets[k] > 4) p->merge_rounds = false;
 #ifdef SC_EXPERIMENTS
     if (const char *e = std::getenv("SC_MERGE")) p->merge_rounds = p->merge_rounds && std::atoi(e) != 0;
-    if (const char *e = std::getenv("SC_FUSED_FIN")) p->fused_finalize = std::atoi(e) != 0;
 #endif
     p->use_tail = scd::policy(scd::kPolTail) != 0;
 
@@ -378,10 +377,10 @@
         HIP_TRY(hipMalloc(&p->d_chunk_msg, (size_t)2 * p->D * 32));
     }
     HIP_TRY(hipMalloc(&p->d_partials, std::max<uint64_t>(partial_elems, 1) * 32));
-    HIP_TRY(hipMalloc(&p->d_partials2, std::max<uint64_t>(partial_elems, 1) * 32));
-    HIP_TRY(hipMalloc(&p->d_fin_counters, 4 * (2 + scd::kMaxGrid / 32 + 16)));
-    HIP_TRY(hipMemsetAsync(p->d_fin_counters, 0, 4 * (2 + scd::kMaxGrid / 32 + 16), p->stream));
-    p->d_fin_mb_counter = p->d_fin_counters + (2 + scd::kMaxGrid / 32 + 8);
+    HIP_TRY(hipMalloc(&p->d_fin_acc, scd::kFusedRingWords * 8));
+    HIP_TRY(hipMemsetAsync(p->d_fin_acc, 0, scd::kFusedRingWords * 8, p->stream));
+    HIP_TRY(hipMalloc(&p->d_fin_mb_counter, 64));
+    HIP_TRY(hipMemsetAsync(p->d_fin_mb_counter, 0, 64, p->stream));
     HIP_TRY(hipMalloc(&p->d_finprods, std::max<size_t>(p->K, 1) * sizeof(FinProd)));
     if (p->K) HIP_TRY(hipMemcpyAsync(p->d_finprods, fin.data(), p->K * sizeof(FinProd), hipMemcpyHostToDevice, p->stream));
     p->h_finprods = fin;
@@ -1043,7 +1042,7 @@
 constexpr PolicyDef kPolicyDefs[scd::kPolCount] = {
     {"pipeline", 1, 0, 1},     {"resident", 1, 0, 1},          {"tail_slices", 1, 0, 1}, {"vram_mailbox", 1, 0, 1},           {"wide_tree", 1, 0, 1},
     {"rccl_direct", 1, 0, 1},  {"shard_gather_log2", 15, 1, 15}, {"gkr_direct", 1, 0, 1},  {"wait_spins", 1 << 22, 1, 0xffffffffLL}, {"tail", 1, 0, 1},
-    {"staged_init", 1, 0, 1},  {"batch", 1, 0, 2},
+    {"staged_init", 1, 0, 1},  {"batch", 1, 0, 2},             {"fused_finalize", 1, 0, 1},
 };
 struct PolicyTable {
     std::atomic<int64_t> v[scd::kPolCount];
@@ -1066,7 +1065,7 @@
 std::atomic<uint64_t> g_plan[scd::kPlanCount];
 constexpr const char *kPlanNames[scd::kPlanCount] = {
     "big.merged.round1", "big.merged.bind_chain", "big.merged.bind", "big.claim_identity", "big.store_f29", "big.store_canonical", "big.per_product_tree",
-    "big.wide", "big.wide16", "big.generic", "big.node_by_node", "big.bind_pass", "big.streamed", "big.staged_round1", "finalize.multi_block", "finalize.one_block", "finalize.no_lds",
+    "big.wide", "big.wide16", "big.generic", "big.node_by_node", "big.bind_pass", "big.streamed", "big.staged_round1", "finalize.multi_block", "finalize.one_block", "finalize.no_lds", "big.fused_finalize",
     "small.launched", "small.combos_table", "small.ptrs", "small.pipelined", "tail.slices8", "tail.slices12", "tail.rounds", "resident.slices",
     "resident.rounds", "sharded.rccl_direct", "sharded.rccl_publish", "sharded.host", "sharded.p2p", "sharded.gather_tail", "gkr.bucketed_grouped",
     "gkr.bucketed_counted", "gkr.list_form", "gkr.coeff_from_bound_table", "gkr.sharded", "fold_multi",
@@ -1291,6 +1290,19 @@
     return SC_OK;
 }
 
+extern "C" int sc_fused_finalize_plan(uint32_t grid, uint32_t n_items, uint64_t *out) {
+    if (!out) return sc_internal_fail(SC_ERR_BAD_ARG, "null argument");
+    if (grid < 1 || grid > (uint32_t)scd::kMaxGrid || n_items < 1 || n_items > scd::kFusedMaxItems)
+        return sc_internal_fail(SC_ERR_BAD_ARG, "in-kernel finalize: grid 1..%d and 1..%u (product, node) pairs, not %u and %u", scd::kMaxGrid, scd::kFusedMaxItems, grid, n_items);
+    const uint32_t groups = scd::fused_groups(grid);
+    out[0] = groups;
+    out[1] = scd::fused_group_size(grid, groups, 0);
+    out[2] = scd::fused_set_words(grid, n_items);
+    out[3] = scd::kFusedSetWords;
+    out[4] = scd::kFusedRing;
+    out[5] = scd::kFusedCountShift;
+    return SC_OK;
+}
 extern "C" int sc_claim_weights(uint32_t M, const uint64_t *r, uint64_t *out) {
     if (!r || !out) return sc_internal_fail(SC_ERR_BAD_ARG, "null argument");
     if (M < 1 || M > 4) return sc_internal_fail(SC_ERR_BAD_ARG, "claim weights exist for 1..4 multiplicands, not %u", M);
diff --git a/sumcheck_amd/csrc/kernels.h b/sumcheck_amd/csrc/kernels.h
--- a/sumcheck_amd/csrc/kernels.h
+++ b/sumcheck_amd/csrc/kernels.h
@@ -47,21 +47,50 @@
 struct TreeProd {
     Slot slot[4];
     uint32_t M;
+    uint32_t item_off;
+    uint64_t partial_off;
+};
+constexpr int kFusedCountShift = 44;
+constexpr uint32_t kFusedPerGroup = 32;
+constexpr uint32_t kFusedMaxItems = 5 * 12;
+__host__ __device__ constexpr uint32_t fused_groups(uint32_t grid) { return (grid + kFusedPerGroup - 1) / kFusedPerGroup; }
+__host__ __device__ constexpr uint32_t fused_group_size(uint32_t grid, uint32_t groups, uint32_t g) { return grid / groups + (g < grid % groups ? 1u : 0u); }
+__host__ __device__ constexpr size_t fused_set_words(uint32_t grid, uint32_t n_items) { return (size_t)fused_groups(grid) * n_items * 8; }
+constexpr size_t kFusedSetWords = (size_t)(1024 / kFusedPerGroup) * kFusedMaxItems * 8;
+constexpr size_t kFusedScratchBytes = 16384;
+constexpr int kFusedRing = 2;
+constexpr size_t kFusedRingWords = kFusedRing * kFusedSetWords + kFusedRing;
+#ifdef SC_SERIAL_EPILOGUE
+constexpr bool kFusedFinalizeBuilt = false;
+#else
+constexpr bool kFusedFinalizeBuilt = true;
+#endif
+struct ClaimArgs {
+    uint32_t skip1;
     uint32_t pad;
-    uint64_t partial_off;
-};
+    const uint4 *prev;
+    FrHost lam[14];
+};
+__host__ __device__ constexpr int claim_off(int M) { return (M - 1) * (M + 2) / 2; }
 struct RoundFin {
     int enabled;
     int D;
+    uint32_t groups;
+    uint32_t n_items;
+    uint32_t total;
+    uint32_t zero_words;
     uint64_t w_off[kMaxRoundProds];
     const uint4 *Wm;
-    uint4 *partials2;
-    uint32_t *counters;
+    uint64_t *acc;
+    uint64_t *counter;
+    uint64_t *acc_next;
+    uint64_t *counter_next;
+    uint4 *sums;
     uint4 *out;
-    uint64_t *out_wide;
     uint4 *h_out;
     uint32_t *h_flag;
     uint32_t seq;
+    ClaimArgs claim;
 };
 struct RoundArgs {
     TreeProd prod[kMaxRoundProds];
@@ -237,6 +266,7 @@
     kPolTail,
     kPolStagedInit,
     kPolBatch,
+    kPolFusedFinalize,
     kPolCount
 };
 int64_t policy(int key);
@@ -259,6 +289,7 @@
     kPlanFinalizeMultiBlock,
     kPlanFinalizeOneBlock,
     kPlanFinalizeNoLds,
+    kPlanBigFusedFinalize,
     kPlanSmallLaunched,
     kPlanSmallCombosTable,
     kPlanSmallPtrs,
@@ -325,13 +356,6 @@
                                   const uint32_t *d_slot_exp, uint64_t n_pairs, FrHost *d_partials, int grid, hipStream_t stream);
 hipError_t launch_sum_combos_meta(const TablePtrs &tp, const ComboMeta &meta, int n_combos, uint64_t n_pairs, FrHost *d_partials, int grid,
                                   hipStream_t stream);
-struct ClaimArgs {
-    uint32_t skip1;
-    uint32_t pad;
-    const uint4 *prev;
-    FrHost lam[14];
-};
-__host__ __device__ constexpr int claim_off(int M) { return (M - 1) * (M + 2) / 2; }
 constexpr int kWideTagShift = 44;
 __host__ __device__ constexpr uint32_t wide_tag_of(uint32_t seq) { return (seq & 0x7fffu) + 1u; }
 bool finalize_keeps_sums(int K, int D, int nblocks, bool have_host_prods, bool have_counter);
diff --git a/sumcheck_amd/csrc/kernels_big.hip b/sumcheck_amd/csrc/kernels_big.hip
--- a/sumcheck_amd/csrc/kernels_big.hip
+++ b/sumcheck_amd/csrc/kernels_big.hip
@@ -149,7 +149,8 @@
 
 template <int M, bool kR1 = false, bool kChain = kChainDefault, bool kSkip1 = false>
 __device__ __forceinline__ void tree_pass(const Slot *S, const int32_t (&r)[kBindLds], const uint64_t n_pairs, uint4 *__restrict__ row, uint32_t (*sm)[8],
-                                          int32_t *lacc, const uint32_t part_stride = 0) {
+                                          int32_t *lacc, const uint32_t part_stride = 0, const RoundFin *F = nullptr, const bool fuse = false, const uint32_t item0 = 0,
+                                          uint32_t *fin_last = nullptr) {
     const uint64_t pstride = part_stride ? part_stride : gridDim.x;
     static_assert(!(kSkip1 && kR1), "round 1 has no previous round to take node 1 from");
     int32_t *my = lacc + threadIdx.x;
@@ -393,7 +394,19 @@
             for (int i = 0; i < 8; ++i) o.v[i] = x[(w * (M + 1) + t) * 8 + i];
             acc = fr_add(acc, o);
         }
-        fr_store(row + 2 * ((uint64_t)t * pstride), acc);
+        if (fuse) {
+            const uint32_t g = blockIdx.x % F->groups, last = fused_group_size(gridDim.x, F->groups, g) - 1;
+            uint64_t *a = F->acc + ((size_t)g * F->n_items + item0 + (uint32_t)t) * 8;
+            uint64_t old[8];
+#pragma unroll
+            for (int i = 0; i < 8; ++i) old[i] = __hip_atomic_fetch_add(a + i, (1ULL << kFusedCountShift) | (uint64_t)acc.v[i], __ATOMIC_RELAXED, __HIP_MEMORY_SCOPE_AGENT);
+            uint32_t done = 0;
+#pragma unroll
+            for (int i = 0; i < 8; ++i) done += (uint32_t)(old[i] >> kFusedCountShift) == last ? 1u : 0u;
+            if (done && __hip_atomic_fetch_add(F->counter, (uint64_t)done, __ATOMIC_RELAXED, __HIP_MEMORY_SCOPE_AGENT) + done == F->total) *fin_last = 1u;
+        } else {
+            fr_store(row + 2 * ((uint64_t)t * pstride), acc);
+        }
     }
     __syncthreads();
 #else
@@ -505,15 +518,11 @@
 #endif
 
 #ifdef SC_EXPERIMENTS
-constexpr int kFinGroup = 32;
 __global__ __launch_bounds__(kBlock, 3) void k_round_tree(const RoundArgs R, const BindConst r, const uint64_t n_pairs,
                                                        uint4 *__restrict__ partials) {
     __shared__ uint32_t sm[kBlock / 64][8];
     __shared__ int32_t rt[kBindLds];
     __shared__ int32_t lacc[9 * 5 * kBlock];
-#ifdef SC_EXPERIMENTS
-    __shared__ uint32_t role_sh;
-#endif
     bind_consts_to_lds(r, rt);
     const int n = R.n_prod;
     int k = (int)((blockIdx.x & 7u) % (uint32_t)n);
@@ -528,65 +537,102 @@
         }
         if (++k == n) k = 0;
     }
-#ifdef SC_EXPERIMENTS
-    if (!R.fin.enabled) return;
-    const uint32_t G = gridDim.x, n_groups = (G + kFinGroup - 1) / kFinGroup;
-    const uint32_t g = blockIdx.x / kFinGroup, g_first = g * kFinGroup, g_size = min((uint32_t)kFinGroup, G - g_first);
+}
+#endif
+
+__device__ __forceinline__ void round_finalize(const RoundArgs &R, uint4 *__restrict__ fin_lds) {
+    const RoundFin &F = R.fin;
+    const int K = R.n_prod, D = F.D, tid = (int)threadIdx.x;
+    struct Meta {
+        uint32_t M[kMaxRoundProds], item_off[kMaxRoundProds];
+        uint64_t w_off[kMaxRoundProds];
+        FrHost lam[14];
+    };
+    static_assert(kFusedScratchBytes + sizeof(Meta) <= sizeof(int32_t) * 9 * 5 * kBlock, "behind the finalize scratch, inside the running sums' LDS");
+    Meta *ms = reinterpret_cast<Meta *>(reinterpret_cast<char *>(fin_lds) + kFusedScratchBytes);
+    for (int k = 0; k < K; ++k) {
+        if (tid == 0) {
+            ms->M[k] = R.prod[k].M;
+            ms->item_off[k] = R.prod[k].item_off;
+            ms->w_off[k] = F.w_off[k];
+        }
+    }
+    if (F.claim.skip1) {
+        for (int i = 0; i < 14; ++i)
+            if (tid == 0) ms->lam[i] = F.claim.lam[i];
+    }
     __syncthreads();
-    if (threadIdx.x == 0) {
-        __builtin_amdgcn_fence(__ATOMIC_RELEASE, "agent");
-        const uint32_t d = __hip_atomic_fetch_add(R.fin.counters + 1 + g, 1u, __ATOMIC_RELAXED, __HIP_MEMORY_SCOPE_AGENT);
-        role_sh = d == g_size - 1 ? 1u : 0u;
-        if (role_sh) __builtin_amdgcn_fence(__ATOMIC_ACQUIRE, "agent");
-    }
-    __syncthreads();
-    if (!role_sh) return;
-    {
-        int n_items = 0;
-        for (int q = 0; q < n; ++q) n_items += (int)R.prod[q].M + 1;
-        for (int it0 = 0; it0 < 4 * n_items; it0 += kBlock) {
-            const int it = it0 + (int)threadIdx.x;
-            const bool live = it < 4 * n_items;
-            int c = live ? it >> 2 : 0, q4 = it & 3, pk = 0;
-            while (c > (int)R.prod[pk].M) { c -= (int)R.prod[pk].M + 1; ++pk; }
-            const uint4 *base = partials + 2 * (R.prod[pk].partial_off + (uint64_t)c * G + g_first);
-            Fr acc = fr_zero();
-            if (live)
-                for (uint32_t b = (uint32_t)q4 * 8; b < min((uint32_t)q4 * 8 + 8, g_size); ++b) acc = fr_add(acc, fr_load(base + 2 * b));
-            acc = fr_add(acc, fr_shfl_down(acc, 2));
-            acc = fr_add(acc, fr_shfl_down(acc, 1));
-            if (live && q4 == 0) fr_store(R.fin.partials2 + 2 * (R.prod[pk].partial_off + (uint64_t)c * n_groups + g), acc);
-        }
-    }
-    __syncthreads();
-    if (threadIdx.x == 0) {
-        __builtin_amdgcn_fence(__ATOMIC_RELEASE, "agent");
-        const uint32_t d = __hip_atomic_fetch_add(R.fin.counters, 1u, __ATOMIC_RELAXED, __HIP_MEMORY_SCOPE_AGENT);
-        role_sh = d == n_groups - 1 ? 2u : 0u;
-        if (role_sh) __builtin_amdgcn_fence(__ATOMIC_ACQUIRE, "agent");
-    }
-    __syncthreads();
-    if (role_sh != 2u) return;
-    for (uint32_t i = threadIdx.x; i <= n_groups; i += kBlock)
-        __hip_atomic_store(R.fin.counters + i, 0u, __ATOMIC_RELAXED, __HIP_MEMORY_SCOPE_AGENT);
     auto prod_of = [&](int q) -> FinProd {
         FinProd f;
-        f.M = R.prod[q].M;
+        f.M = ms->M[q];
         f.pad = 0;
-        f.partial_off = R.prod[q].partial_off;
-        f.w_off = R.fin.w_off[q];
+        f.partial_off = 0;
+        f.w_off = ms->w_off[q];
         return f;
     };
-    finalize_body<kBlock>(prod_of, R.fin.Wm, n, R.fin.D, (int)n_groups, R.fin.partials2, reinterpret_cast<uint4 *>(lacc), R.fin.out, R.fin.out_wide,
-                          R.fin.h_out, R.fin.h_flag, R.fin.seq, 1);
-#endif
-}
-#endif
+    const bool compact = fin_compact<kBlock>(K, D);
+    Fr w_pre = fr_zero();
+    if (compact) w_pre = fin_prefetch_weight(prod_of, F.Wm, K, D, 1);
+    const uint32_t groups = F.groups, n_items = F.n_items;
+    const int sh = groups > 1 ? 32 - __builtin_clz(groups - 1) : 0;
+    for (uint32_t base = 0; base < (n_items << sh); base += kBlock) {
+        const uint32_t idx = base + (uint32_t)tid, item = idx >> sh, g = idx & ((1u << sh) - 1u);
+        int k = 0, t = 0;
+        bool live = item < n_items && g < groups;
+        if (item < n_items) {
+            for (k = 0; k + 1 < K && item >= ms->item_off[k + 1]; ++k) {}
+            t = (int)(item - ms->item_off[k]);
+        }
+        live = live && !(F.claim.skip1 && t == 1);
+        Fr v = fr_zero();
+        if (live) {
+            const uint64_t *a = F.acc + ((size_t)g * n_items + item) * 8;
+            uint64_t w[8];
+#pragma unroll
+            for (int q = 0; q < 8; ++q) w[q] = __hip_atomic_load(a + q, __ATOMIC_RELAXED, __HIP_MEMORY_SCOPE_AGENT);
+            Fr x;
+            uint64_t carry = 0;
+#pragma unroll
+            for (int q = 0; q < 8; ++q) {
+                const uint64_t s = (w[q] & ((1ULL << kFusedCountShift) - 1)) + carry;
+                x.v[q] = (uint32_t)s;
+                carry = s >> 32;
+            }
+            Fe e = fe_from_fr(x);
+            e.l[8] += (int32_t)(carry << 24);
+            v = fe_to_fr(e);
+        }
+        for (int off = (1 << sh) >> 1; off >= 1; off >>= 1) v = fr_add(v, fr_shfl_down(v, off));
+        if (live && g == 0) fr_store(fin_lds + 2 * (k * D + t), v);
+    }
+    __syncthreads();
+    if (F.claim.skip1) {
+        for (int c = tid; c < K * D; c += kBlock) {
+            const int M = (int)ms->M[c / D], sN = c % D;
+            if (sN <= M) fr_store(fin_lds + 2 * (K * D + c), fr_mul(fr_from_host(ms->lam[claim_off(M) + sN]), fr_load(F.claim.prev + 2 * c)));
+        }
+        __syncthreads();
+        for (int k = tid; k < K; k += kBlock) {
+            Fr claim = fr_load(fin_lds + 2 * (K * D + k * D));
+            for (int sN = 1; sN <= (int)ms->M[k]; ++sN) claim = fr_add(claim, fr_load(fin_lds + 2 * (K * D + k * D + sN)));
+            fr_store(fin_lds + 2 * (k * D + 1), fr_sub(claim, fr_load(fin_lds + 2 * (k * D))));
+        }
+        __syncthreads();
+    }
+    for (int c = tid; c < K * D; c += kBlock)
+        if (c % D <= (int)ms->M[c / D]) fr_store(F.sums + 2 * c, fr_load(fin_lds + 2 * c));
+    finalize_message<kBlock>(prod_of, F.Wm, K, D, fin_lds, F.out, (uint64_t *)nullptr, F.h_out, F.h_flag, F.seq, 1, compact ? &w_pre : nullptr);
+    for (uint32_t i = (uint32_t)tid; i < F.zero_words; i += kBlock) __hip_atomic_store(F.acc_next + i, 0ULL, __ATOMIC_RELAXED, __HIP_MEMORY_SCOPE_AGENT);
+    if (tid == 0) __hip_atomic_store(F.counter_next, 0ULL, __ATOMIC_RELAXED, __HIP_MEMORY_SCOPE_AGENT);
+}
 
 __global__ __launch_bounds__(kBlock, 3) void k_round1_tree_split(const RoundArgs R, const uint64_t n_pairs, uint4 *__restrict__ partials) {
     __shared__ uint32_t sm[kBlock / 64][8];
     __shared__ int32_t rt[kBindLds];
     __shared__ int32_t lacc[9 * 5 * kBlock];
+    __shared__ uint32_t fin_last;
+    if (threadIdx.x == 0) fin_last = 0;
+    const bool fuse = R.fin.enabled != 0;
     const TreeProd &T = R.prod[blockIdx.y];
     uint4 *row = partials + 2 * (T.partial_off + (uint64_t)R.part_block0 + (uint64_t)blockIdx.x);
 #ifdef SC_NO_CHAIN_R1
@@ -595,26 +641,31 @@
     constexpr bool kC1 = true;
 #endif
     switch (T.M) {
-    case 1: tree_pass<1, true, kC1>(T.slot, rt, n_pairs, row, sm, lacc, R.part_stride); break;
-    case 2: tree_pass<2, true, kC1>(T.slot, rt, n_pairs, row, sm, lacc, R.part_stride); break;
-    case 3: tree_pass<3, true, kC1>(T.slot, rt, n_pairs, row, sm, lacc, R.part_stride); break;
-    default: tree_pass<4, true, kC1>(T.slot, rt, n_pairs, row, sm, lacc, R.part_stride); break;
-    }
+    case 1: tree_pass<1, true, kC1>(T.slot, rt, n_pairs, row, sm, lacc, R.part_stride, &R.fin, fuse, T.item_off, &fin_last); break;
+    case 2: tree_pass<2, true, kC1>(T.slot, rt, n_pairs, row, sm, lacc, R.part_stride, &R.fin, fuse, T.item_off, &fin_last); break;
+    case 3: tree_pass<3, true, kC1>(T.slot, rt, n_pairs, row, sm, lacc, R.part_stride, &R.fin, fuse, T.item_off, &fin_last); break;
+    default: tree_pass<4, true, kC1>(T.slot, rt, n_pairs, row, sm, lacc, R.part_stride, &R.fin, fuse, T.item_off, &fin_last); break;
+    }
+    if (fuse && fin_last) round_finalize(R, reinterpret_cast<uint4 *>(lacc));
 }
 template <bool kChain, bool kSkip1>
 __global__ __launch_bounds__(kBlock, 3) void k_round_tree_split(const RoundArgs R, const BindConst r, const uint64_t n_pairs, uint4 *__restrict__ partials) {
     __shared__ uint32_t sm[kBlock / 64][8];
     __shared__ int32_t rt[kBindLds];
     __shared__ int32_t lacc[9 * 5 * kBlock];
+    __shared__ uint32_t fin_last;
+    if (threadIdx.x == 0) fin_last = 0;
+    const bool fuse = R.fin.enabled != 0;
     bind_consts_to_lds(r, rt);
     const TreeProd &T = R.prod[blockIdx.y];
     uint4 *row = partials + 2 * (T.partial_off + (uint64_t)blockIdx.x);
     switch (T.M) {
-    case 1: tree_pass<1, false, kChain, kSkip1>(T.slot, rt, n_pairs, row, sm, lacc); break;
-    case 2: tree_pass<2, false, kChain, kSkip1>(T.slot, rt, n_pairs, row, sm, lacc); break;
-    case 3: tree_pass<3, false, kChain, kSkip1>(T.slot, rt, n_pairs, row, sm, lacc); break;
-    default: tree_pass<4, false, kChain, kSkip1>(T.slot, rt, n_pairs, row, sm, lacc); break;
-    }
+    case 1: tree_pass<1, false, kChain, kSkip1>(T.slot, rt, n_pairs, row, sm, lacc, 0, &R.fin, fuse, T.item_off, &fin_last); break;
+    case 2: tree_pass<2, false, kChain, kSkip1>(T.slot, rt, n_pairs, row, sm, lacc, 0, &R.fin, fuse, T.item_off, &fin_last); break;
+    case 3: tree_pass<3, false, kChain, kSkip1>(T.slot, rt, n_pairs, row, sm, lacc, 0, &R.fin, fuse, T.item_off, &fin_last); break;
+    default: tree_pass<4, false, kChain, kSkip1>(T.slot, rt, n_pairs, row, sm, lacc, 0, &R.fin, fuse, T.item_off, &fin_last); break;
+    }
+    if (fuse && fin_last) round_finalize(R, reinterpret_cast<uint4 *>(lacc));
 }
 
 #ifdef SC_EXPERIMENTS
@@ -698,7 +749,8 @@
     }();
     extra_lds = env_lds;
 #endif
-    bool round1 = args.fin.enabled == 0;
+    if (args.fin.enabled && !(kFusedFinalizeBuilt && split && args.part_stride == 0 && args.fin.groups == fused_groups((uint32_t)grid))) return hipErrorInvalidValue;
+    bool round1 = true;
     for (int q = 0; q < args.n_prod && round1; ++q)
         for (uint32_t f = 0; f < args.prod[q].M; ++f) round1 = round1 && args.prod[q].slot[f].mode == 0 && args.prod[q].slot[f].src_top == nullptr;
 #ifdef SC_EXPERIMENTS
diff --git a/sumcheck_amd/csrc/protocol.hip b/sumcheck_amd/csrc/protocol.hip
--- a/sumcheck_amd/csrc/protocol.hip
+++ b/sumcheck_amd/csrc/protocol.hip
@@ -296,7 +296,7 @@
 };
 bool fin_mb_enabled();
 bool staged_init_applies(const sc_prover *p) {
-    return scd::policy(scd::kPolStagedInit) != 0 && p->merge_rounds && !p->any_generic && !p->streamed && !p->borrow && !p->fused_finalize && p->kernel_variant == 3 &&
+    return scd::policy(scd::kPolStagedInit) != 0 && p->merge_rounds && !p->any_generic && !p->streamed && !p->borrow && p->kernel_variant == 3 &&
            p->nv >= 18 && p->K > 0 && p->K <= (uint32_t)scd::kMetaProds;
 }
 int staged_copy_and_round1(sc_prover *p, const uint64_t *const *host_tables) {
@@ -528,10 +528,24 @@
     bool ptrs_uploaded = false;
     bool finalized = false;
     bool skip1 = false;
+    auto fill_claim = [&](scd::ClaimArgs &ca) {
+        std::memset(&ca, 0, sizeof(ca));
+        ca.skip1 = 1;
+        ca.prev = reinterpret_cast<const uint4 *>(p->d_sums[(p->round - 1) & 1]);
+        bool done[5] = {false, false, false, false, false};
+        for (uint32_t k = 0; k < p->K; ++k) {
+            const uint32_t M = p->prods[k].M;
+            if (done[M]) continue;
+            done[M] = true;
+            sch::Fr lam[5];
+            claim_weights(M, r, lam);
+            for (uint32_t s2 = 0; s2 <= M; ++s2) ca.lam[scd::claim_off((int)M) + (int)s2] = to_dev(lam[s2]);
+        }
+    };
     const bool merged = !small && p->merge_rounds && !p->any_generic;
     if (merged) {
         grid = std::min(grid, scd::kRoundTreeGrid);
-        bool split = !p->fused_finalize;
+        bool split = true;
         int split_grid = n_pairs >= (1ULL << 21) ? 1024 : n_pairs >= (1ULL << 20) ? 768 : n_pairs >= (1ULL << 18) ? 384 : n_pairs >= (1ULL << 17) ? 256 : 192;
 #ifdef SC_EXPERIMENTS
         static const bool split_off = std::getenv("SC_SPLIT") && std::atoi(std::getenv("SC_SPLIT")) == 0;
@@ -588,25 +602,50 @@
                 }
             }
         }
-        p->seq += 1;
-        ra.fin.enabled = p->fused_finalize ? 1 : 0;
-        ra.fin.D = (int)p->D;
-        for (uint32_t k = 0; k < p->K; ++k) ra.fin.w_off[k] = p->h_finprods[k].w_off;
-        ra.fin.Wm = reinterpret_cast<const uint4 *>(p->d_W);
-        ra.fin.partials2 = reinterpret_cast<uint4 *>(p->d_partials2);
-        ra.fin.counters = p->d_fin_counters;
-        ra.fin.out = reinterpret_cast<uint4 *>(p->d_out);
-        ra.fin.out_wide = d_wide;
-        ra.fin.h_out = publish_to_host ? reinterpret_cast<uint4 *>(p->h_out_dev) : nullptr;
-        ra.fin.h_flag = publish_to_host ? p->h_flag_dev : nullptr;
-        ra.fin.seq = p->seq;
+        const bool fuse = split && scd::kFusedFinalizeBuilt && scd::policy(scd::kPolFusedFinalize) != 0 && d_wide == nullptr && p->d_fin_acc != nullptr &&
+                          scd::finalize_keeps_sums((int)p->K, (int)p->D, grid, !p->h_finprods.empty(), fin_mb_enabled()) &&
+                          (size_t)p->K * p->D * (p->D + 2) * 32 <= scd::kFusedScratchBytes && grid <= scd::kMaxGrid;
+        if (fuse) {
+            scd::RoundFin &f = ra.fin;
+            uint32_t n_items = 0;
+            for (uint32_t k = 0; k < p->K; ++k) {
+                ra.prod[k].item_off = n_items;
+                n_items += p->prods[k].M + 1;
+                f.w_off[k] = p->h_finprods[k].w_off;
+            }
+            const uint32_t set = (uint32_t)(p->fin_launches & 1u);
+            p->fin_launches += 1;
+            p->seq += 1;
+            f.enabled = 1;
+            f.D = (int)p->D;
+            f.groups = scd::fused_groups((uint32_t)grid);
+            f.n_items = n_items;
+            f.total = 8 * f.groups * (n_items - (skip1 ? p->K : 0u));
+            f.zero_words = p->fin_dirty_words[set ^ 1u];
+            p->fin_dirty_words[set ^ 1u] = 0;
+            p->fin_dirty_words[set] = (uint32_t)scd::fused_set_words((uint32_t)grid, n_items);
+            f.Wm = reinterpret_cast<const uint4 *>(p->d_W);
+            f.acc = p->d_fin_acc + (size_t)set * scd::kFusedSetWords;
+            f.acc_next = p->d_fin_acc + (size_t)(set ^ 1u) * scd::kFusedSetWords;
+            f.counter = p->d_fin_acc + scd::kFusedRing * scd::kFusedSetWords + set;
+            f.counter_next = p->d_fin_acc + scd::kFusedRing * scd::kFusedSetWords + (set ^ 1u);
+            f.sums = reinterpret_cast<uint4 *>(p->d_sums[p->round & 1]);
+            f.out = reinterpret_cast<uint4 *>(p->d_out);
+            f.h_out = publish_to_host ? reinterpret_cast<uint4 *>(p->h_out_dev) : nullptr;
+            f.h_flag = publish_to_host ? p->h_flag_dev : nullptr;
+            f.seq = p->seq;
+            if (skip1) fill_claim(f.claim);
+            scd::plan_hit(scd::kPlanBigFusedFinalize);
+        }
         if (p->timing) HIP_TRY(hipEventRecord(p->prod_ev[0], p->stream));
         if (bind) scd::plan_hit(p->use_f29 ? scd::kPlanBigF29Store : scd::kPlanBigCanonicalStore);
         HIP_TRY(scd::launch_round_tree(ra, rc, n_pairs, p->d_partials, grid, p->stream, split, skip1));
         if (p->timing) HIP_TRY(hipEventRecord(p->prod_ev[1], p->stream));
         scaled = 1;
-        if (p->fused_finalize) finalized = true;
-        else p->seq -= 1;
+        if (fuse) {
+            finalized = true;
+            p->sums_round = (int64_t)p->round;
+        }
     }
     for (uint32_t k = 0; k < p->K && !small && !merged; ++k) {
         const Product &pr = p->prods[k];
@@ -723,19 +762,7 @@
     const bool keeps = scd::finalize_keeps_sums((int)p->K, (int)p->D, grid, !p->h_finprods.empty(), fin_mb_enabled());
     scd::ClaimArgs ca;
     std::memset(&ca, 0, sizeof(ca));
-    if (skip1) {
-        ca.skip1 = 1;
-        ca.prev = reinterpret_cast<const uint4 *>(p->d_sums[(p->round - 1) & 1]);
-        bool done[5] = {false, false, false, false, false};
-        for (uint32_t k = 0; k < p->K; ++k) {
-            const uint32_t M = p->prods[k].M;
-            if (done[M]) continue;
-            done[M] = true;
-            sch::Fr lam[5];
-            claim_weights(M, r, lam);
-            for (uint32_t s2 = 0; s2 <= M; ++s2) ca.lam[scd::claim_off((int)M) + (int)s2] = to_dev(lam[s2]);
-        }
-    }
+    if (skip1) fill_claim(ca);
     SlowCallProbe pr_fin("launch k_finalize");
     HIP_TRY(scd::launch_finalize(p->d_finprods, p->h_finprods.empty() ? nullptr : p->h_finprods.data(), p->d_W, (int)p->K, (int)p->D, grid, p->d_partials,
                                  keeps ? p->d_sums[p->round & 1] : p->d_scratch, p->d_out, d_wide,
diff --git a/sumcheck_amd/csrc/prover_internal.hpp b/sumcheck_amd/csrc/prover_internal.hpp
--- a/sumcheck_amd/csrc/prover_internal.hpp
+++ b/sumcheck_amd/csrc/prover_internal.hpp
@@ -107,9 +107,10 @@
     std::vector<Table> tabs;
     void *arena = nullptr;
     FrHost *d_partials = nullptr;
-    FrHost *d_partials2 = nullptr;
+    uint64_t *d_fin_acc = nullptr;
+    uint64_t fin_launches = 0;
+    uint32_t fin_dirty_words[2] = {0, 0};
     uint32_t *d_fin_mb_counter = nullptr;
-    uint32_t *d_fin_counters = nullptr;
     FinProd *d_finprods = nullptr;
     FrHost *d_W = nullptr;
     uint32_t w_elems = 0;
@@ -167,7 +168,6 @@
     } res;
     uint32_t resident_spins = kResidentSpinsDefault;
     bool deferred_pending = false;
-    bool fused_finalize = false;
     bool use_tail = true;
     bool merge_rounds = false;
     bool wide_tree = true;
```

New measurement: 535.5 billion field-ops/s. About the same (-0.2%).
